# marqo-ai/marqo

Measured on AMD Instinct MI355X. Metric: embeddings/sec, higher is better.
Workload: dtype bf16; 1 GPU; open_clip ViT-B/32 image tower, uint8 224x224 resident in HBM (tower-only), batch 256/GPU; global_batch=256, parallelism=dp1 (replicated weights, sharded items, RCCL all_gather of embeddings), weights=random-init (seed 0) ViT-B-32, last_block_rows=pooled

## Files before the change

marqo_amd/csrc/embed.hip:

```cpp
#include "common.h"

namespace {

template <bool U8>
__global__ __launch_bounds__(256) void patchify_kernel(const void* __restrict__ in, bf16_t* __restrict__ out,
                                                       int64_t total_groups, int S, int P, int G, int Kp,
                                                       float sc0, float sc1, float sc2, float of0, float of1, float of2) {
    const int groups_per_row = Kp >> 3;
    const int PP = P * P;
    __shared__ float lutf[U8 ? 3 * 256 : 1];
    if (U8) {
        const float t = (float)threadIdx.x;
        lutf[threadIdx.x] = (t / 255.0f - of0) / sc0;
        lutf[(U8 ? 256 : 0) + (U8 ? threadIdx.x : 0)] = (t / 255.0f - of1) / sc1;
        lutf[(U8 ? 512 : 0) + (U8 ? threadIdx.x : 0)] = (t / 255.0f - of2) / sc2;
        __syncthreads();
    }
    for (int64_t gi = (int64_t)blockIdx.x * 256 + threadIdx.x; gi < total_groups; gi += (int64_t)gridDim.x * 256) {
        const int64_t prow = gi / groups_per_row;
        const int col0 = (int)(gi - prow * groups_per_row) * 8;
        const int64_t img = prow / (G * G);
        const int pidx = (int)(prow - img * (G * G));
        const int py = pidx / G, px = pidx - py * G;
        float v[8];
        if (U8 && (P & 7) == 0 && col0 < 3 * PP) {
            const int c = col0 / PP;
            const int rem = col0 - c * PP;
            const int ky = rem / P, kx = rem - ky * P;
            const uint8_t* src = (const uint8_t*)in + ((img * S + (py * P + ky)) * S + (px * P + kx)) * 3 + c;
#pragma unroll
            for (int e = 0; e < 8; ++e) v[e] = lutf[U8 ? c * 256 + src[e * 3] : 0];
        } else
#pragma unroll
        for (int e = 0; e < 8; ++e) {
            const int col = col0 + e;
            float val = 0.f;
            if (col < 3 * PP) {
                const int c = col / PP;
                const int rem = col - c * PP;
                const int ky = rem / P, kx = rem - ky * P;
                const int y = py * P + ky, x = px * P + kx;
                if (U8) {
                    const uint8_t b = ((const uint8_t*)in)[((img * S + y) * S + x) * 3 + c];
                    val = lutf[U8 ? c * 256 + b : 0];
                } else {
                    val = ((const float*)in)[((img * 3 + c) * S + y) * (int64_t)S + x];
                }
            }
            v[e] = val;
        }
        uint4 p;
        p.x = pack_bf16x2(v[0], v[1]);
        p.y = pack_bf16x2(v[2], v[3]);
        p.z = pack_bf16x2(v[4], v[5]);
        p.w = pack_bf16x2(v[6], v[7]);
        *(uint4*)(out + prow * Kp + col0) = p;
    }
}

__global__ __launch_bounds__(256) void patchify_u8x8_kernel(const uint8_t* __restrict__ in, bf16_t* __restrict__ out, int64_t total,
                                                            int S, int P, int G, int Kp, float sc0, float sc1, float sc2,
                                                            float of0, float of1, float of2) {
    __shared__ bf16_t lut[3 * 256];
    {
        const float t = (float)threadIdx.x;
        lut[threadIdx.x] = f32_to_bf16((t / 255.0f - of0) / sc0);
        lut[256 + threadIdx.x] = f32_to_bf16((t / 255.0f - of1) / sc1);
        lut[512 + threadIdx.x] = f32_to_bf16((t / 255.0f - of2) / sc2);
    }
    __syncthreads();
    const int per_row = P >> 3, per_patch = P * per_row, PP = P * P;
    for (int64_t gi = (int64_t)blockIdx.x * 256 + threadIdx.x; gi < total; gi += (int64_t)gridDim.x * 256) {
        const int64_t prow = gi / per_patch;
        const int rem = (int)(gi - prow * per_patch);
        const int ky = rem / per_row, kx = (rem - ky * per_row) * 8;
        const int64_t img = prow / (G * G);
        const int pidx = (int)(prow - img * (G * G));
        const int py = pidx / G, px = pidx - py * G;
        const uint2* src = (const uint2*)(in + ((img * S + (py * P + ky)) * S + (px * P + kx)) * 3);
        const uint2 w0 = src[0], w1 = src[1], w2 = src[2];
        const uint32_t words[6] = {w0.x, w0.y, w1.x, w1.y, w2.x, w2.y};
        uint32_t v[3][8];
#pragma unroll
        for (int b = 0; b < 24; ++b) {
            const uint32_t byte = (words[b >> 2] >> ((b & 3) * 8)) & 0xffu;
            const int c = b % 3, e = b / 3;
            v[c][e] = (uint32_t)lut[c * 256 + byte];
        }
        bf16_t* dst = out + prow * Kp + ky * P + kx;
#pragma unroll
        for (int c = 0; c < 3; ++c) {
            uint4 p;
            p.x = v[c][0] | (v[c][1] << 16);
            p.y = v[c][2] | (v[c][3] << 16);
            p.z = v[c][4] | (v[c][5] << 16);
            p.w = v[c][6] | (v[c][7] << 16);
            *(uint4*)(dst + c * PP) = p;
        }
    }
}

constexpr int MAXC = 8;
template <int CH>
__global__ __launch_bounds__(256, (CH <= 4 ? 8 : 4)) void vit_assemble_kernel(
    const float* __restrict__ patch_out, const float* __restrict__ cls, const float* __restrict__ pos,
    const float* __restrict__ gam, const float* __restrict__ bet, float* __restrict__ x, int64_t rows, int T, int W, float eps, int x_bf16) {
    const int lane = threadIdx.x & 63;
    const int64_t row = (int64_t)blockIdx.x * 4 + (threadIdx.x >> 6);
    if (row >= rows) return;
    auto put = [&](int c, const f32x4& y) {
        if (x_bf16) {
            uint2 q;
            q.x = pack_bf16x2(y[0], y[1]);
            q.y = pack_bf16x2(y[2], y[3]);
            *(uint2*)((bf16_t*)x + row * W + c * 4) = q;
        } else {
            *(f32x4*)(x + row * W + c * 4) = y;
        }
    };
    const int64_t b = row / T;
    const int t = (int)(row - b * T);
    const float* src = !cls ? patch_out + row * W : (t == 0 ? cls : patch_out + (b * (T - 1) + (t - 1)) * W);
    const float* pr = pos + (int64_t)t * W;
    const int nch = W >> 2;
    f32x4 v[CH];
#pragma unroll
    for (int i = 0; i < CH; ++i) {
        const int c = lane + i * 64;
        v[i] = c < nch ? *(const f32x4*)(src + c * 4) + *(const f32x4*)(pr + c * 4) : f32x4{0.f, 0.f, 0.f, 0.f};
    }
    if (!gam) {
#pragma unroll
        for (int i = 0; i < CH; ++i) {
            const int c = lane + i * 64;
            if (c < nch) put(c, v[i]);
        }
        return;
    }
    ln_normalize_row<CH>(v, lane, nch, W, eps);
#pragma unroll
    for (int i = 0; i < CH; ++i) {
        const int c = lane + i * 64;
        if (c < nch) {
            const f32x4 gg = *(const f32x4*)(gam + c * 4);
            const f32x4 bb = *(const f32x4*)(bet + c * 4);
            f32x4 y;
#pragma unroll
            for (int e = 0; e < 4; ++e) y[e] = v[i][e] * gg[e] + bb[e];
            put(c, y);
        }
    }
}

__global__ __launch_bounds__(256) void map_pool_kernel(const bf16_t* __restrict__ kv, const float* __restrict__ q, bf16_t* __restrict__ out,
                                                       int64_t nh, int T, int W, int heads, int hd) {
    extern __shared__ float sp[];
    const int lane = threadIdx.x & 63, wave = threadIdx.x >> 6;
    const int64_t item = (int64_t)blockIdx.x * 4 + wave;
    if (item >= nh) return;
    const int64_t img = item / heads;
    const int h = (int)(item - img * heads);
    float* p = sp + wave * T;
    const bf16_t* kbase = kv + img * T * (int64_t)(2 * W) + h * hd;
    const float* qh = q + h * hd;
    float mx = -INFINITY;
    for (int t = lane; t < T; t += 64) {
        const bf16_t* kr = kbase + (int64_t)t * (2 * W);
        float s = 0.f;
        for (int d = 0; d < hd; d += 8) {
            const uint4 k8 = *(const uint4*)(kr + d);
            const uint32_t kw[4] = {k8.x, k8.y, k8.z, k8.w};
#pragma unroll
            for (int e = 0; e < 4; ++e)
                s += __uint_as_float(kw[e] << 16) * qh[d + 2 * e] + __uint_as_float(kw[e] & 0xffff0000u) * qh[d + 2 * e + 1];
        }
        p[t] = s;
        mx = fmaxf(mx, s);
    }
    mx = wave_max(mx);
    float sum = 0.f;
    for (int t = lane; t < T; t += 64) {
        const float e = __expf(p[t] - mx);
        p[t] = e;
        sum += e;
    }
    sum = wave_sum(sum);
    const float inv = 1.0f / sum;
    __builtin_amdgcn_fence(__ATOMIC_RELEASE, "wavefront");
    __builtin_amdgcn_wave_barrier();
    const bf16_t* vbase = kbase + W;
    float o0 = 0.f, o1 = 0.f;
    const bool two = lane + 64 < hd;
    if (lane < hd) {
        for (int t = 0; t < T; ++t) {
            const bf16_t* vr = vbase + (int64_t)t * (2 * W);
            const float pt = p[t];
            o0 += pt * bf16_to_f32(vr[lane]);
            if (two) o1 += pt * bf16_to_f32(vr[lane + 64]);
        }
        bf16_t* orow = out + img * W + h * hd;
        orow[lane] = f32_to_bf16(o0 * inv);
        if (two) orow[lane + 64] = f32_to_bf16(o1 * inv);
    }
}

template <bool LN, int CH>
__global__ __launch_bounds__(256, (CH <= 2 ? 8 : 4)) void embed_tokens_kernel(
    const int32_t* __restrict__ ids, const int32_t* __restrict__ cu, const float* __restrict__ tok,
    const float* __restrict__ pos, const float* __restrict__ type0, const float* __restrict__ gam,
    const float* __restrict__ bet, float* __restrict__ x, bf16_t* __restrict__ xb, int W, int vocab, float eps, int last_pos) {
    const int lane = threadIdx.x & 63, wave = threadIdx.x >> 6;
    const int row0 = cu[blockIdx.x], len = cu[blockIdx.x + 1] - row0;
    const int nch = W >> 2;
    for (int t = wave; t < len; t += 4) {
        const int64_t row = row0 + t;
        int id = ids[row];
        id = id < 0 ? 0 : (id >= vocab ? vocab - 1 : id);
        const float* tr = tok + (int64_t)id * W;
        const float* pr = pos ? pos + (int64_t)((last_pos > 0 && t == len - 1) ? last_pos : t) * W : nullptr;
        f32x4 v[CH];
#pragma unroll
        for (int i = 0; i < CH; ++i) {
            const int c = lane + i * 64;
            v[i] = f32x4{0.f, 0.f, 0.f, 0.f};
            if (c < nch) {
                v[i] = *(const f32x4*)(tr + c * 4);
                if (pr) v[i] += *(const f32x4*)(pr + c * 4);
                if (type0) v[i] += *(const f32x4*)(type0 + c * 4);
            }
        }
        if (LN) ln_normalize_row<CH>(v, lane, nch, W, eps);
#pragma unroll
        for (int i = 0; i < CH; ++i) {
            const int c = lane + i * 64;
            if (c < nch) {
                f32x4 y = v[i];
                if (LN) {
                    const f32x4 gg = *(const f32x4*)(gam + c * 4);
                    const f32x4 bb = *(const f32x4*)(bet + c * 4);
#pragma unroll
                    for (int e = 0; e < 4; ++e) y[e] = v[i][e] * gg[e] + bb[e];
                }
                if (x) *(f32x4*)(x + row * W + c * 4) = y;
                if (xb) {
                    uint2 p;
                    p.x = pack_bf16x2(y[0], y[1]);
                    p.y = pack_bf16x2(y[2], y[3]);
                    *(uint2*)(xb + row * W + c * 4) = p;
                }
            }
        }
    }
}

__global__ __launch_bounds__(256) void pool_kernel(const float* __restrict__ x, const int32_t* __restrict__ cu,
                                                   float* __restrict__ out, int W, int pool, int normalize) {
    __shared__ float red[4];
    const int row0 = cu[blockIdx.x], len = cu[blockIdx.x + 1] - row0;
    float acc[8];
    float ss = 0.f;
#pragma unroll
    for (int i = 0; i < 8; ++i) {
        acc[i] = 0.f;
        const int c = threadIdx.x + i * 256;
        if (c < W) {
            if (pool == MQ_POOL_CLS) {
                acc[i] = x[(int64_t)row0 * W + c];
            } else {
                float s = 0.f;
                for (int t = 0; t < len; ++t) s += x[(int64_t)(row0 + t) * W + c];
                acc[i] = s / (float)len;
            }
            ss += acc[i] * acc[i];
        }
    }
    float inv = 1.f;
    if (normalize) {
        ss = wave_sum(ss);
        if ((threadIdx.x & 63) == 0) red[threadIdx.x >> 6] = ss;
        __syncthreads();
        const float tot = red[0] + red[1] + red[2] + red[3];
        inv = 1.0f / fmaxf(sqrtf(tot), 1e-12f);
    }
#pragma unroll
    for (int i = 0; i < 8; ++i) {
        const int c = threadIdx.x + i * 256;
        if (c < W) out[(int64_t)blockIdx.x * W + c] = acc[i] * inv;
    }
}

__global__ void last_rows_kernel(const int32_t* __restrict__ cu, int32_t* __restrict__ rows, int nseq) {
    const int i = blockIdx.x * blockDim.x + threadIdx.x;
    if (i < nseq) rows[i] = cu[i + 1] - 1;
}
__global__ void cls_rows_kernel(int32_t* __restrict__ rows, int n, int T) {
    const int i = blockIdx.x * blockDim.x + threadIdx.x;
    if (i < n) rows[i] = i * T;
}

template <bool SCATTER>
__global__ __launch_bounds__(256) void move_rows_kernel(uint4* __restrict__ sparse, const int32_t* __restrict__ idx,
                                                         uint4* __restrict__ dense, int64_t n, int chunks) {
    const int64_t total = n * chunks;
    for (int64_t i = (int64_t)blockIdx.x * 256 + threadIdx.x; i < total; i += (int64_t)gridDim.x * 256) {
        const int64_t r = i / chunks;
        const int c = (int)(i - r * chunks);
        uint4* sp = sparse + (int64_t)idx[r] * chunks + c;
        if (SCATTER) *sp = dense[i];
        else dense[i] = *sp;
    }
}

}

extern "C" int mq_patchify(const void* d_in, int32_t is_u8, void* d_out, int64_t n, int32_t S, int32_t P, int32_t Kp, const float* mean,
                           const float* std, void* stream) {
    const hipStream_t s = (hipStream_t)stream;
    const int G = S / P;
    const int64_t total = n * G * G * (Kp >> 3);
    if (total <= 0) return MQ_OK;
    MqProfScope prof(5, s);
    const unsigned grid = (unsigned)(cdiv64(total, 256) < 16384 ? cdiv64(total, 256) : 16384);
    if (is_u8 && (P & 7) == 0 && Kp == 3 * P * P && (S * 3) % 8 == 0 && ((uintptr_t)d_in & 7) == 0) {
        const int64_t items = n * G * G * P * (P >> 3);
        const unsigned g8 = (unsigned)(cdiv64(items, 256) < 16384 ? cdiv64(items, 256) : 16384);
        hipLaunchKernelGGL(patchify_u8x8_kernel, dim3(g8), dim3(256), 0, s, (const uint8_t*)d_in, (bf16_t*)d_out, items, S, P, G, Kp,
                           std[0], std[1], std[2], mean[0], mean[1], mean[2]);
    } else if (is_u8)
        hipLaunchKernelGGL(patchify_kernel<true>, dim3(grid), dim3(256), 0, s, d_in, (bf16_t*)d_out, total, S, P, G, Kp,
                           std[0], std[1], std[2], mean[0], mean[1], mean[2]);
    else
        hipLaunchKernelGGL(patchify_kernel<false>, dim3(grid), dim3(256), 0, s, d_in, (bf16_t*)d_out, total, S, P, G, Kp,
                           1.f, 1.f, 1.f, 0.f, 0.f, 0.f);
    MQ_CHECK_LAUNCH("mq_patchify");
    return MQ_OK;
}

extern "C" int mq_vit_assemble(const float* d_patch_out, const float* cls, const float* pos, const float* g, const float* b, void* d_x, int64_t n,
                               int32_t T, int32_t W, float eps, int32_t x_bf16, void* stream) {
    const hipStream_t s = (hipStream_t)stream;
    MQ_CHECK_ARG(W % 4 == 0 && W <= 64 * 4 * MAXC, "vit_assemble: W=%d unsupported", W);
    const int64_t rows = n * T;
    if (rows <= 0) return MQ_OK;
    MqProfScope prof(3, s);
    MQ_DISPATCH_CH(W, hipLaunchKernelGGL(vit_assemble_kernel<CH>, dim3((unsigned)cdiv64(rows, 4)), dim3(256), 0, s, d_patch_out,
                                         cls, pos, g, b, (float*)d_x, rows, T, W, eps, x_bf16));
    MQ_CHECK_LAUNCH("vit_assemble");
    return MQ_OK;
}

__global__ __launch_bounds__(256) void avg_tokens_kernel(const void* __restrict__ xv, int x_bf16, float* __restrict__ out, int T, int first, int W) {
    const int64_t img = blockIdx.x;
    const float inv = 1.0f / (float)(T - first);
    for (int c = threadIdx.x * 4; c < W; c += 256 * 4) {
        f32x4 acc = f32x4{0.f, 0.f, 0.f, 0.f};
        for (int t = first; t < T; ++t) {
            const int64_t o = (img * T + t) * (int64_t)W + c;
            if (x_bf16) {
                const uint2 q = *(const uint2*)((const bf16_t*)xv + o);
                acc += f32x4{__uint_as_float(q.x << 16), __uint_as_float(q.x & 0xffff0000u), __uint_as_float(q.y << 16), __uint_as_float(q.y & 0xffff0000u)};
            } else {
                acc += *(const f32x4*)((const float*)xv + o);
            }
        }
        *(f32x4*)(out + img * W + c) = acc * inv;
    }
}

extern "C" int mq_avg_tokens(const void* d_x, int32_t x_bf16, float* d_out, int64_t n, int32_t T, int32_t first, int32_t W, void* stream) {
    const hipStream_t s = (hipStream_t)stream;
    MQ_CHECK_ARG(W % 4 == 0 && first >= 0 && first < T, "avg_tokens: bad shape W=%d T=%d first=%d", W, T, first);
    if (n <= 0) return MQ_OK;
    MqProfScope prof(4, s);
    hipLaunchKernelGGL(avg_tokens_kernel, dim3((unsigned)n), dim3(256), 0, s, d_x, x_bf16, d_out, T, first, W);
    MQ_CHECK_LAUNCH("avg_tokens");
    return MQ_OK;
}

extern "C" int mq_map_pool(const void* d_kv, const float* d_q, void* d_out, int64_t n, int32_t T, int32_t W, int32_t heads, void* stream) {
    const hipStream_t s = (hipStream_t)stream;
    MQ_CHECK_ARG(heads >= 1 && W % heads == 0, "map_pool: W=%d heads=%d", W, heads);
    const int hd = W / heads;
    MQ_CHECK_ARG(hd % 8 == 0 && hd <= 128, "map_pool: head dim %d unsupported (multiple of 8, <= 128)", hd);
    MQ_CHECK_ARG(T >= 1 && T <= 4096, "map_pool: %d tokens unsupported", T);
    if (n <= 0) return MQ_OK;
    MqProfScope prof(4, s);
    const int64_t nh = n * heads;
    hipLaunchKernelGGL(map_pool_kernel, dim3((unsigned)cdiv64(nh, 4)), dim3(256), (size_t)4 * T * sizeof(float), s, (const bf16_t*)d_kv, d_q,
                       (bf16_t*)d_out, nh, T, W, heads, hd);
    MQ_CHECK_LAUNCH("map_pool");
    return MQ_OK;
}

extern "C" int mq_embed_tokens(const int32_t* d_ids, const int32_t* d_cu, int64_t nseq, const float* tok, const float* pos, const float* type0,
                               const float* g, const float* b, float* d_x, void* d_xb, int32_t W, int32_t vocab, float eps, int32_t last_pos,
                               void* stream) {
    const hipStream_t s = (hipStream_t)stream;
    MQ_CHECK_ARG(W % 4 == 0 && W <= 64 * 4 * MAXC, "embed_tokens: W=%d unsupported", W);
    if (nseq <= 0) return MQ_OK;
    MqProfScope prof(3, s);
    if (g)
        MQ_DISPATCH_CH(W, hipLaunchKernelGGL((embed_tokens_kernel<true, CH>), dim3((unsigned)nseq), dim3(256), 0, s, d_ids, d_cu,
                                             tok, pos, type0, g, b, d_x, (bf16_t*)d_xb, W, vocab, eps, last_pos));
    else
        MQ_DISPATCH_CH(W, hipLaunchKernelGGL((embed_tokens_kernel<false, CH>), dim3((unsigned)nseq), dim3(256), 0, s, d_ids, d_cu,
                                             tok, pos, type0, g, b, d_x, (bf16_t*)d_xb, W, vocab, eps, last_pos));
    MQ_CHECK_LAUNCH("embed_tokens");
    return MQ_OK;
}

__global__ __launch_bounds__(256) void rope_kernel(bf16_t* __restrict__ qkv, const int32_t* __restrict__ cu, int fixed_len, int Wa, int heads,
                                                   int hs, int hd, const float* __restrict__ inv_freq) {
    const int row0 = cu ? cu[blockIdx.x] : blockIdx.x * fixed_len;
    const int len = cu ? cu[blockIdx.x + 1] - row0 : fixed_len;
    const int half = hd >> 1, chunks = half >> 3;
    const int per_row = 2 * heads * chunks;
    for (int it = threadIdx.x; it < len * per_row; it += 256) {
        const int t = it / per_row, r = it - t * per_row;
        const int qk = r / (heads * chunks), r2 = r - qk * heads * chunks;
        const int h = r2 / chunks, c = r2 - h * chunks;
        bf16_t* p = qkv + (int64_t)(row0 + t) * (3 * Wa) + qk * Wa + h * hs + c * 8;
        uint4 lo = *(const uint4*)p, hi = *(const uint4*)(p + half);
        uint32_t* l = (uint32_t*)&lo;
        uint32_t* u = (uint32_t*)&hi;
#pragma unroll
        for (int e = 0; e < 4; ++e) {
            float x1[2] = {bf16_to_f32((bf16_t)(l[e] & 0xffff)), bf16_to_f32((bf16_t)(l[e] >> 16))};
            float x2[2] = {bf16_to_f32((bf16_t)(u[e] & 0xffff)), bf16_to_f32((bf16_t)(u[e] >> 16))};
            float y1[2], y2[2];
#pragma unroll
            for (int k = 0; k < 2; ++k) {
                float sn, cs;
                sincosf((float)t * inv_freq[c * 8 + e * 2 + k], &sn, &cs);
                y1[k] = x1[k] * cs - x2[k] * sn;
                y2[k] = x2[k] * cs + x1[k] * sn;
            }
            l[e] = pack_bf16x2(y1[0], y1[1]);
            u[e] = pack_bf16x2(y2[0], y2[1]);
        }
        *(uint4*)p = lo;
        *(uint4*)(p + half) = hi;
    }
}

extern "C" int mq_rope(void* d_qkv, const int32_t* d_cu, int64_t nseq, int32_t fixed_len, int32_t Wa, int32_t heads, const float* d_inv_freq,
                       void* stream) {
    const hipStream_t s = (hipStream_t)stream;
    const int hs = Wa / heads;
    MQ_CHECK_ARG(hs * heads == Wa && hs % 16 == 0, "rope: head width %d must be a multiple of 16", hs);
    if (nseq <= 0) return MQ_OK;
    MqProfScope prof(3, s);
    hipLaunchKernelGGL(rope_kernel, dim3((unsigned)nseq), dim3(256), 0, s, (bf16_t*)d_qkv, d_cu, fixed_len, Wa, heads, hs, hs, d_inv_freq);
    MQ_CHECK_LAUNCH("rope");
    return MQ_OK;
}

__device__ __forceinline__ float glu_act(float g, int act) { return act == MQ_ACT_SILU ? silu(g) : act == MQ_ACT_QUICKGELU ? quick_gelu(g) : gelu_erf(g); }

__global__ __launch_bounds__(256) void glu_kernel(bf16_t* __restrict__ buf, int64_t rows, int F, int act) {
    const int chunks = F >> 3;
    for (int64_t i = (int64_t)blockIdx.x * 256 + threadIdx.x; i < rows * chunks; i += (int64_t)gridDim.x * 256) {
        const int64_t r = i / chunks;
        const int c = (int)(i - r * chunks);
        bf16_t* p = buf + r * (2 * (int64_t)F) + c * 8;
        uint4 up = *(const uint4*)p;
        const uint4 gt = *(const uint4*)(p + F);
        uint32_t* a = (uint32_t*)&up;
        const uint32_t* g = (const uint32_t*)&gt;
#pragma unroll
        for (int e = 0; e < 4; ++e) {
            const float u0 = bf16_to_f32((bf16_t)(a[e] & 0xffff)), u1 = bf16_to_f32((bf16_t)(a[e] >> 16));
            const float g0 = bf16_to_f32((bf16_t)(g[e] & 0xffff)), g1 = bf16_to_f32((bf16_t)(g[e] >> 16));
            a[e] = pack_bf16x2(u0 * glu_act(g0, act), u1 * glu_act(g1, act));
        }
        *(uint4*)p = up;
    }
}

int mq_glu_il_rows(void* d_buf, int64_t rows, int F, int act, hipStream_t s);
extern "C" int mq_glu(void* d_buf, int64_t rows, int32_t F, int32_t act, int32_t interleaved, void* stream) {
    const hipStream_t s = (hipStream_t)stream;
    MQ_CHECK_ARG(F % 8 == 0 && (!interleaved || F % 16 == 0), "glu: F=%d must be a multiple of 8 (16 interleaved)", F);
    if (rows <= 0) return MQ_OK;
    MqProfScope prof(3, s);
    const int64_t blocks = cdiv64(rows * (F >> 3), 256);
    if (interleaved) {
        MQ_CHECK_ARG(F <= 4096, "glu (interleaved): F=%d > 4096", F);
        return mq_glu_il_rows(d_buf, rows, F, act, s);
    }
    hipLaunchKernelGGL(glu_kernel, dim3((unsigned)(blocks < 16384 ? blocks : 16384)), dim3(256), 0, s, (bf16_t*)d_buf, rows, F, act);
    MQ_CHECK_LAUNCH("glu");
    return MQ_OK;
}

template <int CH, int MODE = 0>
__global__ __launch_bounds__(256) void glu_ln_kernel(bf16_t* __restrict__ buf, int64_t rows, int F, int Ft, int act, const float* __restrict__ g,
                                                     const float* __restrict__ b, float eps) {
    const int64_t row = (int64_t)blockIdx.x * 4 + (threadIdx.x >> 6);
    const int lane = threadIdx.x & 63;
    if (row >= rows) return;
    bf16_t* p = buf + row * (2 * (int64_t)F);
    float v[CH][8];
    float s1 = 0.f;
// ... 165 lines not shown
```

marqo_amd/csrc/gemm_bf16.hip:

```cpp
#include <map>
#include <mutex>
#include <string>
#include <type_traits>
#include "common.h"
#include "gemm_epilogue.h"
#include "gemm_loop.h"
#include "gemm_sched.h"

extern mq_knob mq_tower_row_select;
extern mq_knob mq_tower_ln_fold;
extern mq_knob mq_tower_subln_fold;
extern mq_knob mq_tower_attn_proj;
extern mq_knob mq_tower_panel_gemm;
extern mq_knob mq_attention_waves;
extern mq_knob mq_tower_residual_bf16;
extern mq_knob mq_gemm_small_max_rows;
bool mq_gemm_small_ok(int64_t M, int64_t N, int64_t K, bool ln);
bool mq_gemm_small_grouped_ok(int64_t M, int64_t N, int64_t K);
extern mq_knob mq_gemm_small_group_rows;
extern mq_knob mq_ln_prefetch;
extern mq_knob mq_ln_rows_per_wave;
extern mq_knob mq_ln_bf16_wide;
int mq_gemm_small(const void* d_A, int64_t lda, const void* d_W, int64_t ldw, const float* d_bias, const void* d_residual, void* d_out,
                  int64_t ldc, int64_t M, int64_t N, int64_t K, int flags, hipStream_t s);
int mq_gemm_wd_launch(int flags, int mt, int ns, const void* A, int64_t lda, const void* W, int64_t ldw, const float* bias, const float* residual, void* out,
                      int64_t ldc, int M, int N, int K, const GemmGeom& g, int wide, const GemmLn& ln, hipStream_t s);

int mq_device_ok();

namespace {

struct GemmSk {
    float* partials;
    unsigned* flags;
    unsigned epoch;
    int tail_splits;
};

template <int FLAGS, int MT, int NH, int WM, int ORD>
__global__ __launch_bounds__(128 * WM, (NH == 1 && WM == 2) ? 2 : 1) void gemm_nt_kernel(
    const bf16_t* __restrict__ A, int64_t lda, const bf16_t* __restrict__ Wt, int64_t ldw,
    const float* __restrict__ bias, const float* residual, void* out, int64_t ldc,
    int M, int N, int K, int tiles_n, int num_tiles, int cgroup, int band_rows, int wide_store,
    unsigned a_bytes, unsigned w_bytes, GemmLn ln, GemmSk sk) {
    static_assert(!(NH == 2 && WM == 2), "the 4-wave 224 x 256 tile (one wave per SIMD) lost on every shape (profiles/r05a, r05b) and was removed in round 6");
    constexpr int BM = 16 * MT * WM, BN = 128 * NH;
    constexpr bool TAIL = WM == 4;
    constexpr int NTW = 4 * NH;
    constexpr int A_TILE_BYTES = BM * BK * 2, W_TILE_BYTES = BN * BK * 2;
    constexpr int STAGE_BYTES = A_TILE_BYTES + W_TILE_BYTES;
    constexpr int NPA = MT, NPW = 8 * NH / WM;
    constexpr int NLD = NPA + NPW;
    constexpr int NLR = MT + NTW;
    constexpr int NM = NTW * MT;
    constexpr bool LN_RES = (FLAGS & MQ_EPI_LN_APPLY) && (FLAGS & MQ_EPI_RESIDUAL);
    constexpr int ERG = !(FLAGS & MQ_EPI_RESIDUAL) ? MT : LN_RES ? ((NH == 2 || WM == 4) ? 1 : MT <= 4 ? MT : 2) : (NH == 2 || WM == 4) ? MT
                        : (FLAGS & MQ_EPI_OUT_F32) ? (MT <= 3 ? MT : (MT + 1) / 2) : (MT <= 5 ? MT : 3);
    extern __shared__ __attribute__((aligned(16))) char smem[];

    const GemmTileMap<BM, BN> tile_map(num_tiles, tiles_n, M, cgroup, band_rows);

    const int tid = threadIdx.x;
    const int lane = tid & 63;
    const int wave = __builtin_amdgcn_readfirstlane(tid >> 6);
    const int wm = wave >> 1, wn = wave & 1;
    const int l15 = lane & 15, g = lane >> 4;

    const int srow = lane >> 3;
    const unsigned chunk_off = (unsigned)(((lane & 7) ^ (srow & 7)) * 16);
    unsigned a_vo[NPA], w_vo[NPW];
    auto set_sources = [&](int m0, int n0) {
#pragma unroll
        for (int i = 0; i < MT; ++i) {
            int gm = m0 + wave * (8 * MT) + i * 8 + srow; gm = gm < M ? gm : M - 1;
            a_vo[i] = (unsigned)gm * (unsigned)lda * 2u + chunk_off;
        }
#pragma unroll
        for (int i = 0; i < NPW; ++i) {
            int gn = n0 + wave * (8 * NPW) + i * 8 + srow; gn = gn < N ? gn : N - 1;
            w_vo[i] = (unsigned)gn * (unsigned)ldw * 2u + chunk_off;
        }
    };
    const int nk = K / BK;
    int d_vbid = blockIdx.x, d_k = 0;
    unsigned a_rec = a_bytes, w_rec = w_bytes;
    bool tail_mode = false;
    int d_left = 0;
    const bool has_main = !TAIL || (int)blockIdx.x < num_tiles;
    if (has_main) {
        int m0, n0;
        tile_map.origin(d_vbid, m0, n0);
        set_sources(m0, n0);
    } else {
        a_rec = 0; w_rec = 0;
#pragma unroll
        for (int i = 0; i < NPA; ++i) a_vo[i] = 0;
#pragma unroll
        for (int i = 0; i < NPW; ++i) w_vo[i] = 0;
    }
    const unsigned lds0 = (unsigned)(uintptr_t)(__attribute__((address_space(3))) char*)smem;
    const unsigned dma_a0 = lds0 + (unsigned)wave * (8 * MT * 128), dma_w0 = lds0 + A_TILE_BYTES + (unsigned)wave * (8 * NPW * 128);
    auto issue_piece = [&](int i, unsigned bufoff) {
        const unsigned soff = (unsigned)d_k * (BK * 2);
        if (i < NPA) dma16(__builtin_amdgcn_make_buffer_rsrc((void*)A, 0, a_rec, 0x00020000), a_vo[i < NPA ? i : 0], soff, dma_a0 + bufoff + (unsigned)i * 1024u);
        else dma16(__builtin_amdgcn_make_buffer_rsrc((void*)Wt, 0, w_rec, 0x00020000), w_vo[i >= NPA ? i - NPA : 0], soff, dma_w0 + bufoff + (unsigned)(i - NPA) * 1024u);
    };
    auto advance_cursor = [&]() {
        if (TAIL && tail_mode) {
            ++d_k;
            if (--d_left <= 0) { a_rec = 0; w_rec = 0; }
            return;
        }
        if (++d_k == nk) {
            d_k = 0;
            d_vbid += gridDim.x;
            if (d_vbid < num_tiles) {
                int m0, n0;
                tile_map.origin(d_vbid, m0, n0);
                set_sources(m0, n0);
            } else {
                a_rec = 0; w_rec = 0;
            }
        }
    };

    const unsigned sw0 = (unsigned)((g ^ (l15 & 7)) << 4), sw1 = (unsigned)(((g + 4) ^ (l15 & 7)) << 4);
    const unsigned a_row = lds0 + (unsigned)((wm * (16 * MT) + l15) * 128);
    const unsigned w_row = lds0 + A_TILE_BYTES + (unsigned)((wn * (16 * NTW) + l15) * 128);
    const unsigned aB0 = a_row + sw0, aB1 = a_row + sw1, wB0 = w_row + sw0, wB1 = w_row + sw1;

    f32x4 acc[NH][MT][4];
    bf16x8 wf0[NTW], af0[MT], wf1[NTW], af1[MT];
    auto read_piece = [&](auto p_tag, unsigned wbase, unsigned abase, bf16x8 (&wf)[NTW], bf16x8 (&af)[MT]) {
        constexpr int P = decltype(p_tag)::value;
        if constexpr (P < NTW) wf[P] = lds_read16<P * 2048>(wbase);
        else af[P - NTW] = lds_read16<(P - NTW) * 2048>(abase);
    };

    unsigned bufoff = 0;
    auto prime = [&]() {
        bufoff = 0;
#pragma unroll
        for (int i = 0; i < NLD; ++i) issue_piece(i, 0);
        advance_cursor();
#pragma unroll
        for (int i = 0; i < NLD; ++i) issue_piece(i, STAGE_BYTES);
        advance_cursor();
        asm volatile("s_waitcnt vmcnt(%0)" ::"n"(NLD) : "memory");
        __builtin_amdgcn_s_barrier();
        asm volatile("" ::: "memory");
        static_for<NLR>([&](auto p_tag) { read_piece(p_tag, wB0, aB0, wf0, af0); });
    };
    if (has_main) prime();

    int c_vbid = blockIdx.x;

    auto kstep = [&]() {
        asm volatile("s_waitcnt lgkmcnt(0)" ::: "memory");
#pragma unroll
        for (int t = 0; t < NTW; ++t) landed(wf0[t]);
#pragma unroll
        for (int t = 0; t < MT; ++t) landed(af0[t]);
        __builtin_amdgcn_sched_barrier(0);
        {
            const unsigned wb = wB1 + bufoff, ab = aB1 + bufoff;
            constexpr int NS1 = NLR;
            static_for<NM>([&](auto idx_tag) {
                constexpr int idx = decltype(idx_tag)::value, mt = idx / NTW, nt = idx % NTW;
// ... 357 lines not shown
    MQ_CHECK_ARG(d_A && d_W && d_out, "mq_gemm_bf16: null operand");
    MQ_TRY(check_shape("mq_gemm_bf16", M, N, K, lda, ldw, ldc));
    MQ_CHECK_ARG(!(flags & MQ_EPI_BIAS) || d_bias, "mq_gemm_bf16: MQ_EPI_BIAS without bias");
    MQ_CHECK_ARG(!(flags & MQ_EPI_RESIDUAL) || d_residual, "mq_gemm_bf16: MQ_EPI_RESIDUAL without residual");
    MQ_CHECK_ARG(!(flags & MQ_EPI_GLU) || N % 32 == 0, "mq_gemm_bf16: MQ_EPI_GLU needs N %% 32 == 0 (16 up + 16 gate rows per group)");
    hipStream_t s = (hipStream_t)stream;
    if (flags & MQ_EPI_GLU) {
        MqProfScope prof(0, s, 2.0 * (double)M * (double)N * (double)K);
        return launch_gemm<MQ_EPI_BIAS | MQ_EPI_GLU>(d_A, lda, d_W, ldw, d_bias, d_residual ? (const float*)d_residual : nullptr, d_out, ldc, (int)M, (int)N, (int)K, s);
    }
    if (flags & MQ_EPI_RELU) {
        MqProfScope prof(0, s, 2.0 * (double)M * (double)N * (double)K);
        if (flags == (MQ_EPI_BIAS | MQ_EPI_RELU))
            return launch_gemm<MQ_EPI_BIAS | MQ_EPI_RELU>(d_A, lda, d_W, ldw, d_bias, nullptr, d_out, ldc, (int)M, (int)N, (int)K, s);
        if (flags == (MQ_EPI_BIAS | MQ_EPI_RESIDUAL | MQ_EPI_RELU))
            return launch_gemm<MQ_EPI_BIAS | MQ_EPI_RESIDUAL | MQ_EPI_RELU>(d_A, lda, d_W, ldw, d_bias, d_residual, d_out, ldc, (int)M, (int)N, (int)K, s);
        mq_set_error("mq_gemm_bf16: unsupported epilogue flag combination 0x%x", flags);
        return MQ_ERR_INVALID;
    }
    if (mq_gemm_small_ok(M, N, K, false) || mq_gemm_small_grouped_ok(M, N, K)) return mq_gemm_small(d_A, lda, d_W, ldw, d_bias, d_residual, d_out, ldc, M, N, K, flags, s);
    MqProfScope prof(0, s, 2.0 * (double)M * (double)N * (double)K);
    const int m = (int)M, n = (int)N, k = (int)K;
#define MQ_GEMM_CASE(F) \
    case (F): return launch_gemm<(F)>(d_A, lda, d_W, ldw, d_bias, d_residual, d_out, ldc, m, n, k, s)
    switch (flags) {
        MQ_GEMM_CASE(0);
        MQ_GEMM_CASE(MQ_EPI_OUT_F32);
        MQ_GEMM_CASE(MQ_EPI_BIAS | MQ_EPI_OUT_F32);
        MQ_GEMM_CASE(MQ_EPI_BIAS);
        MQ_GEMM_CASE(MQ_EPI_BIAS | MQ_EPI_GELU);
        MQ_GEMM_CASE(MQ_EPI_BIAS | MQ_EPI_QUICKGELU);
        MQ_GEMM_CASE(MQ_EPI_BIAS | MQ_EPI_RESIDUAL | MQ_EPI_OUT_F32);
        MQ_GEMM_CASE(MQ_EPI_BIAS | MQ_EPI_RESIDUAL);
        MQ_GEMM_CASE(MQ_EPI_BIAS | MQ_EPI_GLU);
        default:
            mq_set_error("mq_gemm_bf16: unsupported epilogue flag combination 0x%x", flags);
            return MQ_ERR_INVALID;
    }
#undef MQ_GEMM_CASE
}

extern "C" int mq_gemm_bf16_ln(const void* d_A, int64_t lda, const void* d_W, int64_t ldw, const float* d_bias, const float* d_colsum,
                               const float* d_rowstats, void* d_out, int64_t ldc, int64_t M, int64_t N, int64_t K, int flags, void* stream) {
    MQ_CHECK_ARG(d_A && d_W && d_out && d_bias && d_colsum && d_rowstats, "mq_gemm_bf16_ln: null operand");
    MQ_TRY(check_shape("mq_gemm_bf16_ln", M, N, K, lda, ldw, ldc));
    MQ_CHECK_ARG(!(flags & MQ_EPI_GLU) || N % 32 == 0, "mq_gemm_bf16_ln: MQ_EPI_GLU needs N %% 32 == 0");
    hipStream_t s = (hipStream_t)stream;
    MqProfScope prof(0, s, 2.0 * (double)M * (double)N * (double)K);
    const int m = (int)M, n = (int)N, k = (int)K;
    GemmLn ln{};
    ln.colsum = d_colsum;
    ln.rowstats = (const float2*)d_rowstats;
#define MQ_GEMM_LN_CASE(F) \
    case (F): return launch_gemm<(F)>(d_A, lda, d_W, ldw, d_bias, nullptr, d_out, ldc, m, n, k, s, ln)
    switch (flags | MQ_EPI_LN_APPLY) {
        MQ_GEMM_LN_CASE(MQ_EPI_BIAS | MQ_EPI_LN_APPLY);
        MQ_GEMM_LN_CASE(MQ_EPI_BIAS | MQ_EPI_GELU | MQ_EPI_LN_APPLY);
        MQ_GEMM_LN_CASE(MQ_EPI_BIAS | MQ_EPI_QUICKGELU | MQ_EPI_LN_APPLY);
        MQ_GEMM_LN_CASE(MQ_EPI_BIAS | MQ_EPI_RELU | MQ_EPI_LN_APPLY);
        MQ_GEMM_LN_CASE(MQ_EPI_BIAS | MQ_EPI_GLU | MQ_EPI_LN_APPLY);
        default:
            mq_set_error("mq_gemm_bf16_ln: unsupported epilogue flag combination 0x%x", flags);
            return MQ_ERR_INVALID;
    }
#undef MQ_GEMM_LN_CASE
}

extern "C" int mq_gemm_bf16_rs(const void* d_A, int64_t lda, const void* d_W, int64_t ldw, const float* d_bias, const void* d_residual, void* d_out,
                               int64_t ldc, int64_t M, int64_t N, int64_t K, int flags, float* d_partials, void* stream) {
    MQ_CHECK_ARG(d_A && d_W && d_out && d_bias && d_residual && d_partials, "mq_gemm_bf16_rs: null operand");
    MQ_CHECK_ARG((flags | MQ_EPI_ROW_STATS) == (MQ_EPI_BIAS | MQ_EPI_RESIDUAL | MQ_EPI_ROW_STATS), "mq_gemm_bf16_rs: flags must be MQ_EPI_BIAS | MQ_EPI_RESIDUAL");
    MQ_TRY(check_shape("mq_gemm_bf16_rs", M, N, K, lda, ldw, ldc));
    hipStream_t s = (hipStream_t)stream;
    MqProfScope prof(0, s, 2.0 * (double)M * (double)N * (double)K);
    GemmLn ln{};
    ln.partials = (float2*)d_partials;
    ln.nslots = (int)((N + 63) / 64);
    ln.part_ld = M;
    return launch_gemm<MQ_EPI_BIAS | MQ_EPI_RESIDUAL | MQ_EPI_ROW_STATS>(d_A, lda, d_W, ldw, d_bias, (const float*)d_residual, d_out, ldc, (int)M, (int)N, (int)K, s, ln);
}

extern "C" int mq_gemm_bf16_lnrs(const void* d_A, int64_t lda, const void* d_W, int64_t ldw, const float* d_bias, const float* d_colsum, const float* d_rowstats,
                                 const void* d_residual, void* d_out, int64_t ldc, int64_t M, int64_t N, int64_t K, int flags, float* d_partials, void* stream) {
    MQ_CHECK_ARG(d_A && d_W && d_out && d_bias && d_colsum && d_rowstats && d_partials, "mq_gemm_bf16_lnrs: null operand");
    MQ_CHECK_ARG(flags == (MQ_EPI_BIAS | MQ_EPI_RESIDUAL) || flags == (MQ_EPI_BIAS | MQ_EPI_GLU), "mq_gemm_bf16_lnrs: flags must be MQ_EPI_BIAS | MQ_EPI_RESIDUAL or MQ_EPI_BIAS | MQ_EPI_GLU");
    MQ_CHECK_ARG(!(flags & MQ_EPI_RESIDUAL) || d_residual, "mq_gemm_bf16_lnrs: MQ_EPI_RESIDUAL without residual");
    MQ_TRY(check_shape("mq_gemm_bf16_lnrs", M, N, K, lda, ldw, ldc));
    MQ_CHECK_ARG(!(flags & MQ_EPI_GLU) || N % 32 == 0, "mq_gemm_bf16_lnrs: MQ_EPI_GLU needs N %% 32 == 0");
    hipStream_t s = (hipStream_t)stream;
    MqProfScope prof(0, s, 2.0 * (double)M * (double)N * (double)K);
    GemmLn ln{};
    ln.colsum = d_colsum;
    ln.rowstats = (const float2*)d_rowstats;
    ln.partials = (float2*)d_partials;
    ln.nslots = (int)((N + 63) / 64);
    ln.part_ld = M;
    if (flags & MQ_EPI_GLU)
        return launch_gemm<MQ_EPI_BIAS | MQ_EPI_GLU | MQ_EPI_LN_APPLY | MQ_EPI_ROW_STATS>(d_A, lda, d_W, ldw, d_bias, nullptr, d_out, ldc, (int)M, (int)N, (int)K, s, ln);
    return launch_gemm<MQ_EPI_BIAS | MQ_EPI_RESIDUAL | MQ_EPI_LN_APPLY | MQ_EPI_ROW_STATS>(d_A, lda, d_W, ldw, d_bias, (const float*)d_residual, d_out, ldc, (int)M, (int)N, (int)K, s, ln);
}

int mq_row_stats_finalize_pf(const float* d_partials, int32_t nslots, float* d_stats, int64_t rows, int32_t W, float eps, const void* pf_a, size_t bytes_a,
                             const void* pf_b, size_t bytes_b, hipStream_t s);
extern "C" int64_t mq_gemm_band_counters(int64_t M) { return M / 32 + 16; }
bool mq_gemm_rs_in_launch() { return g_tune.rs_fin && !g_tune.tail; }
extern "C" int mq_gemm_bf16_rsf(const void* d_A, int64_t lda, const void* d_W, int64_t ldw, const float* d_bias, const void* d_residual, void* d_out,
                                int64_t ldc, int64_t M, int64_t N, int64_t K, int flags, float* d_partials, float* d_stats, float eps,
                                uint32_t* d_band_ctr, const void* d_pf_a, size_t pf_a_bytes, const void* d_pf_b, size_t pf_b_bytes, void* stream) {
    MQ_CHECK_ARG(d_A && d_W && d_out && d_bias && d_residual && d_partials && d_stats, "mq_gemm_bf16_rsf: null operand");
    MQ_CHECK_ARG((flags | MQ_EPI_ROW_STATS) == (MQ_EPI_BIAS | MQ_EPI_RESIDUAL | MQ_EPI_ROW_STATS), "mq_gemm_bf16_rsf: flags must be MQ_EPI_BIAS | MQ_EPI_RESIDUAL");
    MQ_TRY(check_shape("mq_gemm_bf16_rsf", M, N, K, lda, ldw, ldc));
    hipStream_t s = (hipStream_t)stream;
    const int nslots = (int)((N + 63) / 64);
    const bool in_launch = d_band_ctr && g_tune.rs_fin && !g_tune.tail;
    {
        MqProfScope prof(0, s, 2.0 * (double)M * (double)N * (double)K);
        GemmLn ln{};
        ln.partials = (float2*)d_partials;
        ln.nslots = nslots;
        ln.part_ld = M;
        if (in_launch) {
            ln.band_ctr = d_band_ctr;
            ln.stats_out = (float2*)d_stats;
            ln.inv_w = 1.0f / (float)N;
            ln.eps = eps;
            ln.pf_a = (const unsigned*)d_pf_a;
            ln.pf_b = (const unsigned*)d_pf_b;
            ln.pf_na = d_pf_a ? (unsigned)(pf_a_bytes / 128) : 0u;
            ln.pf_nb = d_pf_b ? (unsigned)(pf_b_bytes / 128) : 0u;
        }
        MQ_TRY(launch_gemm<MQ_EPI_BIAS | MQ_EPI_RESIDUAL | MQ_EPI_ROW_STATS>(d_A, lda, d_W, ldw, d_bias, (const float*)d_residual, d_out, ldc, (int)M, (int)N, (int)K, s, ln));
    }
    if (in_launch) return MQ_OK;
    return mq_row_stats_finalize_pf(d_partials, nslots, d_stats, M, (int32_t)N, eps, d_pf_a, pf_a_bytes, d_pf_b, pf_b_bytes, s);
}

extern "C" int mq_tune(const char* key, int value) {
    MQ_CHECK_ARG(key, "mq_tune: null key");
    const std::string k(key);
    if (k == "gemm_mt") g_tune.mt = value;
    else if (k == "gemm_cgroup") g_tune.cgroup = value;
    else if (k == "gemm_nh") { g_tune.nh = value; g_tune.fp8_big = value == 4 ? 0 : value; }
    else if (k == "gemm_tail") g_tune.tail = value;
    else if (k == "gemm_wd") g_tune.wd = value;
    else if (k == "rs_finalize") g_tune.rs_fin = value;
    else if (k == "row_select") mq_tower_row_select = value;
    else if (k == "ln_fold") mq_tower_ln_fold = value;
    else if (k == "subln_fold") mq_tower_subln_fold = value;
    else if (k == "attn_proj") mq_tower_attn_proj = value;
    else if (k == "panel_gemm") mq_tower_panel_gemm = value;
    else if (k == "xcd_band") mq_xcd_band = value;
    else if (k == "attn_waves") mq_attention_waves = value;
    else if (k == "residual_bf16") mq_tower_residual_bf16 = value;
    else if (k == "small_m") mq_gemm_small_max_rows = value;
    else if (k == "small_m_grouped") mq_gemm_small_group_rows = value;
    else if (k == "ln_prefetch") mq_ln_prefetch = value;
    else if (k == "ln_rows") mq_ln_rows_per_wave = value;
    else if (k == "ln_bf16_wide") mq_ln_bf16_wide = value;
    else if (k == "gemm_addr_limit_mb") mq_gemm_addr_limit = value > 0 ? ((uint64_t)value << 20) - 1 : 0xffffffffull;
    else { mq_set_error("mq_tune: unknown key %s", key); return MQ_ERR_INVALID; }
    return MQ_OK;
}
#endif
```

marqo_amd/csrc/rowops.hip:

```cpp
#include <stdlib.h>
#include "common.h"

mq_knob mq_ln_rows_per_wave{getenv("MQ_LN_ROWS") ? atoi(getenv("MQ_LN_ROWS")) : 2};
extern mq_knob mq_gemm_small_max_rows;
int mq_layernorm_pf(const void* d_x, int x_bf16, const int32_t* d_row_idx, const float* d_g, const float* d_b, void* d_out_bf16, float* d_out_f32,
                    int64_t rows, int32_t W, float eps, const void* pf_a, size_t bytes_a, const void* pf_b, size_t bytes_b, hipStream_t s);
int mq_layernorm_fp8_pf(const void* d_x, int x_bf16, const float* d_g, const float* d_b, void* d_out_fp8, float* d_row_scale, float* d_out_f32,
                        int64_t rows, int32_t W, float eps, const void* pf_a, size_t bytes_a, const void* pf_b, size_t bytes_b, hipStream_t s);
mq_knob mq_ln_bf16_wide{getenv("MQ_LN_BF16_WIDE") ? atoi(getenv("MQ_LN_BF16_WIDE")) : 1};

namespace {

constexpr int LN_MAX_CHUNKS = 8;

struct LnExtra {
    int band;
    unsigned na, nb;
    const unsigned* pfa;
    const unsigned* pfb;
    unsigned step;
};
constexpr int LN_PF = 2;

__device__ __forceinline__ void ln_prefetch_issue(const LnExtra& ex, unsigned (&pq)[LN_PF]) {
#pragma unroll
    for (int j = 0; j < LN_PF; ++j) pq[j] = 0u;
    if (ex.na | ex.nb) {
        const unsigned nt = gridDim.x * 256u, t = blockIdx.x * 256u + threadIdx.x;
#pragma unroll
        for (int j = 0; j < LN_PF; ++j) {
            const unsigned c = t + j * nt;
            if (c < ex.na) pq[j] = ex.pfa[(size_t)c * ex.step];
            else if (c - ex.na < ex.nb) pq[j] = ex.pfb[(size_t)(c - ex.na) * ex.step];
        }
    }
}
__device__ __forceinline__ void ln_prefetch_retire(const unsigned (&pq)[LN_PF]) {
#pragma unroll
    for (int j = 0; j < LN_PF; ++j) asm volatile("" ::"v"(pq[j]));
}

template <int CH, int R, bool XB = false>
__global__ __launch_bounds__(256, (CH * R <= 2 ? 8 : CH * R <= 4 ? 5 : CH * R <= 6 ? 3 : 2)) void layernorm_kernel(
    const void* __restrict__ xv, const int32_t* __restrict__ row_idx, const float* __restrict__ gam,
    const float* __restrict__ bet, bf16_t* out_bf16, float* out_f32, int64_t rows, int W, float eps, LnExtra ex) {
    const int lane = threadIdx.x & 63;
    const int64_t row0 = ((int64_t)xcd_banded_block(blockIdx.x, gridDim.x, ex.band) * 4 + (threadIdx.x >> 6)) * R;
    if (row0 >= rows) return;
    const int nch = W >> 2;

    f32x4 v[R][CH];
#pragma unroll
    for (int r = 0; r < R; ++r) {
        const int64_t row = row0 + r < rows ? row0 + r : rows - 1;
        const int64_t src = row_idx ? (int64_t)row_idx[row] : row;
#pragma unroll
        for (int i = 0; i < CH; ++i) {
            const int c = lane + i * 64;
            if (c >= nch) { v[r][i] = f32x4{0.f, 0.f, 0.f, 0.f}; continue; }
            if (XB) {
                const uint2 q = *(const uint2*)((const bf16_t*)xv + src * W + c * 4);
                v[r][i] = f32x4{__uint_as_float(q.x << 16), __uint_as_float(q.x & 0xffff0000u), __uint_as_float(q.y << 16), __uint_as_float(q.y & 0xffff0000u)};
            } else {
                v[r][i] = *(const f32x4*)((const float*)xv + src * W + c * 4);
            }
        }
    }
    unsigned pq[LN_PF];
    ln_prefetch_issue(ex, pq);
    f32x4 gv[CH], bv[CH];
#pragma unroll
    for (int i = 0; i < CH; ++i) {
        const int c = lane + i * 64;
        gv[i] = c < nch ? *(const f32x4*)(gam + c * 4) : f32x4{0.f, 0.f, 0.f, 0.f};
        bv[i] = c < nch ? *(const f32x4*)(bet + c * 4) : f32x4{0.f, 0.f, 0.f, 0.f};
    }
    float mean[R], rstd[R];
#pragma unroll
    for (int r = 0; r < R; ++r) {
        float s1 = 0.f;
#pragma unroll
        for (int i = 0; i < CH; ++i)
            if (lane + i * 64 < nch) s1 += (v[r][i][0] + v[r][i][1]) + (v[r][i][2] + v[r][i][3]);
        mean[r] = s1;
    }
#pragma unroll
    for (int o = 32; o > 0; o >>= 1)
#pragma unroll
        for (int r = 0; r < R; ++r) mean[r] += __shfl_xor(mean[r], o, 64);
#pragma unroll
    for (int r = 0; r < R; ++r) {
        mean[r] = mean[r] / (float)W;
        float s2 = 0.f;
#pragma unroll
        for (int i = 0; i < CH; ++i)
            if (lane + i * 64 < nch) {
#pragma unroll
                for (int e = 0; e < 4; ++e) { const float d = v[r][i][e] - mean[r]; s2 += d * d; }
            }
        rstd[r] = s2;
    }
#pragma unroll
    for (int o = 32; o > 0; o >>= 1)
#pragma unroll
        for (int r = 0; r < R; ++r) rstd[r] += __shfl_xor(rstd[r], o, 64);
#pragma unroll
    for (int r = 0; r < R; ++r) rstd[r] = rsqrtf(rstd[r] / (float)W + eps);

#pragma unroll
    for (int i = 0; i < CH; ++i) {
        const int c = lane + i * 64;
        if (c < nch) {
            const f32x4 gg = gv[i], bb = bv[i];
#pragma unroll
            for (int r = 0; r < R; ++r) {
                const int64_t row = row0 + r;
                if (row >= rows) continue;
                f32x4 y;
#pragma unroll
                for (int e = 0; e < 4; ++e) y[e] = (v[r][i][e] - mean[r]) * rstd[r] * gg[e] + bb[e];
                if (out_f32) *(f32x4*)(out_f32 + row * W + c * 4) = y;
                if (out_bf16) {
                    uint2 p;
                    p.x = pack_bf16x2(y[0], y[1]);
                    p.y = pack_bf16x2(y[2], y[3]);
                    *(uint2*)(out_bf16 + row * W + c * 4) = p;
                }
            }
        }
    }
    ln_prefetch_retire(pq);
}

template <int CH8, int R>
__global__ __launch_bounds__(256) void layernorm_bf16in_kernel(
    const bf16_t* __restrict__ x, const int32_t* __restrict__ row_idx, const float* __restrict__ gam, const float* __restrict__ bet,
    bf16_t* out_bf16, float* out_f32, int64_t rows, int W, float eps, LnExtra ex) {
    const int lane = threadIdx.x & 63;
    const int64_t row0 = ((int64_t)xcd_banded_block(blockIdx.x, gridDim.x, ex.band) * 4 + (threadIdx.x >> 6)) * R;
    if (row0 >= rows) return;
    const int nch = W >> 3;
    float v[R][CH8][8];
#pragma unroll
    for (int r = 0; r < R; ++r) {
        const int64_t row = row0 + r < rows ? row0 + r : rows - 1;
        const int64_t src = row_idx ? (int64_t)row_idx[row] : row;
#pragma unroll
        for (int i = 0; i < CH8; ++i) {
            const int c = lane + i * 64;
            uint4 q = make_uint4(0u, 0u, 0u, 0u);
            if (c < nch) q = *(const uint4*)(x + src * W + c * 8);
            const unsigned w4[4] = {q.x, q.y, q.z, q.w};
#pragma unroll
            for (int e = 0; e < 4; ++e) { v[r][i][2 * e] = __uint_as_float(w4[e] << 16); v[r][i][2 * e + 1] = __uint_as_float(w4[e] & 0xffff0000u); }
        }
    }
    unsigned pq[LN_PF];
    ln_prefetch_issue(ex, pq);
    f32x4 gv[CH8][2], bv[CH8][2];
#pragma unroll
    for (int i = 0; i < CH8; ++i) {
        const int c = lane + i * 64;
#pragma unroll
        for (int h = 0; h < 2; ++h) {
            gv[i][h] = c < nch ? *(const f32x4*)(gam + c * 8 + h * 4) : f32x4{0.f, 0.f, 0.f, 0.f};
            bv[i][h] = c < nch ? *(const f32x4*)(bet + c * 8 + h * 4) : f32x4{0.f, 0.f, 0.f, 0.f};
        }
    }
    float mean[R], rstd[R];
#pragma unroll
    for (int r = 0; r < R; ++r) {
        float s1 = 0.f;
#pragma unroll
        for (int i = 0; i < CH8; ++i)
            if (lane + i * 64 < nch) s1 += ((v[r][i][0] + v[r][i][1]) + (v[r][i][2] + v[r][i][3])) + ((v[r][i][4] + v[r][i][5]) + (v[r][i][6] + v[r][i][7]));
        mean[r] = s1;
    }
#pragma unroll
    for (int o = 32; o > 0; o >>= 1)
#pragma unroll
        for (int r = 0; r < R; ++r) mean[r] += __shfl_xor(mean[r], o, 64);
#pragma unroll
    for (int r = 0; r < R; ++r) {
        mean[r] = mean[r] / (float)W;
        float s2 = 0.f;
#pragma unroll
        for (int i = 0; i < CH8; ++i)
            if (lane + i * 64 < nch) {
#pragma unroll
                for (int e = 0; e < 8; ++e) { const float d = v[r][i][e] - mean[r]; s2 += d * d; }
            }
        rstd[r] = s2;
    }
#pragma unroll
    for (int o = 32; o > 0; o >>= 1)
#pragma unroll
        for (int r = 0; r < R; ++r) rstd[r] += __shfl_xor(rstd[r], o, 64);
#pragma unroll
    for (int r = 0; r < R; ++r) rstd[r] = rsqrtf(rstd[r] / (float)W + eps);
#pragma unroll
    for (int i = 0; i < CH8; ++i) {
        const int c = lane + i * 64;
        if (c >= nch) continue;
#pragma unroll
        for (int r = 0; r < R; ++r) {
            const int64_t row = row0 + r;
            if (row >= rows) continue;
            float y[8];
#pragma unroll
            for (int e = 0; e < 8; ++e) y[e] = (v[r][i][e] - mean[r]) * rstd[r] * gv[i][e >> 2][e & 3] + bv[i][e >> 2][e & 3];
            if (out_f32) {
                *(f32x4*)(out_f32 + row * W + c * 8) = f32x4{y[0], y[1], y[2], y[3]};
                *(f32x4*)(out_f32 + row * W + c * 8 + 4) = f32x4{y[4], y[5], y[6], y[7]};
            }
            if (out_bf16)
                *(uint4*)(out_bf16 + row * W + c * 8) = make_uint4(pack_bf16x2(y[0], y[1]), pack_bf16x2(y[2], y[3]), pack_bf16x2(y[4], y[5]), pack_bf16x2(y[6], y[7]));
        }
    }
    ln_prefetch_retire(pq);
}

template <int CH8, int R>
__global__ __launch_bounds__(256) void row_stats_bf16_kernel(const bf16_t* __restrict__ x, float2* __restrict__ stats, int64_t rows, int W, float eps, LnExtra ex) {
    const int lane = threadIdx.x & 63;
    const int64_t row0 = ((int64_t)xcd_banded_block(blockIdx.x, gridDim.x, ex.band) * 4 + (threadIdx.x >> 6)) * R;
    if (row0 >= rows) return;
    const int nch = W >> 3;
    float v[R][CH8][8];
#pragma unroll
    for (int r = 0; r < R; ++r) {
        const int64_t row = row0 + r < rows ? row0 + r : rows - 1;
#pragma unroll
        for (int i = 0; i < CH8; ++i) {
            const int c = lane + i * 64;
            uint4 q = make_uint4(0u, 0u, 0u, 0u);
            if (c < nch) q = *(const uint4*)(x + row * W + c * 8);
            const unsigned w4[4] = {q.x, q.y, q.z, q.w};
#pragma unroll
            for (int e = 0; e < 4; ++e) { v[r][i][2 * e] = __uint_as_float(w4[e] << 16); v[r][i][2 * e + 1] = __uint_as_float(w4[e] & 0xffff0000u); }
        }
    }
    unsigned pq[LN_PF];
    ln_prefetch_issue(ex, pq);
    float mean[R], rstd[R];
#pragma unroll
    for (int r = 0; r < R; ++r) {
        float s1 = 0.f;
#pragma unroll
        for (int i = 0; i < CH8; ++i)
            if (lane + i * 64 < nch) s1 += ((v[r][i][0] + v[r][i][1]) + (v[r][i][2] + v[r][i][3])) + ((v[r][i][4] + v[r][i][5]) + (v[r][i][6] + v[r][i][7]));
        mean[r] = s1;
    }
#pragma unroll
    for (int o = 32; o > 0; o >>= 1)
#pragma unroll
        for (int r = 0; r < R; ++r) mean[r] += __shfl_xor(mean[r], o, 64);
#pragma unroll
    for (int r = 0; r < R; ++r) {
        mean[r] = mean[r] / (float)W;
        float s2 = 0.f;
#pragma unroll
        for (int i = 0; i < CH8; ++i)
            if (lane + i * 64 < nch) {
#pragma unroll
                for (int e = 0; e < 8; ++e) { const float d = v[r][i][e] - mean[r]; s2 += d * d; }
            }
        rstd[r] = s2;
    }
#pragma unroll
    for (int o = 32; o > 0; o >>= 1)
#pragma unroll
        for (int r = 0; r < R; ++r) rstd[r] += __shfl_xor(rstd[r], o, 64);
#pragma unroll
    for (int r = 0; r < R; ++r)
        if (lane == 0 && row0 + r < rows) stats[row0 + r] = make_float2(mean[r], rsqrtf(rstd[r] / (float)W + eps));
    ln_prefetch_retire(pq);
}

template <int CH, bool NORM = true, bool XB = false>
__global__ __launch_bounds__(256, (CH <= 2 ? 8 : CH <= 4 ? 5 : CH <= 6 ? 3 : 2)) void layernorm_fp8_kernel(
    const void* __restrict__ x, const float* __restrict__ gam, const float* __restrict__ bet, uint8_t* __restrict__ out8,
    float* __restrict__ row_scale, float* out_f32, int64_t rows, int W, float eps, LnExtra ex) {
    const int lane = threadIdx.x & 63;
    const int64_t row = (int64_t)blockIdx.x * 4 + (threadIdx.x >> 6);
    if (row >= rows) return;
    const int nch = W >> 2;
    f32x4 v[CH];
#pragma unroll
    for (int i = 0; i < CH; ++i) {
        const int c = lane + i * 64;
        if (c >= nch) { v[i] = f32x4{0.f, 0.f, 0.f, 0.f}; continue; }
        if (XB) {
            const uint2 q = *(const uint2*)((const bf16_t*)x + row * W + c * 4);
            v[i] = f32x4{__uint_as_float(q.x << 16), __uint_as_float(q.x & 0xffff0000u), __uint_as_float(q.y << 16), __uint_as_float(q.y & 0xffff0000u)};
        } else {
            v[i] = *(const f32x4*)((const float*)x + row * W + c * 4);
        }
    }
    unsigned pq[LN_PF];
    ln_prefetch_issue(ex, pq);
    if (NORM) ln_normalize_row<CH>(v, lane, nch, W, eps);
    float mx = 0.f;
#pragma unroll
    for (int i = 0; i < CH; ++i) {
        const int c = lane + i * 64;
        if (c < nch) {
            if (NORM) {
                const f32x4 gg = *(const f32x4*)(gam + c * 4);
                const f32x4 bb = *(const f32x4*)(bet + c * 4);
#pragma unroll
                for (int e = 0; e < 4; ++e) v[i][e] = v[i][e] * gg[e] + bb[e];
                if (out_f32) *(f32x4*)(out_f32 + row * W + c * 4) = v[i];
            }
#pragma unroll
            for (int e = 0; e < 4; ++e) mx = fmaxf(mx, fabsf(v[i][e]));
        }
    }
    mx = wave_max(mx);
    const float sc = mx > 0.f ? mx * (1.0f / 448.f) : 1.f;
    const float inv = 1.0f / sc;
    if (lane == 0) row_scale[row] = sc;
#pragma unroll
    for (int i = 0; i < CH; ++i) {
        const int c = lane + i * 64;
        if (c < nch) {
            int w = __builtin_amdgcn_cvt_pk_fp8_f32(v[i][0] * inv, v[i][1] * inv, 0, false);
            w = __builtin_amdgcn_cvt_pk_fp8_f32(v[i][2] * inv, v[i][3] * inv, w, true);
            *(int*)(out8 + row * W + c * 4) = w;
        }
    }
    ln_prefetch_retire(pq);
}

__global__ __launch_bounds__(256) void l2norm_kernel(const float* __restrict__ x, float* out, int64_t rows, int D) {
    const int lane = threadIdx.x & 63;
    const int64_t row = (int64_t)blockIdx.x * 4 + (threadIdx.x >> 6);
    if (row >= rows) return;
    const float* xr = x + row * D;
    float s = 0.f;
    for (int c = lane; c < D; c += 64) { const float t = xr[c]; s += t * t; }
    const float inv = 1.0f / sqrtf(wave_sum(s));
    for (int c = lane; c < D; c += 64) out[row * D + c] = xr[c] * inv;
}

__global__ __launch_bounds__(256) void cast_bf16_kernel(const float* __restrict__ x, bf16_t* out, int64_t n4) {
    for (int64_t i = (int64_t)blockIdx.x * 256 + threadIdx.x; i < n4; i += (int64_t)gridDim.x * 256) {
        const f32x4 v = *(const f32x4*)(x + i * 4);
        uint2 p;
        p.x = pack_bf16x2(v[0], v[1]);
        p.y = pack_bf16x2(v[2], v[3]);
        *(uint2*)(out + i * 4) = p;
    }
}

}

extern "C" int mq_layernorm(const float* d_x, const int32_t* d_row_idx, const float* d_g, const float* d_b,
                            void* d_out_bf16, float* d_out_f32, int64_t rows, int32_t W, float eps, void* stream) {
    return mq_layernorm_ex(d_x, 0, d_row_idx, d_g, d_b, d_out_bf16, d_out_f32, rows, W, eps, stream);
}

mq_knob mq_ln_prefetch{getenv("MQ_LN_PREFETCH") ? atoi(getenv("MQ_LN_PREFETCH")) : 1};

static LnExtra ln_extra(int band, int64_t rows, const void* pf_a, size_t bytes_a, const void* pf_b, size_t bytes_b) {
    LnExtra ex{band, 0u, 0u, nullptr, nullptr, 32u};
    if (mq_ln_prefetch && rows >= 1024) {
        const size_t gran = mq_ln_prefetch == 2 ? 64 : mq_ln_prefetch == 3 ? 32 : 128;
        ex.step = (unsigned)(gran / 4);
        auto lines = [gran](const void* p, size_t b) { return (p && ((uintptr_t)p & 3) == 0) ? (unsigned)(b < ((size_t)1 << 30) ? b / gran : 0) : 0u; };
        ex.pfa = (const unsigned*)pf_a; ex.na = lines(pf_a, bytes_a);
        ex.pfb = (const unsigned*)pf_b; ex.nb = lines(pf_b, bytes_b);
    }
    return ex;
}


extern "C" int mq_layernorm_ex(const void* d_x, int x_bf16, const int32_t* d_row_idx, const float* d_g, const float* d_b,
                               void* d_out_bf16, float* d_out_f32, int64_t rows, int32_t W, float eps, void* stream) {
    return mq_layernorm_pf(d_x, x_bf16, d_row_idx, d_g, d_b, d_out_bf16, d_out_f32, rows, W, eps, nullptr, 0, nullptr, 0, (hipStream_t)stream);
}

int mq_layernorm_pf(const void* d_x, int x_bf16, const int32_t* d_row_idx, const float* d_g, const float* d_b, void* d_out_bf16, float* d_out_f32,
                    int64_t rows, int32_t W, float eps, const void* pf_a, size_t bytes_a, const void* pf_b, size_t bytes_b, hipStream_t s) {
    MQ_CHECK_ARG(d_x && d_g && d_b && (d_out_bf16 || d_out_f32), "mq_layernorm: null pointer");
    MQ_CHECK_ARG(W >= 4 && W % 4 == 0 && W <= 64 * 4 * LN_MAX_CHUNKS, "mq_layernorm: W=%d unsupported (multiple of 4, <= 2048)", W);
    if (rows <= 0) return MQ_OK;
    MqProfScope prof(1, s);
    const LnExtra band = ln_extra((mq_xcd_band && !d_row_idx && rows >= 4096) ? 1 : 0, rows, pf_a, bytes_a, pf_b, bytes_b);
    if (x_bf16 && mq_ln_bf16_wide && rows > mq_gemm_small_max_rows && W % 8 == 0 && W <= 1024 && ((uintptr_t)d_x & 15) == 0 && (!d_out_bf16 || ((uintptr_t)d_out_bf16 & 15) == 0)) {
        const bf16_t* xb = (const bf16_t*)d_x;
        const bool many = rows >= 16384;
        if (W <= 512) {
            if (many && mq_ln_bf16_wide < 4) hipLaunchKernelGGL((layernorm_bf16in_kernel<1, 2>), dim3((unsigned)cdiv64(rows, 8)), dim3(256), 0, s, xb, d_row_idx, d_g, d_b, (bf16_t*)d_out_bf16, d_out_f32, rows, (int)W, eps, band);
            else if (many) hipLaunchKernelGGL((layernorm_bf16in_kernel<1, 4>), dim3((unsigned)cdiv64(rows, 16)), dim3(256), 0, s, xb, d_row_idx, d_g, d_b, (bf16_t*)d_out_bf16, d_out_f32, rows, (int)W, eps, band);
            else hipLaunchKernelGGL((layernorm_bf16in_kernel<1, 1>), dim3((unsigned)cdiv64(rows, 4)), dim3(256), 0, s, xb, d_row_idx, d_g, d_b, (bf16_t*)d_out_bf16, d_out_f32, rows, (int)W, eps, band);
        } else {
            if (rows >= 16384 && mq_ln_bf16_wide >= 4) hipLaunchKernelGGL((layernorm_bf16in_kernel<2, 4>), dim3((unsigned)cdiv64(rows, 16)), dim3(256), 0, s, xb, d_row_idx, d_g, d_b, (bf16_t*)d_out_bf16, d_out_f32, rows, (int)W, eps, band);
            else if (rows >= 8192) hipLaunchKernelGGL((layernorm_bf16in_kernel<2, 2>), dim3((unsigned)cdiv64(rows, 8)), dim3(256), 0, s, xb, d_row_idx, d_g, d_b, (bf16_t*)d_out_bf16, d_out_f32, rows, (int)W, eps, band);
            else hipLaunchKernelGGL((layernorm_bf16in_kernel<2, 1>), dim3((unsigned)cdiv64(rows, 4)), dim3(256), 0, s, xb, d_row_idx, d_g, d_b, (bf16_t*)d_out_bf16, d_out_f32, rows, (int)W, eps, band);
        }
    } else if (x_bf16) {
        if (mq_ln_rows_per_wave >= 2 && rows >= 8192 && W <= 1024)
            MQ_DISPATCH_CH(W, hipLaunchKernelGGL((layernorm_kernel<CH, 2, true>), dim3((unsigned)cdiv64(rows, 8)), dim3(256), 0, s, d_x, d_row_idx,
                                                 d_g, d_b, (bf16_t*)d_out_bf16, d_out_f32, rows, (int)W, eps, band));
        else
            MQ_DISPATCH_CH(W, hipLaunchKernelGGL((layernorm_kernel<CH, 1, true>), dim3((unsigned)cdiv64(rows, 4)), dim3(256), 0, s, d_x, d_row_idx,
                                                 d_g, d_b, (bf16_t*)d_out_bf16, d_out_f32, rows, (int)W, eps, band));
    } else if (mq_ln_rows_per_wave >= 2 && rows >= 8192 && W <= 1024)
        MQ_DISPATCH_CH(W, hipLaunchKernelGGL((layernorm_kernel<CH, 2>), dim3((unsigned)cdiv64(rows, 8)), dim3(256), 0, s, d_x, d_row_idx,
                                             d_g, d_b, (bf16_t*)d_out_bf16, d_out_f32, rows, (int)W, eps, band));
    else
        MQ_DISPATCH_CH(W, hipLaunchKernelGGL((layernorm_kernel<CH, 1>), dim3((unsigned)cdiv64(rows, 4)), dim3(256), 0, s, d_x, d_row_idx,
                                             d_g, d_b, (bf16_t*)d_out_bf16, d_out_f32, rows, (int)W, eps, band));
    MQ_CHECK_LAUNCH("mq_layernorm");
    return MQ_OK;
}

extern "C" int mq_layernorm_fp8_ex(const void* d_x, int x_bf16, const float* d_g, const float* d_b, void* d_out_fp8, float* d_row_scale,
                                   float* d_out_f32, int64_t rows, int32_t W, float eps, void* stream) {
    return mq_layernorm_fp8_pf(d_x, x_bf16, d_g, d_b, d_out_fp8, d_row_scale, d_out_f32, rows, W, eps, nullptr, 0, nullptr, 0, (hipStream_t)stream);
}

int mq_layernorm_fp8_pf(const void* d_x, int x_bf16, const float* d_g, const float* d_b, void* d_out_fp8, float* d_row_scale, float* d_out_f32,
                        int64_t rows, int32_t W, float eps, const void* pf_a, size_t bytes_a, const void* pf_b, size_t bytes_b, hipStream_t s) {
    MQ_CHECK_ARG(d_x && d_g && d_b && d_out_fp8 && d_row_scale, "mq_layernorm_fp8: null pointer");
    MQ_CHECK_ARG(W >= 4 && W % 4 == 0 && W <= 64 * 4 * LN_MAX_CHUNKS, "mq_layernorm_fp8: W=%d unsupported (multiple of 4, <= 2048)", W);
    MQ_CHECK_ARG(!x_bf16 || !d_out_f32, "mq_layernorm_fp8: the fp32 copy of the normalised rows belongs to the fp32 stream");
    if (rows <= 0) return MQ_OK;
    MqProfScope prof(1, s);
    const LnExtra ex = ln_extra(0, rows, pf_a, bytes_a, pf_b, bytes_b);
    if (x_bf16)
        MQ_DISPATCH_CH(W, hipLaunchKernelGGL((layernorm_fp8_kernel<CH, true, true>), dim3((unsigned)cdiv64(rows, 4)), dim3(256), 0, s, d_x, d_g, d_b,
                                             (uint8_t*)d_out_fp8, d_row_scale, d_out_f32, rows, (int)W, eps, ex));
    else
        MQ_DISPATCH_CH(W, hipLaunchKernelGGL((layernorm_fp8_kernel<CH, true, false>), dim3((unsigned)cdiv64(rows, 4)), dim3(256), 0, s, d_x, d_g, d_b,
                                             (uint8_t*)d_out_fp8, d_row_scale, d_out_f32, rows, (int)W, eps, ex));
    MQ_CHECK_LAUNCH("mq_layernorm_fp8");
    return MQ_OK;
}

extern "C" int mq_layernorm_fp8(const float* d_x, const float* d_g, const float* d_b, void* d_out_fp8, float* d_row_scale, float* d_out_f32,
                                int64_t rows, int32_t W, float eps, void* stream) {
    return mq_layernorm_fp8_ex(d_x, 0, d_g, d_b, d_out_fp8, d_row_scale, d_out_f32, rows, W, eps, stream);
}

extern "C" int mq_rowquant_fp8(const float* d_x, void* d_out_fp8, float* d_row_scale, int64_t rows, int32_t W, void* stream) {
    MQ_CHECK_ARG(d_x && d_out_fp8 && d_row_scale, "mq_rowquant_fp8: null pointer");
    MQ_CHECK_ARG(W >= 4 && W % 4 == 0 && W <= 64 * 4 * LN_MAX_CHUNKS, "mq_rowquant_fp8: W=%d unsupported (multiple of 4, <= 2048)", W);
    if (rows <= 0) return MQ_OK;
    hipStream_t s = (hipStream_t)stream;
    MqProfScope prof(1, s);
    MQ_DISPATCH_CH(W, hipLaunchKernelGGL((layernorm_fp8_kernel<CH, false>), dim3((unsigned)cdiv64(rows, 4)), dim3(256), 0, s, (const void*)d_x,
                                         (const float*)nullptr, (const float*)nullptr, (uint8_t*)d_out_fp8, d_row_scale, (float*)nullptr, rows,
                                         (int)W, 0.f, LnExtra{0, 0u, 0u, nullptr, nullptr, 32u}));
    MQ_CHECK_LAUNCH("mq_rowquant_fp8");
    return MQ_OK;
}

extern "C" int mq_l2_normalize(const float* d_x, float* d_out, int64_t rows, int32_t D, void* stream) {
    MQ_CHECK_ARG(d_x && d_out && D >= 1, "mq_l2_normalize: bad argument");
    if (rows <= 0) return MQ_OK;
    hipStream_t s = (hipStream_t)stream;
    MqProfScope prof(4, s);
    hipLaunchKernelGGL(l2norm_kernel, dim3((unsigned)cdiv64(rows, 4)), dim3(256), 0, s, d_x, d_out, rows, (int)D);
    MQ_CHECK_LAUNCH("mq_l2_normalize");
    return MQ_OK;
}

int mq_cast_bf16(const float* d_x, void* d_out, int64_t n, hipStream_t s) {
    MQ_CHECK_ARG(n % 4 == 0, "mq_cast_bf16: n must be a multiple of 4");
    if (n <= 0) return MQ_OK;
    MqProfScope prof(1, s);
    const int64_t n4 = n / 4;
    const unsigned grid = (unsigned)(cdiv64(n4, 256) < 4096 ? cdiv64(n4, 256) : 4096);
    hipLaunchKernelGGL(cast_bf16_kernel, dim3(grid), dim3(256), 0, s, d_x, (bf16_t*)d_out, n4);
    MQ_CHECK_LAUNCH("mq_cast_bf16");
    return MQ_OK;
}


__global__ __launch_bounds__(256) void row_stats_finalize_kernel(const float2* __restrict__ partials, int nslots, float2* __restrict__ stats, int64_t rows,
                                                                 float inv_w, float eps, LnExtra ex) {
    const int64_t row = (int64_t)blockIdx.x * 256 + threadIdx.x;
    float s1 = 0.f, s2 = 0.f;
    if (row < rows) {
        const float2* p = partials + row;
        for (int i0 = 0; i0 < nslots; i0 += 8) {
            float2 v[8];
#pragma unroll
            for (int j = 0; j < 8; ++j) v[j] = i0 + j < nslots ? p[(int64_t)(i0 + j) * rows] : make_float2(0.f, 0.f);
#pragma unroll
            for (int j = 0; j < 8; ++j) { s1 += v[j].x; s2 += v[j].y; }
        }
    }
    unsigned pq[LN_PF];
    ln_prefetch_issue(ex, pq);
    if (row < rows) stats[row] = mq_finalize_stats(s1, s2, inv_w, eps);
    ln_prefetch_retire(pq);
}
int mq_row_stats_finalize_pf(const float* d_partials, int32_t nslots, float* d_stats, int64_t rows, int32_t W, float eps, const void* pf_a, size_t bytes_a,
                             const void* pf_b, size_t bytes_b, hipStream_t s) {
    MQ_CHECK_ARG(d_partials && d_stats && nslots >= 1 && W >= 1, "mq_row_stats_finalize: bad argument");
    if (rows <= 0) return MQ_OK;
    MqProfScope prof(1, s);
    LnExtra ex = ln_extra(0, rows, pf_a, bytes_a, pf_b, bytes_b);
    const int64_t want = ((int64_t)ex.na + ex.nb + LN_PF - 1) / LN_PF;
    const int64_t threads = rows > want ? rows : want;
    hipLaunchKernelGGL(row_stats_finalize_kernel, dim3((unsigned)cdiv64(threads, 256)), dim3(256), 0, s, (const float2*)d_partials, (int)nslots, (float2*)d_stats,
                       rows, 1.0f / (float)W, eps, ex);
    MQ_CHECK_LAUNCH("mq_row_stats_finalize");
    return MQ_OK;
}
extern "C" int mq_row_stats_finalize(const float* d_partials, int32_t nslots, float* d_stats, int64_t rows, int32_t W, float eps, void* stream) {
    return mq_row_stats_finalize_pf(d_partials, nslots, d_stats, rows, W, eps, nullptr, 0, nullptr, 0, (hipStream_t)stream);
}

bool mq_row_stats_ok(int32_t W) { return W % 8 == 0 && W >= 8 && W <= 2048; }
int mq_row_stats_pf(const void* d_x_bf16, float* d_stats, int64_t rows, int32_t W, float eps, const void* pf_a, size_t bytes_a, const void* pf_b,
                    size_t bytes_b, hipStream_t s) {
    MQ_CHECK_ARG(d_x_bf16 && d_stats, "mq_row_stats: null pointer");
    MQ_CHECK_ARG(mq_row_stats_ok(W), "mq_row_stats: W=%d unsupported (multiple of 8, <= 2048)", W);
    if (rows <= 0) return MQ_OK;
    MqProfScope prof(1, s);
    const LnExtra ex = ln_extra((mq_xcd_band && rows >= 4096) ? 1 : 0, rows, pf_a, bytes_a, pf_b, bytes_b);
    const int ch8 = ((W >> 3) + 63) / 64;
    const bool many = rows >= 4096;
    const int R = !many ? 1 : ch8 == 1 ? 4 : ch8 == 2 ? 2 : 1;
    const unsigned grid = (unsigned)cdiv64(rows, 4 * R);
#define MQ_RS(C, RR) hipLaunchKernelGGL((row_stats_bf16_kernel<C, RR>), dim3(grid), dim3(256), 0, s, (const bf16_t*)d_x_bf16, (float2*)d_stats, rows, (int)W, eps, ex)
    if (ch8 == 1) { if (R == 4) MQ_RS(1, 4); else MQ_RS(1, 1); }
    else if (ch8 == 2) { if (R == 2) MQ_RS(2, 2); else MQ_RS(2, 1); }
    else MQ_RS(4, 1);
#undef MQ_RS
    MQ_CHECK_LAUNCH("mq_row_stats");
    return MQ_OK;
}
extern "C" int mq_row_stats(const void* d_x_bf16, float* d_stats, int64_t rows, int32_t W, float eps, void* stream) {
    return mq_row_stats_pf(d_x_bf16, d_stats, rows, W, eps, nullptr, 0, nullptr, 0, (hipStream_t)stream);
}
```

marqo_amd/csrc/towers.hip:

```cpp
#include <stdlib.h>
#include "common.h"

int mq_cast_bf16(const float* d_x, void* d_out, int64_t n, hipStream_t s);
extern "C" int mq_rowquant_fp8(const float* d_x, void* d_out_fp8, float* d_row_scale, int64_t rows, int32_t W, void* stream);

static_assert(sizeof(mq_block_weights) == 36 * 8, "mq_block_weights layout");
static_assert(sizeof(mq_encoder_cfg) == 112, "mq_encoder_cfg layout");
static_assert(sizeof(mq_vit_cfg) == 168 && sizeof(mq_clip_text_cfg) == 128 && sizeof(mq_bert_cfg) == 136, "tower cfg layouts");
static_assert(sizeof(mq_vit_weights) == 11 * 8 && sizeof(mq_map_head) == 11 * 8 && sizeof(mq_clip_text_weights) == 7 * 8, "tower weight layouts");

mq_knob mq_tower_row_select{getenv("MQ_ROW_SELECT") ? atoi(getenv("MQ_ROW_SELECT")) : 1};
mq_knob mq_tower_ln_fold{getenv("MQ_LN_FOLD") ? atoi(getenv("MQ_LN_FOLD")) : 2};
mq_knob mq_tower_subln_fold{getenv("MQ_SUBLN_FOLD") ? atoi(getenv("MQ_SUBLN_FOLD")) : 1};
mq_knob mq_tower_attn_proj{getenv("MQ_ATTN_PROJ") ? atoi(getenv("MQ_ATTN_PROJ")) : 128};
static bool attn_proj_fill_ok(int64_t nseq) {
    const int64_t rounds = (nseq + 255) / 256;
    return mq_tower_attn_proj > 0 && nseq >= mq_tower_attn_proj && (rounds == 1 || nseq * 4 >= rounds * 256 * 3);
}
mq_knob mq_tower_panel_gemm{getenv("MQ_PANEL_GEMM") ? atoi(getenv("MQ_PANEL_GEMM")) : 0};
static bool panel_fill_ok(int64_t nseq) {
    const int64_t rounds = (nseq + 255) / 256;
    return mq_tower_panel_gemm > 0 && nseq >= mq_tower_panel_gemm && nseq * 4 >= rounds * 256 * 3;
}
mq_knob mq_tower_residual_bf16{getenv("MQ_RESIDUAL_BF16") ? atoi(getenv("MQ_RESIDUAL_BF16")) : 0};
extern "C" int mq_layernorm_ex(const void* d_x, int x_bf16, const int32_t* d_row_idx, const float* d_g, const float* d_b, void* d_out_bf16,
                               float* d_out_f32, int64_t rows, int32_t W, float eps, void* stream);
bool mq_gemm_small_ok(int64_t M, int64_t N, int64_t K, bool ln);
int mq_ln_gemm_small(const void* d_x, int64_t ldx, int x_bf16, const float* ln_g, const float* ln_b, float eps, const void* d_W, int64_t ldw,
                     const float* d_bias, void* d_out, int64_t ldc, int64_t M, int64_t N, int64_t K, int flags, float* d_ln_out,
                     const int32_t* d_rows, hipStream_t s);
int mq_layernorm_pf(const void* d_x, int x_bf16, const int32_t* d_row_idx, const float* d_g, const float* d_b, void* d_out_bf16, float* d_out_f32,
                    int64_t rows, int32_t W, float eps, const void* pf_a, size_t bytes_a, const void* pf_b, size_t bytes_b, hipStream_t s);
static thread_local bool t_ln_prefetch = false;
static bool weights_outlive_cache(const mq_encoder_cfg* c, int Wa) {
    const double per_layer = ((double)4 * Wa * c->width + (double)(c->mlp_glu ? 3 : 2) * c->width * c->mlp_dim) * 2.0;
    return per_layer * c->layers >= 128.0 * 1024 * 1024;
}
static inline const void* pf(const void* w) { return t_ln_prefetch ? w : nullptr; }
int mq_layernorm_fp8_pf(const void* d_x, int x_bf16, const float* d_g, const float* d_b, void* d_out_fp8, float* d_row_scale, float* d_out_f32,
                        int64_t rows, int32_t W, float eps, const void* pf_a, size_t bytes_a, const void* pf_b, size_t bytes_b, hipStream_t s);
bool mq_gemm_small_grouped_ok(int64_t M, int64_t N, int64_t K);
int mq_gemm_small(const void* d_A, int64_t lda, const void* d_W, int64_t ldw, const float* d_bias, const void* d_residual, void* d_out, int64_t ldc, int64_t M,
                  int64_t N, int64_t K, int flags, hipStream_t s);
static inline int act_epi(int act) { return act == MQ_ACT_QUICKGELU ? MQ_EPI_QUICKGELU : act == MQ_ACT_RELU ? MQ_EPI_RELU : MQ_EPI_GELU; }
extern "C" int mq_gemm_bf16_ln(const void* d_A, int64_t lda, const void* d_W, int64_t ldw, const float* d_bias, const float* d_colsum,
                               const float* d_rowstats, void* d_out, int64_t ldc, int64_t M, int64_t N, int64_t K, int flags, void* stream);
extern "C" int mq_gemm_bf16_rs(const void* d_A, int64_t lda, const void* d_W, int64_t ldw, const float* d_bias, const void* d_residual, void* d_out,
                               int64_t ldc, int64_t M, int64_t N, int64_t K, int flags, float* d_partials, void* stream);
extern "C" int mq_gemm_bf16_rsf(const void* d_A, int64_t lda, const void* d_W, int64_t ldw, const float* d_bias, const void* d_residual, void* d_out,
                                int64_t ldc, int64_t M, int64_t N, int64_t K, int flags, float* d_partials, float* d_stats, float eps,
                                uint32_t* d_band_ctr, const void* d_pf_a, size_t pf_a_bytes, const void* d_pf_b, size_t pf_b_bytes, void* stream);
extern "C" int64_t mq_gemm_band_counters(int64_t M);
bool mq_gemm_rs_in_launch();
int mq_row_stats_finalize_pf(const float* d_partials, int32_t nslots, float* d_stats, int64_t rows, int32_t W, float eps, const void* pf_a, size_t bytes_a,
                             const void* pf_b, size_t bytes_b, hipStream_t s);
bool mq_row_stats_ok(int32_t W);
int mq_row_stats_pf(const void* d_x_bf16, float* d_stats, int64_t rows, int32_t W, float eps, const void* pf_a, size_t bytes_a, const void* pf_b,
                    size_t bytes_b, hipStream_t s);
static bool fold_ok(int xb, const void* wf, const float* bf, const float* sf, int64_t rows, int N, int K) {
    return mq_tower_ln_fold && xb && wf && bf && sf && mq_row_stats_ok(K) && !mq_gemm_small_ok(rows, N, K, false) && !mq_gemm_small_grouped_ok(rows, N, K);
}
static int ln_gemm(const void* d_x, int xb, const float* g, const float* b, float eps, void* h, const void* W, const float* bias, void* out,
                   int64_t rows, int N, int K, int flags, hipStream_t s, const void* next_w = nullptr, size_t next_bytes = 0,
                   const void* wf = nullptr, const float* bf = nullptr, const float* sf = nullptr, float* row_stats = nullptr,
                   bool stats_ready = false ) {
    if (mq_gemm_small_ok(rows, N, K, true)) return mq_ln_gemm_small(d_x, K, xb, g, b, eps, W, K, bias, out, N, rows, N, K, flags, nullptr, nullptr, s);
    if (row_stats && fold_ok(xb, wf, bf, sf, rows, N, K)) {
        if (!stats_ready) MQ_TRY(mq_row_stats_pf(d_x, row_stats, rows, K, eps, pf(wf), (size_t)N * K * 2, pf(next_w), next_bytes, s));
        return mq_gemm_bf16_ln(d_x, K, wf, K, bf, sf, row_stats, out, N, rows, N, K, flags, s);
    }
    MQ_TRY(mq_layernorm_pf(d_x, xb, nullptr, g, b, h, nullptr, rows, K, eps, pf(W), (size_t)N * K * 2, pf(next_w), next_bytes, s));
    if ((flags & MQ_EPI_RELU) && (mq_gemm_small_ok(rows, N, K, false) || mq_gemm_small_grouped_ok(rows, N, K)))
        return mq_gemm_small(h, K, W, K, bias, nullptr, out, N, rows, N, K, flags, s);
    return mq_gemm_bf16(h, K, W, K, bias, nullptr, out, N, rows, N, K, flags, s);
}
static int ln_gemm_panel(bool& taken, const void* d_x, int xb, float eps, void* out, int64_t rows, int64_t nseq, int32_t fixed_len, const int32_t* d_cu_seqlens, int N, int K,
                         int flags, hipStream_t s, const void* next_w, size_t next_bytes, const void* wf, const float* bf, const float* sf, float* row_stats, bool stats_ready) {
    taken = false;
    if (!(row_stats && xb && !d_cu_seqlens && fixed_len > 0 && rows == nseq * fixed_len && panel_fill_ok(nseq) && fold_ok(xb, wf, bf, sf, rows, N, K) &&
          mq_panel_gemm_ln_ok(nseq, fixed_len, N, K)))
        return MQ_OK;
    if (!stats_ready) MQ_TRY(mq_row_stats_pf(d_x, row_stats, rows, K, eps, pf(wf), (size_t)N * K * 2, pf(next_w), next_bytes, s));
    MQ_TRY(mq_panel_gemm_ln(d_x, wf, bf, sf, row_stats, out, N, nseq, fixed_len, N, K, flags, s));
    taken = true;
    return MQ_OK;
}
static bool stream_bf16(const mq_encoder_cfg* c) {
    const bool want = c->residual_stream == 1 || (c->residual_stream == 0 && mq_tower_residual_bf16 && c->precision == MQ_PREC_BF16);
    return want && (c->precision == MQ_PREC_BF16 || c->precision == MQ_PREC_FP8) && !c->post_ln && !c->d_rope_inv_freq;
}
static bool eva_form(const mq_encoder_cfg* c) { return !c->post_ln && (c->mlp_glu || c->d_rope_table); }

static bool stream_post16(const mq_encoder_cfg* c) {
    return c->residual_stream == 1 && c->post_ln && c->precision == MQ_PREC_BF16 && !c->mlp_glu && !c->d_rope_inv_freq;
}

namespace {
inline int attn_bf16(const mq_encoder_cfg* cfg, const void* qf, void* a, const int32_t* d_cu_seqlens, int64_t nseq, int32_t fixed_len,
                     int32_t max_len, int32_t Wa, hipStream_t s) {
    if (cfg->d_rel_bias) return mq_attention_bias(qf, a, d_cu_seqlens, nseq, fixed_len, max_len, Wa, cfg->heads, cfg->d_rel_bias, cfg->rel_span, s);
    return mq_attention(qf, a, d_cu_seqlens, nseq, fixed_len, max_len, Wa, cfg->heads, cfg->mask, s);
}
}

namespace {

constexpr size_t WS_ALIGN = 256;

struct Off {
    size_t off = 0;
    size_t take(size_t bytes) {
        off = align_up(off, WS_ALIGN);
        const size_t o = off;
        off += bytes;
        return o;
    }
    size_t end() const { return align_up(off, WS_ALIGN); }
};

int check_encoder_cfg(const mq_encoder_cfg* c) {
    MQ_CHECK_ARG(c, "encoder cfg is null");
    MQ_CHECK_ARG(c->width >= 64 && c->width % 64 == 0, "encoder width %d must be a multiple of 64", c->width);
    const int wa = c->attn_width ? c->attn_width : c->width;
    MQ_CHECK_ARG(c->heads >= 1 && (wa == c->heads * 64 || wa == c->heads * 96 || wa == c->heads * 112 || wa == c->heads * 128),
                 "encoder attention width must be heads * {64, 96, 112, 128} (attention width %d, heads %d)", wa, c->heads);
    MQ_CHECK_ARG(c->mlp_dim >= 64 && c->mlp_dim % 64 == 0, "encoder mlp_dim %d must be a multiple of 64", c->mlp_dim);
    MQ_CHECK_ARG(c->layers >= 0, "encoder layers < 0");
    MQ_CHECK_ARG(c->act == MQ_ACT_GELU || c->act == MQ_ACT_QUICKGELU || (c->act == MQ_ACT_SILU && c->mlp_glu) || c->act == MQ_ACT_RELU,
                 "encoder act %d unsupported (MQ_ACT_SILU: gated MLPs only)", c->act);
    if (c->act == MQ_ACT_RELU)
        MQ_CHECK_ARG(c->precision == MQ_PREC_BF16 && !c->post_ln && !c->mlp_glu && !c->d_rope_inv_freq && !c->d_rope_table,
                     "MQ_ACT_RELU: plain pre-LN encoders on bf16 operands only (no fp8, no gated MLP, no rotary positions)");
    MQ_CHECK_ARG(c->mlp_glu >= 0 && c->mlp_glu <= 2 && (c->mlp_glu != 2 || (!c->post_ln && c->act == MQ_ACT_SILU && c->mlp_dim % 16 == 0)),
                 "mlp_glu = 2 (fc1 rows interleaved for MQ_EPI_GLU): pre-LN blocks with MQ_ACT_SILU and mlp_dim %% 16 == 0");
    MQ_CHECK_ARG(c->precision == MQ_PREC_BF16 || c->precision == MQ_PREC_FP8, "encoder precision %d unsupported", c->precision);
    if (c->precision == MQ_PREC_FP8) {
        MQ_CHECK_ARG(c->width % 128 == 0 && c->mlp_dim % 128 == 0 && wa % 128 == 0, "fp8 path needs width / mlp_dim multiples of 128");
        MQ_CHECK_ARG(c->d_fp8_act_scale, "fp8 path needs d_fp8_act_scale");
        MQ_CHECK_ARG(c->fp8_first_layer >= 0, "fp8_first_layer < 0");
        MQ_CHECK_ARG(c->fp8_mlp_extra >= 0 && c->fp8_mlp_extra <= c->fp8_first_layer && (c->fp8_mlp_extra == 0 || !c->post_ln),
                     "fp8_mlp_extra = %d must lie in [0, fp8_first_layer = %d] (pre-LN encoders only)", c->fp8_mlp_extra, c->fp8_first_layer);
        MQ_CHECK_ARG(!c->mlp_glu && !c->d_rope_inv_freq && !c->d_rope_table, "the gated-MLP / rotary encoder variants run on the bf16 path only");
    }
    if (c->d_rope_inv_freq)
        MQ_CHECK_ARG(c->post_ln == 1, "d_rope_inv_freq: the rotary positions of the post-LN NewModel family (EVA02 towers: d_rope_table)");
    if (c->mlp_glu || c->d_rope_inv_freq || c->d_rope_table)
        MQ_CHECK_ARG(wa == c->width, "the gated-MLP / rotary encoder variants run un-padded heads");
    if (c->d_rope_table)
        MQ_CHECK_ARG(!c->post_ln && !c->d_rel_bias && c->rope_prefix >= 0 && c->mask == MQ_MASK_NONE, "d_rope_table: pre-LN, unmasked, fixed-length sequences (the EVA02 vision towers)");
    MQ_CHECK_ARG(c->mlp_ln_dim >= 0 && c->mlp_ln_dim <= c->mlp_dim, "mlp_ln_dim %d must lie in [0, mlp_dim = %d]", c->mlp_ln_dim, c->mlp_dim);
    if (c->d_rel_bias)
        MQ_CHECK_ARG(c->precision == MQ_PREC_BF16 && c->mask == MQ_MASK_NONE && wa == c->width && wa == c->heads * 64 && c->rel_span >= 1,
                     "the relative-position attention bias (MPNet) runs on the bf16 path with un-padded 64-wide heads and no mask");
    return MQ_OK;
}

int attn_width(const mq_encoder_cfg* c) { return c->attn_width ? c->attn_width : c->width; }

constexpr int64_t SMALL_LN_ROWS = 32;

size_t part_slots(const mq_encoder_cfg* c) {
    size_t n = (size_t)(c->width + 63) / 64;
    if (c->mlp_glu == 2) {
        const size_t g = (size_t)(2 * c->mlp_dim + 63) / 64, hd = (size_t)c->heads;
        n = n > g ? n : g;
        n = n > hd ? n : hd;
    }
    return n;
}

size_t encoder_ws(const mq_encoder_cfg* c, int64_t rows) {
    Off cv;
    const int wa = attn_width(c);
    const int fcols = c->mlp_glu ? 2 * c->mlp_dim : c->mlp_dim;
    const size_t big = (size_t)(3 * wa > fcols ? 3 * wa : fcols);
    cv.take((size_t)rows * c->width * 2);
    cv.take((size_t)rows * wa * 2);
    cv.take((size_t)rows * big * 2);
    cv.take((size_t)rows * 4);
    cv.take((size_t)rows * 8);
    cv.take((size_t)rows * part_slots(c) * 8);
    cv.take((size_t)(rows < SMALL_LN_ROWS ? rows : SMALL_LN_ROWS) * c->width * 4);
    cv.take((size_t)mq_gemm_band_counters(rows) * 4);
    return cv.end();
}

int ceil64(int v) { return (v + 63) / 64 * 64; }

}

extern "C" size_t mq_encoder_workspace_bytes(const mq_encoder_cfg* cfg, int64_t rows, int64_t nseq) {
    (void)nseq;
    if (!cfg || rows <= 0) return 0;
    return encoder_ws(cfg, rows);
}

namespace {

int last_block_selected(const mq_encoder_cfg* cfg, const mq_block_weights& b, int l, float* d_x, int64_t rows,
                        const int32_t* d_cu_seqlens, int64_t nseq, int32_t fixed_len, int32_t max_len,
                        const int32_t* d_sel, int64_t nsel, void* h, void* a, void* qf, float* row_scale, float* row_stats, bool stats_ready, float* x_sel,
                        bool f8, hipStream_t s) {
    const int W = cfg->width, F = cfg->mlp_dim, Wa = attn_width(cfg);
    const int act_flag = act_epi(cfg->act);
    const int res_flags = MQ_EPI_BIAS | MQ_EPI_RESIDUAL | MQ_EPI_OUT_F32;
    if (f8) {
        const float* s_attn = cfg->d_fp8_act_scale + 2 * l;
        const float* s_mlp = s_attn + 1;
        const int act8 = act_flag | MQ_EPI_BIAS | MQ_EPI_OUT_FP8;
        const int xb = stream_bf16(cfg) ? 1 : 0;
        const int rflags = xb ? (MQ_EPI_BIAS | MQ_EPI_RESIDUAL) : res_flags;
        MQ_TRY(mq_layernorm_fp8_pf(d_x, xb, b.ln1_g, b.ln1_b, h, row_scale, nullptr, rows, W, cfg->ln_eps, pf(b.qkv_w8), (size_t)3 * Wa * W, nullptr, 0, s));
        MQ_TRY(mq_gemm_fp8(h, W, b.qkv_w8, W, row_scale, 1, b.qkv_ws, b.qkv_b, nullptr, qf, 3 * Wa, nullptr, nullptr, rows, 3 * Wa, W,
                           MQ_EPI_BIAS, s));
        MQ_TRY(mq_attention_ex(qf, a, d_cu_seqlens, nseq, fixed_len, max_len, Wa, cfg->heads, cfg->mask, 1, s_attn, nullptr, s));
        MQ_TRY(mq_move_rows(a, d_sel, h, nsel, (int64_t)Wa, false, s));
        MQ_TRY(mq_move_rows(d_x, d_sel, x_sel, nsel, (int64_t)W * (xb ? 2 : 4), false, s));
        MQ_TRY(mq_gemm_fp8(h, Wa, b.out_w8, Wa, s_attn, 0, b.out_ws, b.out_b, x_sel, x_sel, W, nullptr, nullptr, nsel, W, Wa, rflags, s));
        MQ_TRY(mq_layernorm_fp8_ex(x_sel, xb, b.ln2_g, b.ln2_b, a, row_scale, nullptr, nsel, W, cfg->ln_eps, s));
        MQ_TRY(mq_gemm_fp8(a, W, b.fc1_w8, W, row_scale, 1, b.fc1_ws, b.fc1_b, nullptr, qf, F, s_mlp, nullptr, nsel, F, W, act8, s));
        MQ_TRY(mq_gemm_fp8(qf, F, b.fc2_w8, F, s_mlp, 0, b.fc2_ws, b.fc2_b, x_sel, x_sel, W, nullptr, nullptr, nsel, W, F, rflags, s));
    } else if (!cfg->post_ln) {
        const int xb = stream_bf16(cfg) ? 1 : 0;
        const int rflags = xb ? (MQ_EPI_BIAS | MQ_EPI_RESIDUAL) : res_flags;
        const int64_t xrow = (int64_t)W * (xb ? 2 : 4);
        MQ_TRY(ln_gemm(d_x, xb, b.ln1_g, b.ln1_b, cfg->ln_eps, h, b.qkv_w, b.qkv_b, qf, rows, 3 * Wa, W, MQ_EPI_BIAS, s, nullptr, 0, b.qkv_wf, b.qkv_bf, b.qkv_sf, row_stats, stats_ready));
        MQ_TRY(attn_bf16(cfg, qf, a, d_cu_seqlens, nseq, fixed_len, max_len, Wa, s));
        MQ_TRY(mq_move_rows(a, d_sel, h, nsel, (int64_t)Wa * 2, false, s));
        MQ_TRY(mq_move_rows(d_x, d_sel, x_sel, nsel, xrow, false, s));
        MQ_TRY(mq_gemm_bf16(h, Wa, b.out_w, Wa, b.out_b, x_sel, x_sel, W, nsel, W, Wa, rflags, s));
        MQ_TRY(ln_gemm(x_sel, xb, b.ln2_g, b.ln2_b, cfg->ln_eps, a, b.fc1_w, b.fc1_b, qf, nsel, F, W, MQ_EPI_BIAS | act_flag, s));
        MQ_TRY(mq_gemm_bf16(qf, F, b.fc2_w, F, b.fc2_b, x_sel, x_sel, W, nsel, W, F, rflags, s));
    } else if (stream_post16(cfg)) {
        const int rflags = MQ_EPI_BIAS | MQ_EPI_RESIDUAL;
        void* h_sel = x_sel;
        float* out_sel = (float*)a;
        MQ_TRY(mq_gemm_bf16(h, W, b.qkv_w, W, b.qkv_b, nullptr, qf, 3 * Wa, rows, 3 * Wa, W, MQ_EPI_BIAS, s));
        MQ_TRY(attn_bf16(cfg, qf, a, d_cu_seqlens, nseq, fixed_len, max_len, Wa, s));
        MQ_TRY(mq_move_rows(a, d_sel, qf, nsel, (int64_t)Wa * 2, false, s));
        MQ_TRY(mq_move_rows(h, d_sel, h_sel, nsel, (int64_t)W * 2, false, s));
        MQ_TRY(mq_gemm_bf16(qf, Wa, b.out_w, Wa, b.out_b, (const float*)h_sel, h_sel, W, nsel, W, Wa, rflags, s));
        MQ_TRY(mq_layernorm_ex(h_sel, 1, nullptr, b.ln1_g, b.ln1_b, h_sel, nullptr, nsel, W, cfg->ln_eps, s));
        MQ_TRY(mq_gemm_bf16(h_sel, W, b.fc1_w, W, b.fc1_b, nullptr, qf, F, nsel, F, W, MQ_EPI_BIAS | act_flag, s));
        MQ_TRY(mq_gemm_bf16(qf, F, b.fc2_w, F, b.fc2_b, (const float*)h_sel, h_sel, W, nsel, W, F, rflags, s));
        MQ_TRY(mq_layernorm_ex(h_sel, 1, nullptr, b.ln2_g, b.ln2_b, nullptr, out_sel, nsel, W, cfg->ln_eps, s));
        MQ_TRY(mq_move_rows(d_x, d_sel, out_sel, nsel, (int64_t)W * 4, true, s));
        return MQ_OK;
    } else {
        MQ_TRY(mq_gemm_bf16(h, W, b.qkv_w, W, b.qkv_b, nullptr, qf, 3 * Wa, rows, 3 * Wa, W, MQ_EPI_BIAS, s));
        MQ_TRY(attn_bf16(cfg, qf, a, d_cu_seqlens, nseq, fixed_len, max_len, Wa, s));
        MQ_TRY(mq_move_rows(a, d_sel, h, nsel, (int64_t)Wa * 2, false, s));
        MQ_TRY(mq_move_rows(d_x, d_sel, x_sel, nsel, (int64_t)W * 4, false, s));
        MQ_TRY(mq_gemm_bf16(h, Wa, b.out_w, Wa, b.out_b, x_sel, x_sel, W, nsel, W, Wa, res_flags, s));
        MQ_TRY(mq_layernorm(x_sel, nullptr, b.ln1_g, b.ln1_b, a, x_sel, nsel, W, cfg->ln_eps, s));
        MQ_TRY(mq_gemm_bf16(a, W, b.fc1_w, W, b.fc1_b, nullptr, qf, F, nsel, F, W, MQ_EPI_BIAS | act_flag, s));
        MQ_TRY(mq_gemm_bf16(qf, F, b.fc2_w, F, b.fc2_b, x_sel, x_sel, W, nsel, W, F, res_flags, s));
        MQ_TRY(mq_layernorm(x_sel, nullptr, b.ln2_g, b.ln2_b, nullptr, x_sel, nsel, W, cfg->ln_eps, s));
    }
    MQ_TRY(mq_move_rows(d_x, d_sel, x_sel, nsel, (int64_t)W * (stream_bf16(cfg) ? 2 : 4), true, s));
    return MQ_OK;
}

struct EncoderPass {
    const mq_encoder_cfg* cfg;
    const mq_block_weights* blocks;
    float* d_x;
    int64_t rows;
    const int32_t* d_cu_seqlens;
    int64_t nseq;
    int32_t fixed_len, max_len;
    const int32_t* d_sel;
    int64_t nsel;
    hipStream_t s;
    int W, F, Wa;
    void *h, *a, *qf;
    float *row_scale, *row_stats, *row_part, *xn;
    uint32_t* band_ctr;
    bool x_has_partials;
    int act_flag, res_flags, first8;

    int block_fp8(const mq_block_weights& b, int l);
    int block_eva(const mq_block_weights& b, int l);
    int block_pre_ln(const mq_block_weights& b, int l);
    int block_post_ln_small(const mq_block_weights& b, int l);
    int block_post_ln_bf16(const mq_block_weights& b, int l);
    int block_post_ln(const mq_block_weights& b, int l);
};

int EncoderPass::block_fp8(const mq_block_weights& b, int l) {
    const float* s_attn = cfg->d_fp8_act_scale + 2 * l;
    const float* s_mlp = s_attn + 1;
    float* m_attn = cfg->d_fp8_act_amax ? cfg->d_fp8_act_amax + 2 * l : nullptr;
    float* m_mlp = m_attn ? m_attn + 1 : nullptr;
    const int act8 = (cfg->act == MQ_ACT_QUICKGELU ? MQ_EPI_QUICKGELU : MQ_EPI_GELU) | MQ_EPI_BIAS | MQ_EPI_OUT_FP8;
    if (cfg->post_ln) {
        MQ_TRY(mq_gemm_fp8(h, W, b.qkv_w8, W, row_scale, 1, b.qkv_ws, b.qkv_b, nullptr, qf, 3 * Wa, nullptr, nullptr, rows, 3 * Wa, W,
                           MQ_EPI_BIAS, s));
        MQ_TRY(mq_attention_ex(qf, a, d_cu_seqlens, nseq, fixed_len, max_len, Wa, cfg->heads, cfg->mask, 1, s_attn, m_attn, s));
        MQ_TRY(mq_gemm_fp8(a, Wa, b.out_w8, Wa, s_attn, 0, b.out_ws, b.out_b, d_x, d_x, W, nullptr, nullptr, rows, W, Wa, res_flags, s));
        MQ_TRY(mq_layernorm_fp8(d_x, b.ln1_g, b.ln1_b, h, row_scale, d_x, rows, W, cfg->ln_eps, s));
        MQ_TRY(mq_gemm_fp8(h, W, b.fc1_w8, W, row_scale, 1, b.fc1_ws, b.fc1_b, nullptr, qf, F, s_mlp, m_mlp, rows, F, W, act8, s));
        MQ_TRY(mq_gemm_fp8(qf, F, b.fc2_w8, F, s_mlp, 0, b.fc2_ws, b.fc2_b, d_x, d_x, W, nullptr, nullptr, rows, W, F, res_flags, s));
        MQ_TRY(mq_layernorm_fp8(d_x, b.ln2_g, b.ln2_b, h, row_scale, d_x, rows, W, cfg->ln_eps, s));
        return MQ_OK;
    }
    const int xb = stream_bf16(cfg) ? 1 : 0;
    const int rflags = xb ? (MQ_EPI_BIAS | MQ_EPI_RESIDUAL) : res_flags;
    MQ_TRY(mq_layernorm_fp8_pf(d_x, xb, b.ln1_g, b.ln1_b, h, row_scale, nullptr, rows, W, cfg->ln_eps, pf(b.qkv_w8), (size_t)3 * Wa * W,
                               pf(b.out_w8), (size_t)W * Wa, s));
    MQ_TRY(mq_gemm_fp8(h, W, b.qkv_w8, W, row_scale, 1, b.qkv_ws, b.qkv_b, nullptr, qf, 3 * Wa, nullptr, nullptr, rows, 3 * Wa, W,
                       MQ_EPI_BIAS, s));
    MQ_TRY(mq_attention_ex(qf, a, d_cu_seqlens, nseq, fixed_len, max_len, Wa, cfg->heads, cfg->mask, 1, s_attn, m_attn, s));
    MQ_TRY(mq_gemm_fp8(a, Wa, b.out_w8, Wa, s_attn, 0, b.out_ws, b.out_b, d_x, d_x, W, nullptr, nullptr, rows, W, Wa, rflags, s));
    MQ_TRY(mq_layernorm_fp8_pf(d_x, xb, b.ln2_g, b.ln2_b, h, row_scale, nullptr, rows, W, cfg->ln_eps, pf(b.fc1_w8), (size_t)F * W,
                               pf(b.fc2_w8), (size_t)W * F, s));
    MQ_TRY(mq_gemm_fp8(h, W, b.fc1_w8, W, row_scale, 1, b.fc1_ws, b.fc1_b, nullptr, qf, F, s_mlp, m_mlp, rows, F, W, act8, s));
    MQ_TRY(mq_gemm_fp8(qf, F, b.fc2_w8, F, s_mlp, 0, b.fc2_ws, b.fc2_b, d_x, d_x, W, nullptr, nullptr, rows, W, F, rflags, s));
    return MQ_OK;
}

int EncoderPass::block_eva(const mq_block_weights& b, int l) {
    MQ_CHECK_ARG(!cfg->d_rope_table || (fixed_len > 0 && !d_cu_seqlens && rows == nseq * fixed_len && fixed_len > cfg->rope_prefix),
                 "mq_encoder_forward: d_rope_table needs fixed-length sequences longer than rope_prefix");
    MQ_CHECK_ARG(!b.attn_ln_g == !b.attn_ln_b && !b.mlp_ln_g == !b.mlp_ln_b && (!b.mlp_ln_g || cfg->mlp_glu), "mq_encoder_forward: layer %d: sub-LayerNorm weights must come in pairs (mlp_ln: gated MLPs only)", l);
    const int xb = stream_bf16(cfg) ? 1 : 0;
    const int rflags = xb ? (MQ_EPI_BIAS | MQ_EPI_RESIDUAL) : res_flags;
    const int fc1_cols = cfg->mlp_glu ? 2 * F : F;
    const bool sub_fold = mq_tower_subln_fold && mq_tower_ln_fold >= 2 && xb;
    const bool fold_attn_ln = sub_fold && b.attn_ln_g && b.out_wf && b.out_sf && b.out_bf && !cfg->d_rel_bias && !mq_gemm_small_ok(rows, W, Wa, false) &&
                              !mq_gemm_small_grouped_ok(rows, W, Wa);
    const void* out_w_run = fold_attn_ln ? b.out_wf : b.out_w;
    MQ_TRY(ln_gemm(d_x, xb, b.ln1_g, b.ln1_b, cfg->ln_eps, h, b.qkv_w, b.qkv_b, qf, rows, 3 * Wa, W, MQ_EPI_BIAS, s, out_w_run, (size_t)W * Wa * 2,
                   b.qkv_wf, b.qkv_bf, b.qkv_sf, row_stats, x_has_partials));
    x_has_partials = false;
    if (cfg->d_rope_table) MQ_TRY(mq_rope_table(qf, rows, fixed_len, cfg->rope_prefix, Wa, cfg->heads, cfg->d_rope_table, s));
    const bool fold_mlp = mq_tower_ln_fold >= 2 && fold_ok(xb, b.fc1_wf, b.fc1_bf, b.fc1_sf, rows, fc1_cols, W) && !mq_gemm_small_ok(rows, W, Wa, false) &&
                          !mq_gemm_small_grouped_ok(rows, W, Wa);
    if (fold_attn_ln) {
        MQ_TRY(mq_attention_stats(qf, a, d_cu_seqlens, nseq, fixed_len, max_len, Wa, cfg->heads, cfg->mask, row_part, rows, s));
        MQ_TRY(mq_row_stats_finalize_pf(row_part, cfg->heads, row_stats, rows, Wa, cfg->ln_eps, nullptr, 0, nullptr, 0, s));
        MQ_TRY(mq_gemm_bf16_lnrs(a, Wa, b.out_wf, Wa, b.out_bf, b.out_sf, row_stats, d_x, d_x, W, rows, W, Wa, rflags, row_part, s));
        if (fold_mlp) MQ_TRY(mq_row_stats_finalize_pf(row_part, (W + 63) / 64, row_stats, rows, W, cfg->ln_eps, pf(b.fc1_wf), (size_t)fc1_cols * W * 2, pf(b.fc2_w), (size_t)W * F * 2, s));
    } else {
        MQ_TRY(attn_bf16(cfg, qf, a, d_cu_seqlens, nseq, fixed_len, max_len, Wa, s));
        if (b.attn_ln_g) MQ_TRY(mq_layernorm_ex(a, 1, nullptr, b.attn_ln_g, b.attn_ln_b, a, nullptr, rows, Wa, cfg->ln_eps, s));
        if (fold_mlp) MQ_TRY(mq_gemm_bf16_rsf(a, Wa, b.out_w, Wa, b.out_b, d_x, d_x, W, rows, W, Wa, rflags, row_part, row_stats, cfg->ln_eps, band_ctr, pf(b.fc1_wf),
                                              (size_t)fc1_cols * W * 2, pf(b.fc2_w), (size_t)W * F * 2, s));
        else MQ_TRY(mq_gemm_bf16(a, Wa, b.out_w, Wa, b.out_b, (const float*)d_x, d_x, W, rows, W, Wa, rflags, s));
    }
    const bool il = cfg->mlp_glu == 2;
    const bool glu_epi = il && !mq_gemm_small_ok(rows, fc1_cols, W, true) && !mq_gemm_small_ok(rows, fc1_cols, W, false) && !mq_gemm_small_grouped_ok(rows, fc1_cols, W);
    const mq_block_weights* nbk = l + 1 < cfg->layers ? &blocks[l + 1] : nullptr;
    const bool fold_next = mq_tower_ln_fold >= 2 && nbk && fold_ok(xb, nbk->qkv_wf, nbk->qkv_bf, nbk->qkv_sf, rows, 3 * Wa, W) && !mq_gemm_small_ok(rows, W, F, false) &&
                           !mq_gemm_small_grouped_ok(rows, W, F);
    const bool fold_mlp_ln = sub_fold && fold_mlp && glu_epi && b.mlp_ln_g && b.fc2_wf && b.fc2_sf && b.fc2_bf && !mq_gemm_small_ok(rows, W, F, false) &&
                             !mq_gemm_small_grouped_ok(rows, W, F);
    if (fold_mlp_ln) {
        const int Fln = cfg->mlp_ln_dim ? cfg->mlp_ln_dim : F;
        MQ_TRY(mq_gemm_bf16_lnrs(d_x, W, b.fc1_wf, W, b.fc1_bf, b.fc1_sf, row_stats, nullptr, qf, fc1_cols, rows, fc1_cols, W, MQ_EPI_BIAS | MQ_EPI_GLU, row_part, s));
        MQ_TRY(mq_row_stats_finalize_pf(row_part, (fc1_cols + 63) / 64, row_stats, rows, Fln, cfg->ln_eps, pf(b.fc2_wf), (size_t)W * F * 2, nullptr, 0, s));
        MQ_TRY(mq_gemm_bf16_lnrs(qf, fc1_cols, b.fc2_wf, F, b.fc2_bf, b.fc2_sf, row_stats, d_x, d_x, W, rows, W, F, rflags, row_part, s));
        if (fold_next) MQ_TRY(mq_row_stats_finalize_pf(row_part, (W + 63) / 64, row_stats, rows, W, cfg->ln_eps, pf(nbk->qkv_wf), (size_t)3 * Wa * W * 2, pf(nbk->out_w),
                                                       (size_t)W * Wa * 2, s));
        x_has_partials = fold_next;
        return MQ_OK;
    }
    MQ_TRY(ln_gemm(d_x, xb, b.ln2_g, b.ln2_b, cfg->ln_eps, h, b.fc1_w, b.fc1_b, qf, rows, fc1_cols, W, MQ_EPI_BIAS | (cfg->mlp_glu ? (glu_epi ? MQ_EPI_GLU : 0) : act_flag), s,
                   b.fc2_w, (size_t)W * F * 2, b.fc1_wf, b.fc1_bf, b.fc1_sf, row_stats, fold_mlp));
    if (cfg->mlp_glu) {
        const int mode = glu_epi ? 2 : il ? 1 : 0;
        if (b.mlp_ln_g) MQ_TRY(mq_glu_ln(qf, rows, F, cfg->mlp_ln_dim ? cfg->mlp_ln_dim : F, cfg->act, b.mlp_ln_g, b.mlp_ln_b, cfg->ln_eps, mode, s));
        else if (!glu_epi) MQ_TRY(mq_glu(qf, rows, F, cfg->act, il ? 1 : 0, s));
    }
    if (fold_next) MQ_TRY(mq_gemm_bf16_rsf(qf, fc1_cols, b.fc2_w, F, b.fc2_b, d_x, d_x, W, rows, W, F, rflags, row_part, row_stats, cfg->ln_eps, band_ctr, pf(nbk->qkv_wf),
                                           (size_t)3 * Wa * W * 2, pf(nbk->out_w), (size_t)W * Wa * 2, s));
    else MQ_TRY(mq_gemm_bf16(qf, fc1_cols, b.fc2_w, F, b.fc2_b, (const float*)d_x, d_x, W, rows, W, F, rflags, s));
    x_has_partials = fold_next;
    return MQ_OK;
}

int EncoderPass::block_pre_ln(const mq_block_weights& b, int l) {
    const int xb = stream_bf16(cfg) ? 1 : 0;
    const int rflags = xb ? (MQ_EPI_BIAS | MQ_EPI_RESIDUAL) : res_flags;
    bool panel = false;
    MQ_TRY(ln_gemm_panel(panel, d_x, xb, cfg->ln_eps, qf, rows, nseq, fixed_len, d_cu_seqlens, 3 * Wa, W, MQ_EPI_BIAS, s, b.out_w, (size_t)W * Wa * 2, b.qkv_wf, b.qkv_bf,
                         b.qkv_sf, row_stats, x_has_partials));
    if (!panel)
        MQ_TRY(ln_gemm(d_x, xb, b.ln1_g, b.ln1_b, cfg->ln_eps, h, b.qkv_w, b.qkv_b, qf, rows, 3 * Wa, W, MQ_EPI_BIAS, s, b.out_w, (size_t)W * Wa * 2,
                       b.qkv_wf, b.qkv_bf, b.qkv_sf, row_stats, x_has_partials));
    x_has_partials = false;
    const bool last_pooled = d_sel && nsel > 0 && l == cfg->layers - 1;
    const bool mlp_fp8 = cfg->precision == MQ_PREC_FP8 && l >= first8 - cfg->fp8_mlp_extra;
    const bool fold_mlp = mq_tower_ln_fold >= 2 && !last_pooled && !mlp_fp8 && fold_ok(xb, b.fc1_wf, b.fc1_bf, b.fc1_sf, rows, F, W) &&
                          !mq_gemm_small_ok(rows, W, Wa, false) && !mq_gemm_small_grouped_ok(rows, W, Wa);
    if (mq_tower_attn_proj && fold_mlp && xb && !d_cu_seqlens && fixed_len > 0 && rows == nseq * fixed_len && Wa == W && cfg->mask == MQ_MASK_NONE && !cfg->d_rel_bias &&
        attn_proj_fill_ok(nseq) && mq_attention_proj_ok(nseq, fixed_len, W, cfg->heads)) {
        MQ_TRY(mq_attention_proj(qf, b.out_w, b.out_b, d_x, row_stats, nseq, fixed_len, W, cfg->heads, cfg->ln_eps, pf(b.fc1_wf), (size_t)F * W * 2, pf(b.fc2_w), (size_t)W * F * 2, s));
    } else {
    MQ_TRY(attn_bf16(cfg, qf, a, d_cu_seqlens, nseq, fixed_len, max_len, Wa, s));
    if (fold_mlp) MQ_TRY(mq_gemm_bf16_rsf(a, Wa, b.out_w, Wa, b.out_b, d_x, d_x, W, rows, W, Wa, rflags, row_part, row_stats, cfg->ln_eps, band_ctr, pf(b.fc1_wf),
                                          (size_t)F * W * 2, pf(b.fc2_w), (size_t)W * F * 2, s));
    else MQ_TRY(mq_gemm_bf16(a, Wa, b.out_w, Wa, b.out_b, (const float*)d_x, d_x, W, rows, W, Wa, rflags, s));
    }
    if (mlp_fp8) {
        MQ_CHECK_ARG(b.fc1_w8 && b.fc1_ws && b.fc2_w8 && b.fc2_ws, "mq_encoder_forward: layer %d has no fp8 MLP weights", l);
        const float* s_mlp = cfg->d_fp8_act_scale + 2 * l + 1;
        float* m_mlp = cfg->d_fp8_act_amax ? cfg->d_fp8_act_amax + 2 * l + 1 : nullptr;
        const int act8 = (cfg->act == MQ_ACT_QUICKGELU ? MQ_EPI_QUICKGELU : MQ_EPI_GELU) | MQ_EPI_BIAS | MQ_EPI_OUT_FP8;
        MQ_TRY(mq_layernorm_fp8_pf(d_x, xb, b.ln2_g, b.ln2_b, h, row_scale, nullptr, rows, W, cfg->ln_eps, pf(b.fc1_w8), (size_t)F * W,
                                   pf(b.fc2_w8), (size_t)W * F, s));
        MQ_TRY(mq_gemm_fp8(h, W, b.fc1_w8, W, row_scale, 1, b.fc1_ws, b.fc1_b, nullptr, qf, F, s_mlp, m_mlp, rows, F, W, act8, s));
        MQ_TRY(mq_gemm_fp8(qf, F, b.fc2_w8, F, s_mlp, 0, b.fc2_ws, b.fc2_b, (const float*)d_x, d_x, W, nullptr, nullptr, rows, W, F, rflags, s));
        return MQ_OK;
    }
    panel = false;
    if (!last_pooled && !(act_flag & MQ_EPI_RELU))
        MQ_TRY(ln_gemm_panel(panel, d_x, xb, cfg->ln_eps, qf, rows, nseq, fixed_len, d_cu_seqlens, F, W, MQ_EPI_BIAS | act_flag, s, b.fc2_w, (size_t)W * F * 2, b.fc1_wf, b.fc1_bf,
                             b.fc1_sf, row_stats, fold_mlp));
    if (!panel)
        MQ_TRY(ln_gemm(d_x, xb, b.ln2_g, b.ln2_b, cfg->ln_eps, h, b.fc1_w, b.fc1_b, qf, rows, F, W, MQ_EPI_BIAS | act_flag, s, b.fc2_w, (size_t)W * F * 2,
                       last_pooled ? nullptr : b.fc1_wf, b.fc1_bf, b.fc1_sf, row_stats, fold_mlp));
    const mq_block_weights* nbk = l + 1 < cfg->layers && l + 1 < first8 ? &blocks[l + 1] : nullptr;
    const bool fold_next = mq_tower_ln_fold >= 2 && nbk && fold_ok(xb, nbk->qkv_wf, nbk->qkv_bf, nbk->qkv_sf, rows, 3 * Wa, W) && !mq_gemm_small_ok(rows, W, F, false) &&
                           !mq_gemm_small_grouped_ok(rows, W, F);
    if (fold_next) MQ_TRY(mq_gemm_bf16_rsf(qf, F, b.fc2_w, F, b.fc2_b, d_x, d_x, W, rows, W, F, rflags, row_part, row_stats, cfg->ln_eps, band_ctr, pf(nbk->qkv_wf),
                                           (size_t)3 * Wa * W * 2, pf(nbk->out_w), (size_t)W * Wa * 2, s));
    else MQ_TRY(mq_gemm_bf16(qf, F, b.fc2_w, F, b.fc2_b, (const float*)d_x, d_x, W, rows, W, F, rflags, s));
    x_has_partials = fold_next;
    return MQ_OK;
}

int EncoderPass::block_post_ln_small(const mq_block_weights& b, int l) {
    const float* res = d_x;
    if (l == 0) MQ_TRY(mq_gemm_bf16(h, W, b.qkv_w, W, b.qkv_b, nullptr, qf, 3 * Wa, rows, 3 * Wa, W, MQ_EPI_BIAS, s));
    else {
        const mq_block_weights& pb = blocks[l - 1];
        MQ_TRY(mq_ln_gemm_small(d_x, W, 0, pb.ln2_g, pb.ln2_b, cfg->ln_eps, b.qkv_w, W, b.qkv_b, qf, 3 * Wa, rows, 3 * Wa, W, MQ_EPI_BIAS, xn, nullptr, s));
        res = xn;
    }
    MQ_TRY(attn_bf16(cfg, qf, a, d_cu_seqlens, nseq, fixed_len, max_len, Wa, s));
    MQ_TRY(mq_gemm_bf16(a, Wa, b.out_w, Wa, b.out_b, res, d_x, W, rows, W, Wa, res_flags, s));
    MQ_TRY(mq_ln_gemm_small(d_x, W, 0, b.ln1_g, b.ln1_b, cfg->ln_eps, b.fc1_w, W, b.fc1_b, qf, F, rows, F, W, MQ_EPI_BIAS | act_flag, xn, nullptr, s));
    MQ_TRY(mq_gemm_bf16(qf, F, b.fc2_w, F, b.fc2_b, xn, d_x, W, rows, W, F, res_flags, s));
    if (l == cfg->layers - 1) MQ_TRY(mq_layernorm(d_x, nullptr, b.ln2_g, b.ln2_b, h, d_x, rows, W, cfg->ln_eps, s));
    return MQ_OK;
}

int EncoderPass::block_post_ln_bf16(const mq_block_weights& b, int l) {
    const int rflags = MQ_EPI_BIAS | MQ_EPI_RESIDUAL;
    const bool last = l == cfg->layers - 1;
    MQ_TRY(mq_gemm_bf16(h, W, b.qkv_w, W, b.qkv_b, nullptr, qf, 3 * Wa, rows, 3 * Wa, W, MQ_EPI_BIAS, s));
    MQ_TRY(attn_bf16(cfg, qf, a, d_cu_seqlens, nseq, fixed_len, max_len, Wa, s));
    MQ_TRY(mq_gemm_bf16(a, Wa, b.out_w, Wa, b.out_b, (const float*)h, h, W, rows, W, Wa, rflags, s));
    MQ_TRY(mq_layernorm_pf(h, 1, nullptr, b.ln1_g, b.ln1_b, h, nullptr, rows, W, cfg->ln_eps, pf(b.fc1_w), (size_t)F * W * 2, pf(b.fc2_w),
                           (size_t)W * F * 2, s));
    MQ_TRY(mq_gemm_bf16(h, W, b.fc1_w, W, b.fc1_b, nullptr, qf, F, rows, F, W, MQ_EPI_BIAS | act_flag, s));
    MQ_TRY(mq_gemm_bf16(qf, F, b.fc2_w, F, b.fc2_b, (const float*)h, h, W, rows, W, F, rflags, s));
    const mq_block_weights* nb = !last ? &blocks[l + 1] : nullptr;
    MQ_TRY(mq_layernorm_pf(h, 1, nullptr, b.ln2_g, b.ln2_b, last ? nullptr : h, last ? d_x : nullptr, rows, W, cfg->ln_eps,
                           pf(nb ? nb->qkv_w : nullptr), (size_t)3 * Wa * W * 2, pf(nb ? nb->out_w : nullptr), (size_t)W * Wa * 2, s));
    return MQ_OK;
}

int EncoderPass::block_post_ln(const mq_block_weights& b, int l) {
    MQ_TRY(mq_gemm_bf16(h, W, b.qkv_w, W, b.qkv_b, nullptr, qf, 3 * Wa, rows, 3 * Wa, W, MQ_EPI_BIAS, s));
    if (cfg->d_rope_inv_freq) MQ_TRY(mq_rope(qf, d_cu_seqlens, nseq, fixed_len, Wa, cfg->heads, cfg->d_rope_inv_freq, s));
    MQ_TRY(attn_bf16(cfg, qf, a, d_cu_seqlens, nseq, fixed_len, max_len, Wa, s));
    MQ_TRY(mq_gemm_bf16(a, Wa, b.out_w, Wa, b.out_b, d_x, d_x, W, rows, W, Wa, res_flags, s));
    MQ_TRY(mq_layernorm_pf(d_x, 0, nullptr, b.ln1_g, b.ln1_b, h, d_x, rows, W, cfg->ln_eps, pf(b.fc1_w), (size_t)(cfg->mlp_glu ? 2 : 1) * F * W * 2,
                           pf(b.fc2_w), (size_t)W * F * 2, s));
    if (cfg->mlp_glu) {
        MQ_TRY(mq_gemm_bf16(h, W, b.fc1_w, W, b.fc1_b, nullptr, qf, 2 * F, rows, 2 * F, W, b.fc1_b ? MQ_EPI_BIAS : 0, s));
        MQ_TRY(mq_glu(qf, rows, F, cfg->act, 0, s));
        MQ_TRY(mq_gemm_bf16(qf, 2 * F, b.fc2_w, F, b.fc2_b, d_x, d_x, W, rows, W, F, res_flags, s));
    } else {
        MQ_TRY(mq_gemm_bf16(h, W, b.fc1_w, W, b.fc1_b, nullptr, qf, F, rows, F, W, MQ_EPI_BIAS | act_flag, s));
        MQ_TRY(mq_gemm_bf16(qf, F, b.fc2_w, F, b.fc2_b, d_x, d_x, W, rows, W, F, res_flags, s));
    }
    const mq_block_weights* nb = l + 1 < cfg->layers && l + 1 < first8 ? &blocks[l + 1] : nullptr;
    MQ_TRY(mq_layernorm_pf(d_x, 0, nullptr, b.ln2_g, b.ln2_b, h, d_x, rows, W, cfg->ln_eps, pf(nb ? nb->qkv_w : nullptr), (size_t)3 * Wa * W * 2,
                           pf(nb ? nb->out_w : nullptr), (size_t)W * Wa * 2, s));
    return MQ_OK;
}

int encoder_forward_impl(const mq_encoder_cfg* cfg, const mq_block_weights* blocks, float* d_x, int64_t rows,
                         const int32_t* d_cu_seqlens, int64_t nseq, int32_t fixed_len, int32_t max_len,
                         const int32_t* d_sel, int64_t nsel, void* d_workspace, size_t workspace_bytes, hipStream_t s) {
    MQ_TRY(check_encoder_cfg(cfg));
    MQ_CHECK_ARG(d_x && (blocks || cfg->layers == 0), "mq_encoder_forward: null pointer");
    if (rows <= 0 || cfg->layers == 0) return MQ_OK;
    if (workspace_bytes < encoder_ws(cfg, rows)) {
        mq_set_error("mq_encoder_forward: workspace %zu < required %zu", workspace_bytes, encoder_ws(cfg, rows));
        return MQ_ERR_WORKSPACE;
    }
    const int W = cfg->width, F = cfg->mlp_dim, Wa = attn_width(cfg);
    const int fcols = cfg->mlp_glu ? 2 * F : F;
    const size_t big = (size_t)(3 * Wa > fcols ? 3 * Wa : fcols);
    Off cv;
    char* wsb = (char*)d_workspace;
    void* h = wsb + cv.take((size_t)rows * W * 2);
    void* a = wsb + cv.take((size_t)rows * Wa * 2);
    void* qf = wsb + cv.take((size_t)rows * big * 2);
    float* row_scale = (float*)(wsb + cv.take((size_t)rows * 4));
    float* row_stats = (float*)(wsb + cv.take((size_t)rows * 8));
    float* row_part = (float*)(wsb + cv.take((size_t)rows * part_slots(cfg) * 8));
    float* xn = (float*)(wsb + cv.take((size_t)(rows < SMALL_LN_ROWS ? rows : SMALL_LN_ROWS) * W * 4));
    uint32_t* band_ctr = (uint32_t*)(wsb + cv.take((size_t)mq_gemm_band_counters(rows) * 4));
    if (stream_bf16(cfg) && mq_gemm_rs_in_launch()) MQ_CHECK_HIP(hipMemsetAsync(band_ctr, 0, (size_t)mq_gemm_band_counters(rows) * 4, s));
    else band_ctr = nullptr;

    const size_t xsel_off = align_up((size_t)(nsel > 0 ? nsel : 0) * F * 2, WS_ALIGN);
    const bool select_last = d_sel && nsel > 0 && nsel * 2 <= rows && mq_tower_row_select && !cfg->mlp_glu && !cfg->d_rope_inv_freq && !cfg->d_rope_table &&
                             !mq_gemm_small_ok(rows, W, W, false) &&
                             !(cfg->precision == MQ_PREC_FP8 && (cfg->d_fp8_act_amax || cfg->post_ln)) &&
                             xsel_off + (size_t)nsel * W * 4 <= (size_t)rows * big * 2;

    t_ln_prefetch = weights_outlive_cache(cfg, Wa);
    const int first8 = cfg->precision == MQ_PREC_FP8 ? (cfg->fp8_first_layer < cfg->layers ? cfg->fp8_first_layer : cfg->layers) : cfg->layers;

    const bool small_post_ln = cfg->post_ln && first8 >= cfg->layers && !cfg->mlp_glu && !cfg->d_rope_inv_freq && rows <= SMALL_LN_ROWS &&
                               mq_gemm_small_ok(rows, 3 * Wa, W, true) && mq_gemm_small_ok(rows, F, W, true) && mq_gemm_small_ok(rows, W, F, false);
    const bool post16 = stream_post16(cfg) && !small_post_ln && !mq_gemm_small_ok(rows, W, W, false);
    if (cfg->post_ln && first8 == 0) MQ_TRY(mq_rowquant_fp8(d_x, h, row_scale, rows, W, s));
    else if (cfg->post_ln) MQ_TRY(mq_cast_bf16(d_x, h, rows * W, s));

    EncoderPass p{cfg, blocks, d_x, rows, d_cu_seqlens, nseq, fixed_len, max_len, d_sel, nsel, s, W, F, Wa, h, a, qf, row_scale, row_stats, row_part, xn, band_ctr,
                   false, act_epi(cfg->act), MQ_EPI_BIAS | MQ_EPI_RESIDUAL | MQ_EPI_OUT_F32, first8};
    for (int l = 0; l < cfg->layers; ++l) {
        const mq_block_weights& b = blocks[l];
        const bool f8 = l >= first8;
        MQ_CHECK_ARG(b.qkv_w && b.out_w && b.fc1_w && b.fc2_w && b.ln1_g && b.ln2_g, "mq_encoder_forward: layer %d has null weights", l);
        if (f8)
            MQ_CHECK_ARG(b.qkv_w8 && b.qkv_ws && b.out_w8 && b.out_ws && b.fc1_w8 && b.fc1_ws && b.fc2_w8 && b.fc2_ws,
                         "mq_encoder_forward: layer %d has no fp8 weights", l);
        if (cfg->post_ln && f8 && l == first8 && l > 0) MQ_TRY(mq_rowquant_fp8(d_x, h, row_scale, rows, W, s));
        if (select_last && l == cfg->layers - 1) {
            MQ_TRY(last_block_selected(cfg, b, l, d_x, rows, d_cu_seqlens, nseq, fixed_len, max_len, d_sel, nsel, h, a, qf, row_scale, row_stats, p.x_has_partials,
                                       (float*)((char*)qf + xsel_off), f8, s));
            break;
        }
        if (f8) MQ_TRY(p.block_fp8(b, l));
        else if (eva_form(cfg)) MQ_TRY(p.block_eva(b, l));
        else if (!cfg->post_ln) MQ_TRY(p.block_pre_ln(b, l));
        else if (small_post_ln) MQ_TRY(p.block_post_ln_small(b, l));
        else if (post16) MQ_TRY(p.block_post_ln_bf16(b, l));
        else MQ_TRY(p.block_post_ln(b, l));
    }
    return MQ_OK;
}
}

extern "C" int mq_encoder_forward(const mq_encoder_cfg* cfg, const mq_block_weights* blocks, float* d_x, int64_t rows,
                                  const int32_t* d_cu_seqlens, int64_t nseq, int32_t fixed_len, int32_t max_len,
                                  void* d_workspace, size_t workspace_bytes, void* stream) {
    return encoder_forward_impl(cfg, blocks, d_x, rows, d_cu_seqlens, nseq, fixed_len, max_len, nullptr, 0, d_workspace, workspace_bytes,
                                (hipStream_t)stream);
}

extern "C" int mq_encoder_forward_rows(const mq_encoder_cfg* cfg, const mq_block_weights* blocks, float* d_x, int64_t rows,
                                       const int32_t* d_cu_seqlens, int64_t nseq, int32_t fixed_len, int32_t max_len,
                                       const int32_t* d_out_rows, int64_t n_out_rows, void* d_workspace, size_t workspace_bytes,
                                       void* stream) {
    MQ_CHECK_ARG(d_out_rows && n_out_rows > 0, "mq_encoder_forward_rows: empty row selection");
    return encoder_forward_impl(cfg, blocks, d_x, rows, d_cu_seqlens, nseq, fixed_len, max_len, d_out_rows, n_out_rows, d_workspace,
                                workspace_bytes, (hipStream_t)stream);
}

namespace {
struct VitPlan {
    int T, np, Kp; int64_t rows;
    size_t off_x, off_rows, off_cls, off_enc, off_patches, off_patch_out, total;
    size_t off_map_y, off_map_z, off_map_h, off_tok, off_kv;
};
VitPlan vit_plan(const mq_vit_cfg* c, int64_t n) {
    VitPlan p;
    const int G = c->image_size / c->patch_size;
    const bool map = c->pool == MQ_VIT_POOL_MAP || c->pool == MQ_VIT_POOL_QUERY;
    p.np = G * G; p.T = p.np + (c->pool == MQ_VIT_POOL_MAP ? 0 : 1); p.Kp = ceil64(3 * c->patch_size * c->patch_size); p.rows = n * p.T;
    const int W = c->enc.width;
    Off cv;
    p.off_x = cv.take((size_t)p.rows * W * 4);
    p.off_rows = cv.take((size_t)n * 4);
    p.off_cls = cv.take((size_t)n * W * 2);
    p.off_map_y = p.off_map_z = p.off_map_h = p.off_tok = p.off_kv = 0;
    if (map) {
        p.off_map_y = cv.take((size_t)n * W * 4);
        p.off_map_z = cv.take((size_t)n * W * 2);
        p.off_map_h = cv.take((size_t)n * c->map_mlp_dim * 2);
    }
    p.off_enc = cv.end();
    size_t enc = encoder_ws(&c->enc, p.rows);
    if (map) {
        Off mv;
        p.off_tok = p.off_enc + mv.take((size_t)p.rows * W * 2);
        p.off_kv = p.off_enc + mv.take((size_t)p.rows * 2 * W * 2);
        if (mv.end() > enc) enc = mv.end();
    }
    Off pv;
    p.off_patches = p.off_enc + pv.take((size_t)n * p.np * p.Kp * 2);
    p.off_patch_out = p.off_enc + pv.take((size_t)n * p.np * W * 4);
    const size_t patches = pv.end();
    p.total = p.off_enc + (enc > patches ? enc : patches);
    return p;
}

int encode_image_impl(const mq_vit_cfg* cfg, const mq_vit_weights* w, const void* d_pixels, bool is_u8, int64_t n,
                      float* d_out, int normalize, void* ws, size_t ws_bytes, hipStream_t s) {
    MQ_CHECK_ARG(cfg && w && d_out, "mq_encode_image: null pointer");
    MQ_TRY(check_encoder_cfg(&cfg->enc));
    MQ_CHECK_ARG(cfg->patch_size > 0 && cfg->image_size >= cfg->patch_size, "mq_encode_image: image %d smaller than patch %d",
                 cfg->image_size, cfg->patch_size);
    MQ_CHECK_ARG(cfg->out_dim >= 4 && cfg->out_dim % 4 == 0, "mq_encode_image: out_dim %d must be a multiple of 4", cfg->out_dim);
    const bool map = cfg->pool == MQ_VIT_POOL_MAP;
    const bool avg = cfg->pool == MQ_VIT_POOL_AVG;
    const bool qpool = cfg->pool == MQ_VIT_POOL_QUERY;
    MQ_CHECK_ARG(cfg->pool == MQ_VIT_POOL_CLS || map || avg || qpool, "mq_encode_image: bad pool %d", cfg->pool);
    MQ_CHECK_ARG(w->patch_w && w->pos && w->ln_post_g && w->ln_post_b, "mq_encode_image: null weight pointer");
    const int W = cfg->enc.width;
    if (map) {
        const mq_map_head* m = w->map;
        MQ_CHECK_ARG(m && m->q && m->kv_w && m->kv_b && m->proj_w && m->proj_b && m->ln_g && m->ln_b && m->fc1_w && m->fc1_b && m->fc2_w && m->fc2_b,
                     "mq_encode_image: MQ_VIT_POOL_MAP needs the attention-pool head's weights");
        MQ_CHECK_ARG(!w->cls && !w->ln_pre_g && !w->ln_pre_b, "mq_encode_image: MQ_VIT_POOL_MAP has no class token / ln_pre");
        MQ_CHECK_ARG(cfg->map_mlp_dim >= 64 && cfg->map_mlp_dim % 64 == 0, "mq_encode_image: map_mlp_dim %d must be a multiple of 64", cfg->map_mlp_dim);
        MQ_CHECK_ARG(w->proj_w || cfg->out_dim == W, "mq_encode_image: without a projection out_dim (%d) must equal the width (%d)", cfg->out_dim, W);
    } else {
        MQ_CHECK_ARG(w->cls && w->proj_w && (avg || eva_form(&cfg->enc) || (w->ln_pre_g && w->ln_pre_b)) && (!w->ln_pre_g == !w->ln_pre_b),
                     "mq_encode_image: null weight pointer (ln_pre may be absent only with MQ_VIT_POOL_AVG and in the EVA02 form)");
        MQ_CHECK_ARG(!w->proj_b || cfg->pool == MQ_VIT_POOL_CLS, "mq_encode_image: proj_b goes with MQ_VIT_POOL_CLS");
    }
    if (qpool) {
        const mq_map_head* m = w->map;
        MQ_CHECK_ARG(m && m->q && m->kv_w && m->kv_b && m->proj_w && m->proj_b && m->ln_g && m->ln_b, "mq_encode_image: MQ_VIT_POOL_QUERY needs the pooler's weights");
        MQ_CHECK_ARG(cfg->pool_dim >= 64 && cfg->pool_dim % 64 == 0 && cfg->pool_dim <= W && cfg->pool_heads >= 1 && cfg->pool_dim % cfg->pool_heads == 0,
                     "mq_encode_image: pool_dim %d / pool_heads %d unsupported (pool_dim a multiple of 64, <= the width %d)", cfg->pool_dim, cfg->pool_heads, W);
    }
    if (n <= 0) return MQ_OK;
    MQ_CHECK_ARG(d_pixels && ws, "mq_encode_image: null input / workspace");
    const VitPlan p = vit_plan(cfg, n);
    if (ws_bytes < p.total) { mq_set_error("mq_encode_image: workspace %zu < required %zu", ws_bytes, p.total); return MQ_ERR_WORKSPACE; }
    char* base = (char*)ws;
    float* x = (float*)(base + p.off_x);
    int32_t* rows_idx = (int32_t*)(base + p.off_rows);
    void* cls_ln = base + p.off_cls;
    void* patches = base + p.off_patches;
    float* patch_out = (float*)(base + p.off_patch_out);

    MQ_TRY(mq_patchify(d_pixels, is_u8, patches, n, cfg->image_size, cfg->patch_size, p.Kp, cfg->mean, cfg->std, s));
    MQ_TRY(mq_gemm_bf16(patches, p.Kp, w->patch_w, p.Kp, nullptr, nullptr, patch_out, W, n * p.np, W, p.Kp, MQ_EPI_OUT_F32, s));
    const int xb = stream_bf16(&cfg->enc) ? 1 : 0;
    MQ_TRY(mq_vit_assemble(patch_out, w->cls, w->pos, w->ln_pre_g, w->ln_pre_b, x, n, p.T, W, cfg->enc.ln_eps, xb, s));
    if (map) {
        const mq_map_head* m = w->map;
        const int F = cfg->map_mlp_dim;
        MQ_TRY(encoder_forward_impl(&cfg->enc, w->blocks, x, p.rows, nullptr, n, p.T, p.T, nullptr, 0, base + p.off_enc,
                                    ws_bytes - p.off_enc, s));
        void* tok = base + p.off_tok;
        void* kv = base + p.off_kv;
        float* y = (float*)(base + p.off_map_y);
        void* z = base + p.off_map_z;
        void* hmid = base + p.off_map_h;
        MQ_TRY(mq_layernorm_ex(x, xb, nullptr, w->ln_post_g, w->ln_post_b, tok, nullptr, p.rows, W, cfg->enc.ln_eps, s));
        MQ_TRY(mq_gemm_bf16(tok, W, m->kv_w, W, m->kv_b, nullptr, kv, 2 * W, p.rows, 2 * W, W, MQ_EPI_BIAS, s));
        MQ_TRY(mq_map_pool(kv, m->q, cls_ln, n, p.T, W, cfg->enc.heads, s));
        MQ_CHECK_HIP(hipMemsetAsync(y, 0, (size_t)n * W * 4, s));
        MQ_TRY(mq_gemm_bf16(cls_ln, W, m->proj_w, W, m->proj_b, y, y, W, n, W, W, MQ_EPI_BIAS | MQ_EPI_RESIDUAL | MQ_EPI_OUT_F32, s));
        MQ_TRY(mq_layernorm(y, nullptr, m->ln_g, m->ln_b, z, nullptr, n, W, cfg->enc.ln_eps, s));
        MQ_TRY(mq_gemm_bf16(z, W, m->fc1_w, W, m->fc1_b, nullptr, hmid, F, n, F, W, MQ_EPI_BIAS | MQ_EPI_GELU, s));
        MQ_TRY(mq_gemm_bf16(hmid, F, m->fc2_w, F, m->fc2_b, y, y, W, n, W, F, MQ_EPI_BIAS | MQ_EPI_RESIDUAL | MQ_EPI_OUT_F32, s));
        if (w->proj_w) {
            MQ_TRY(mq_cast_bf16(y, z, (int64_t)n * W, s));
            MQ_TRY(mq_gemm_bf16(z, W, w->proj_w, W, nullptr, nullptr, d_out, cfg->out_dim, n, cfg->out_dim, W, MQ_EPI_OUT_F32, s));
            if (normalize) MQ_TRY(mq_l2_normalize(d_out, d_out, n, cfg->out_dim, s));
        } else if (normalize) {
            MQ_TRY(mq_l2_normalize(y, d_out, n, W, s));
        } else {
            MQ_CHECK_HIP(hipMemcpyAsync(d_out, y, (size_t)n * W * 4, hipMemcpyDeviceToDevice, s));
        }
        return MQ_OK;
    }
    if (qpool) {
        const mq_map_head* m = w->map;
        const int Dp = cfg->pool_dim;
        MQ_TRY(encoder_forward_impl(&cfg->enc, w->blocks, x, p.rows, nullptr, n, p.T, p.T, nullptr, 0, base + p.off_enc, ws_bytes - p.off_enc, s));
        void* tok = base + p.off_tok;
        void* kv = base + p.off_kv;
        float* y = (float*)(base + p.off_map_y);
        void* z = base + p.off_map_z;
        MQ_TRY(mq_layernorm_ex(x, xb, nullptr, w->ln_post_g, w->ln_post_b, tok, nullptr, p.rows, W, cfg->enc.ln_eps, s));
        MQ_TRY(mq_gemm_bf16(tok, W, m->kv_w, W, m->kv_b, nullptr, kv, 2 * Dp, p.rows, 2 * Dp, W, MQ_EPI_BIAS, s));
        MQ_TRY(mq_map_pool(kv, m->q, cls_ln, n, p.T, Dp, cfg->pool_heads, s));
        MQ_CHECK_HIP(hipMemsetAsync(y, 0, (size_t)n * Dp * 4, s));
        MQ_TRY(mq_gemm_bf16(cls_ln, Dp, m->proj_w, Dp, m->proj_b, y, y, Dp, n, Dp, Dp, MQ_EPI_BIAS | MQ_EPI_RESIDUAL | MQ_EPI_OUT_F32, s));
        MQ_TRY(mq_layernorm(y, nullptr, m->ln_g, m->ln_b, z, nullptr, n, Dp, cfg->enc.ln_eps, s));
        MQ_TRY(mq_gemm_bf16(z, Dp, w->proj_w, Dp, nullptr, nullptr, d_out, cfg->out_dim, n, cfg->out_dim, Dp, MQ_EPI_OUT_F32, s));
        if (normalize) MQ_TRY(mq_l2_normalize(d_out, d_out, n, cfg->out_dim, s));
        return MQ_OK;
    }
    if (avg) {
        MQ_TRY(encoder_forward_impl(&cfg->enc, w->blocks, x, p.rows, nullptr, n, p.T, p.T, nullptr, 0, base + p.off_enc, ws_bytes - p.off_enc, s));
        float* pooled = (float*)(base + p.off_enc);
        MQ_TRY(mq_avg_tokens(x, xb, pooled, n, p.T, 1, W, s));
        MQ_TRY(mq_layernorm(pooled, nullptr, w->ln_post_g, w->ln_post_b, cls_ln, nullptr, n, W, cfg->enc.ln_eps, s));
        MQ_TRY(mq_gemm_bf16(cls_ln, W, w->proj_w, W, nullptr, nullptr, d_out, cfg->out_dim, n, cfg->out_dim, W, MQ_EPI_OUT_F32, s));
        if (normalize) MQ_TRY(mq_l2_normalize(d_out, d_out, n, cfg->out_dim, s));
        return MQ_OK;
    }
    MQ_TRY(mq_cls_rows(rows_idx, n, p.T, s));
    MQ_TRY(encoder_forward_impl(&cfg->enc, w->blocks, x, p.rows, nullptr, n, p.T, p.T, rows_idx, n, base + p.off_enc,
                                ws_bytes - p.off_enc, s));
    if (mq_gemm_small_ok(n, cfg->out_dim, W, true))
        MQ_TRY(mq_ln_gemm_small(x, W, xb, w->ln_post_g, w->ln_post_b, cfg->enc.ln_eps, w->proj_w, W, w->proj_b, d_out, cfg->out_dim, n, cfg->out_dim,
                                W, MQ_EPI_OUT_F32 | (w->proj_b ? MQ_EPI_BIAS : 0), nullptr, rows_idx, s));
    else {
        MQ_TRY(mq_layernorm_ex(x, xb, rows_idx, w->ln_post_g, w->ln_post_b, cls_ln, nullptr, n, W, cfg->enc.ln_eps, s));
        MQ_TRY(mq_gemm_bf16(cls_ln, W, w->proj_w, W, w->proj_b, nullptr, d_out, cfg->out_dim, n, cfg->out_dim, W, MQ_EPI_OUT_F32 | (w->proj_b ? MQ_EPI_BIAS : 0), s));
    }
    if (normalize) MQ_TRY(mq_l2_normalize(d_out, d_out, n, cfg->out_dim, s));
    return MQ_OK;
}
}

extern "C" size_t mq_vit_workspace_bytes(const mq_vit_cfg* cfg, int64_t n_images) {
    if (!cfg || n_images <= 0 || cfg->patch_size <= 0) return 0;
    return vit_plan(cfg, n_images).total;
}

extern "C" int mq_encode_image_u8(const mq_vit_cfg* cfg, const mq_vit_weights* w, const uint8_t* d_pixels, int64_t n,
                                  float* d_out, int normalize, void* d_workspace, size_t workspace_bytes, void* stream) {
    return encode_image_impl(cfg, w, d_pixels, true, n, d_out, normalize, d_workspace, workspace_bytes, (hipStream_t)stream);
}

extern "C" int mq_encode_image_f32(const mq_vit_cfg* cfg, const mq_vit_weights* w, const float* d_pixels, int64_t n,
                                   float* d_out, int normalize, void* d_workspace, size_t workspace_bytes, void* stream) {
    return encode_image_impl(cfg, w, d_pixels, false, n, d_out, normalize, d_workspace, workspace_bytes, (hipStream_t)stream);
}

namespace {
struct TextPlan { size_t off_x, off_rows, off_pool, off_enc, total; };
TextPlan text_plan(const mq_encoder_cfg* enc, int64_t rows, int64_t nseq) {
    TextPlan p;
    Off cv;
    p.off_x = cv.take((size_t)rows * enc->width * 4);
    p.off_rows = cv.take((size_t)nseq * 4);
    p.off_pool = cv.take((size_t)nseq * enc->width * 4);
    p.off_enc = cv.end();
    p.total = p.off_enc + encoder_ws(enc, rows);
    return p;
}
int max_seq_len(const int32_t* h_cu, int64_t nseq, int64_t* rows_out) {
    int mx = 0;
    for (int64_t i = 0; i < nseq; ++i) {
        const int l = h_cu[i + 1] - h_cu[i];
        if (l < 1) return -1;
        if (l > mx) mx = l;
    }
    *rows_out = h_cu[nseq] - h_cu[0];
    return mx;
}
}

extern "C" size_t mq_clip_text_workspace_bytes(const mq_clip_text_cfg* cfg, int64_t rows, int64_t nseq) {
    if (!cfg || rows <= 0 || nseq <= 0) return 0;
    return text_plan(&cfg->enc, rows, nseq).total;
}

extern "C" int mq_encode_clip_text(const mq_clip_text_cfg* cfg, const mq_clip_text_weights* w, const int32_t* d_ids,
                                   const int32_t* d_cu_seqlens, const int32_t* h_cu_seqlens, int64_t nseq,
                                   const int32_t* d_pool_rows, float* d_out, int normalize, void* d_workspace,
                                   size_t workspace_bytes, void* stream) {
    MQ_CHECK_ARG(cfg && w && d_out, "mq_encode_clip_text: null pointer");
    MQ_TRY(check_encoder_cfg(&cfg->enc));
    MQ_CHECK_ARG(cfg->out_dim >= 4 && cfg->out_dim % 4 == 0, "mq_encode_clip_text: out_dim %d must be a multiple of 4", cfg->out_dim);
    MQ_CHECK_ARG(w->tok_emb && w->pos && w->ln_final_g && w->ln_final_b && w->proj_w, "mq_encode_clip_text: null weight pointer");
    if (nseq <= 0) return MQ_OK;
    MQ_CHECK_ARG(d_ids && d_cu_seqlens && h_cu_seqlens && d_workspace, "mq_encode_clip_text: null input / workspace");
    MQ_CHECK_ARG(h_cu_seqlens[0] == 0, "mq_encode_clip_text: cu_seqlens[0] must be 0");
    int64_t rows = 0;
    const int maxl = max_seq_len(h_cu_seqlens, nseq, &rows);
    MQ_CHECK_ARG(maxl >= 1 && maxl <= cfg->ctx + (cfg->cls_pos > 0 ? 1 : 0), "mq_encode_clip_text: sequence lengths must be in [1, ctx=%d]", cfg->ctx);
    MQ_CHECK_ARG(cfg->cls_pos >= 0 && cfg->cls_pos < cfg->ctx, "mq_encode_clip_text: cls_pos %d outside the position table [0, %d)", cfg->cls_pos, cfg->ctx);
    const TextPlan p = text_plan(&cfg->enc, rows, nseq);
    if (workspace_bytes < p.total) { mq_set_error("mq_encode_clip_text: workspace %zu < required %zu", workspace_bytes, p.total); return MQ_ERR_WORKSPACE; }
    hipStream_t s = (hipStream_t)stream;
    char* base = (char*)d_workspace;
    float* x = (float*)(base + p.off_x);
    int32_t* rows_idx = (int32_t*)(base + p.off_rows);
    void* pooled = base + p.off_pool;
    const int W = cfg->enc.width;

    const int xb = stream_bf16(&cfg->enc) ? 1 : 0;
    MQ_TRY(mq_embed_tokens(d_ids, d_cu_seqlens, nseq, w->tok_emb, w->pos, nullptr, nullptr, nullptr, xb ? nullptr : x, xb ? (void*)x : nullptr, W,
                           cfg->vocab, 0.f, cfg->cls_pos, s));
    const int32_t* pool_rows = d_pool_rows;
    if (!pool_rows) { MQ_TRY(mq_last_rows(d_cu_seqlens, rows_idx, nseq, s)); pool_rows = rows_idx; }
    MQ_TRY(encoder_forward_impl(&cfg->enc, w->blocks, x, rows, d_cu_seqlens, nseq, 0, maxl, pool_rows, nseq, base + p.off_enc,
                                workspace_bytes - p.off_enc, s));
    if (!w->proj_b && mq_gemm_small_ok(nseq, cfg->out_dim, W, true)) {
        MQ_TRY(mq_ln_gemm_small(x, W, xb, w->ln_final_g, w->ln_final_b, cfg->enc.ln_eps, w->proj_w, W, nullptr, d_out, cfg->out_dim, nseq,
                                cfg->out_dim, W, MQ_EPI_OUT_F32, nullptr, pool_rows, s));
        if (normalize) MQ_TRY(mq_l2_normalize(d_out, d_out, nseq, cfg->out_dim, s));
        return MQ_OK;
    }
    MQ_TRY(mq_layernorm_ex(x, xb, pool_rows, w->ln_final_g, w->ln_final_b, pooled, nullptr, nseq, W, cfg->enc.ln_eps, s));
    if (w->proj_b) {
        MQ_CHECK_HIP(hipMemsetAsync(d_out, 0, (size_t)nseq * cfg->out_dim * 4, s));
        MQ_TRY(mq_gemm_bf16(pooled, W, w->proj_w, W, w->proj_b, d_out, d_out, cfg->out_dim, nseq, cfg->out_dim, W,
                            MQ_EPI_BIAS | MQ_EPI_RESIDUAL | MQ_EPI_OUT_F32, s));
    } else
        MQ_TRY(mq_gemm_bf16(pooled, W, w->proj_w, W, nullptr, nullptr, d_out, cfg->out_dim, nseq, cfg->out_dim, W, MQ_EPI_OUT_F32, s));
    if (normalize) MQ_TRY(mq_l2_normalize(d_out, d_out, nseq, cfg->out_dim, s));
    return MQ_OK;
}

extern "C" size_t mq_bert_workspace_bytes(const mq_bert_cfg* cfg, int64_t rows, int64_t nseq) {
    if (!cfg || rows <= 0 || nseq <= 0) return 0;
    return text_plan(&cfg->enc, rows, nseq).total;
}

extern "C" int mq_encode_bert(const mq_bert_cfg* cfg, const mq_bert_weights* w, const int32_t* d_ids,
                              const int32_t* d_cu_seqlens, const int32_t* h_cu_seqlens, int64_t nseq, float* d_out,
                              int normalize, void* d_workspace, size_t workspace_bytes, void* stream) {
    MQ_CHECK_ARG(cfg && w && d_out, "mq_encode_bert: null pointer");
    MQ_TRY(check_encoder_cfg(&cfg->enc));
    MQ_CHECK_ARG(cfg->enc.post_ln == 1 && cfg->enc.mask == MQ_MASK_NONE, "mq_encode_bert: BERT is post-LN with full attention");
    MQ_CHECK_ARG(cfg->pool == MQ_POOL_MEAN || cfg->pool == MQ_POOL_CLS, "mq_encode_bert: bad pooling %d", cfg->pool);
    if (cfg->out_dim)
        MQ_CHECK_ARG(cfg->out_dim >= 4 && cfg->out_dim % 4 == 0 && w->proj1_w && w->proj1_b &&
                     (w->proj2_w ? (cfg->proj_hidden >= 64 && cfg->proj_hidden % 64 == 0 && cfg->proj_hidden <= 3 * cfg->enc.width) : cfg->proj_hidden == 0),
                     "mq_encode_bert: projection head needs out_dim %% 4 == 0, proj1_w / proj1_b, and either proj2_w with proj_hidden %% 64 == 0 "
                     "(<= 3 W: the MLP head) or neither (one biased Linear)");
    MQ_CHECK_ARG(w->word_emb && (w->pos_emb || cfg->enc.d_rope_inv_freq) && w->emb_ln_g && w->emb_ln_b, "mq_encode_bert: null weight pointer");
    if (nseq <= 0) return MQ_OK;
    MQ_CHECK_ARG(d_ids && d_cu_seqlens && h_cu_seqlens && d_workspace, "mq_encode_bert: null input / workspace");
    MQ_CHECK_ARG(h_cu_seqlens[0] == 0, "mq_encode_bert: cu_seqlens[0] must be 0");
    int64_t rows = 0;
    const int maxl = max_seq_len(h_cu_seqlens, nseq, &rows);
    MQ_CHECK_ARG(maxl >= 1 && maxl <= cfg->max_pos, "mq_encode_bert: sequence lengths must be in [1, max_pos=%d]", cfg->max_pos);
    const TextPlan p = text_plan(&cfg->enc, rows, nseq);
    if (workspace_bytes < p.total) { mq_set_error("mq_encode_bert: workspace %zu < required %zu", workspace_bytes, p.total); return MQ_ERR_WORKSPACE; }
    hipStream_t s = (hipStream_t)stream;
    char* base = (char*)d_workspace;
    float* x = (float*)(base + p.off_x);
    const int W = cfg->enc.width;

    MQ_TRY(mq_embed_tokens(d_ids, d_cu_seqlens, nseq, w->word_emb, w->pos_emb, w->type_emb, w->emb_ln_g, w->emb_ln_b, x, nullptr, W,
                           cfg->vocab, cfg->enc.ln_eps, 0, s));
    const int32_t* sel = cfg->pool == MQ_POOL_CLS ? d_cu_seqlens : nullptr;
    MQ_TRY(encoder_forward_impl(&cfg->enc, w->blocks, x, rows, d_cu_seqlens, nseq, 0, maxl, sel, sel ? nseq : 0, base + p.off_enc,
                                workspace_bytes - p.off_enc, s));
    if (!cfg->out_dim) {
        MQ_TRY(mq_pool(x, d_cu_seqlens, nseq, d_out, W, cfg->pool, normalize, s));
        return MQ_OK;
    }
    float* pooled = (float*)(base + p.off_pool);
    bf16_t* pb = (bf16_t*)(base + p.off_enc);
    bf16_t* h1 = pb + (size_t)nseq * W;
    MQ_TRY(mq_pool(x, d_cu_seqlens, nseq, pooled, W, cfg->pool, 0, s));
    MQ_TRY(mq_cast_bf16(pooled, pb, (int64_t)nseq * W, s));
    if (!w->proj2_w) {
        MQ_TRY(mq_gemm_bf16(pb, W, w->proj1_w, W, w->proj1_b, nullptr, d_out, cfg->out_dim, nseq, cfg->out_dim, W, MQ_EPI_BIAS | MQ_EPI_OUT_F32, s));
    } else {
        MQ_TRY(mq_gemm_bf16(pb, W, w->proj1_w, W, w->proj1_b, nullptr, h1, cfg->proj_hidden, nseq, cfg->proj_hidden, W, MQ_EPI_BIAS | MQ_EPI_GELU, s));
        MQ_TRY(mq_gemm_bf16(h1, cfg->proj_hidden, w->proj2_w, cfg->proj_hidden, nullptr, nullptr, d_out, cfg->out_dim, nseq, cfg->out_dim,
                            cfg->proj_hidden, MQ_EPI_OUT_F32, s));
    }
    if (normalize) MQ_TRY(mq_l2_normalize(d_out, d_out, nseq, cfg->out_dim, s));
    return MQ_OK;
// ... 2 lines not shown
```

marqo_amd/engine/towers.py:

```python
from __future__ import annotations

import ctypes as C
import logging
import os
import threading
from typing import Dict, Optional, Sequence, Tuple

import numpy as np
import torch

from marqo_amd import _lib as L
from marqo_amd.engine import native_queue as NQ
from marqo_amd.engine.archs import BertArch, ClipTextArch, VitArch, OPENAI_DATASET_MEAN, OPENAI_DATASET_STD
from marqo_amd.engine.tower_weights import (
    EVA_GLU_EPILOGUE, KERNEL_HEAD_DIMS, LN_FOLD, RESNET_BN_EPS, _OPEN_CLIP_KEYS, _TIMM_KEYS, _Holder, _bert_blocks, _ceil64, _clip_blocks,
    _eva_blocks, _head_dim, _kernel_head_dim, _need, _pad_heads, _pad_mlp, convnext_downsample_gather, convnext_downsample_weight,
    convnext_dw_taps, convnext_fold_gamma_fc2, convnext_fold_ln_fc1, fold_layernorm, nllb_clip_state_dict, patch_embed_weight, resnet_attnpool_weights,
    resnet_conv1x1_weight, resnet_conv3x3_weight, resnet_fold_bn, resnet_pad64, resnet_pad_vec, resnet_stem_weight)

Tensor = torch.Tensor
_log = logging.getLogger(__name__)

MAX_ROWS_PER_CALL = 1 << 18

# ... 258 lines not shown
        enc, layers = self.cfg.enc, self.cfg.enc.layers
        getattr(self, "_graphs", {}).clear()
        enc.fp8_first_layer, enc.fp8_mlp_extra = 0, 0
        self.calibrate_fp8(run, passes=2, margin=self.FP8_SCALE_MARGIN if margin is None else margin)
        self._fp8.calibrated = False
        enc.precision = L.MQ_PREC_BF16
        ref = run().double()
        enc.precision = L.MQ_PREC_FP8

        def err_split(first: int, extra: int = 0) -> float:
            enc.fp8_first_layer, enc.fp8_mlp_extra = first, extra
            return _max_cos_error(run().double(), ref)

        enc.residual_stream, self.residual_stream, self.residual_stream_error = 2, "fp32", None
        mode = _residual_mode()
        if not enc.post_ln and mode != "fp32":
            enc.residual_stream = 1
            e_stream = err_split(layers, 0)
            if mode == "bf16" or e_stream <= self.FP8_STREAM_SHARE * budget:
                self.residual_stream, self.residual_stream_error = "bf16", e_stream
            else:
                enc.residual_stream = 2
        e0 = err_split(0)
        self.fp8_all_blocks_error = e0
        if e0 <= budget:
            first, e = 0, e0
        else:
            lo, hi, e = 0, layers, 0.0
            while hi - lo > 1:
                mid = (lo + hi) // 2
                em = err_split(mid)
                if em <= budget:
                    hi, e = mid, em
                else:
                    lo = mid
            first = hi
        extra = 0
        self.fp8_policy_trace = [(first, 0, e)]
        if not enc.post_ln and os.environ.get("MARQO_AMD_FP8_MLP_ONLY", "1") != "0":
            best = (self._fp8_share(layers, first, 0), first, 0, e)
            step = max(1, layers // 8)
            for s_ in sorted({min(layers, first + k * step) for k in range(0, 9)} | {layers}):
                if s_ == 0:
                    continue
                lo_x, hi_x = 0, s_
                e_s = err_split(s_, 0) if s_ != first else e
                if e_s > budget:
                    continue
                e_at = {0: e_s}
                while hi_x - lo_x > 0:
                    mid = (lo_x + hi_x + 1) // 2
                    em = err_split(s_, mid)
                    e_at[mid] = em
                    if em <= budget:
                        lo_x = mid
                    else:
                        hi_x = mid - 1
                share = self._fp8_share(layers, s_, lo_x)
                self.fp8_policy_trace.append((s_, lo_x, e_at[lo_x]))
                if share > best[0] + 1e-9:
                    best = (share, s_, lo_x, e_at[lo_x])
            _, first, extra, e = best
        enc.fp8_first_layer, enc.fp8_mlp_extra = first, extra
        self.fp8_first_layer, self.fp8_mlp_extra, self.fp8_calibration_error = first, extra, e
        self._fp8.calibrated = True
        _log.info("fp8 policy: blocks [%d, %d) on e4m3 + the MLP halves of blocks [%d, %d), %s residual stream, 1 - cos vs bf16 on the calibration "
                  "batch %.2e (all blocks: %.2e, budget %.1e)", first, layers, first - extra, first, self.residual_stream, e, e0, budget)
        return first

    def release_unused_folded(self) -> int:
        blocks = getattr(self, "_blocks", None)
        if blocks is None or not hasattr(blocks[0], "qkv_wf"):
            return 0
        enc = self.cfg.enc
        layers = len(blocks)
        bf16_stream = enc.residual_stream == 1
        fp8 = self.precision == "fp8"
        first = enc.fp8_first_layer if fp8 else layers
        first_mlp = first - (enc.fp8_mlp_extra if fp8 else 0)
        freed = 0
        for i in range(layers):
            b = blocks[i]
            for name, alive in (("qkv", bf16_stream and i < first), ("fc1", bf16_stream and i < first_mlp)):
                if alive:
                    continue
                for suffix in ("_wf", "_bf", "_sf"):
                    ptr = getattr(b, name + suffix)
                    if ptr:
                        freed += self._h.drop(ptr)
                        setattr(b, name + suffix, None)
        if freed:
            getattr(self, "_graphs", {}).clear()
            for _, q in (self._queues or {}).values():
                q.close()
            if self._queues:
                self._queues = {}
        return freed

    def _calibration_run(self):
        raise NotImplementedError(f"{type(self).__name__} has no calibration batch")

    def tune_residual_default(self) -> str:
        return self.tune_residual_stream(self._calibration_run())

    def tune_fp8_default(self, budget: Optional[float] = None) -> int:
        return self.tune_fp8(self._calibration_run(), budget=budget)

    pools_one_row = False

    def _fp8_share(self, layers: int, split: int, extra: int) -> float:
        share = (layers - split) + (2.0 / 3.0) * extra
        if self.pools_one_row:
            if split < layers:
                share -= 0.75
            elif extra >= 1:
                share -= 2.0 / 3.0
        return share

    def __init__(self, device: str):
        self.device = _require_gpu(device)
        self.lib = L.load()
        self._h = _Holder(self.device)
        self._tls = threading.local()
        self._lock = threading.Lock()
        self._graphs: Dict[tuple, "_GraphedCall"] = {}
        self._graphs_off = False
        self._ops = L.load_torch_ops() if L.boundary() == "torch_ops" else None
        self._blobs = None

    _queues: Optional[Dict[bool, tuple]] = None
    _queues_off = False

    def _cached_queue(self, normalize: bool, make, what: str, *how):
        sig = bytes(self.cfg)
        ent = (self._queues or {}).get(bool(normalize))
        if ent is not None and ent[0] == sig:
            return ent[1]
        with self._lock:
            if self._queues is None:
                self._queues = {}
            ent = self._queues.get(bool(normalize))
            if ent is not None and ent[0] == sig:
                return ent[1]
            if ent is not None:
                ent[1].close()
            try:
                q = make(self.device.index if self.device.index is not None else torch.cuda.current_device(), normalize, *how)
            except (L.MarqoHipUnavailableError, L.MarqoHipError) as e:
                self._queues_off = True
                _log.warning("native request queue unavailable (%s); small %s calls keep the direct path", e, what)
                return None
            self._queues[bool(normalize)] = (sig, q)
            return q

    def _forget_queue(self, q) -> None:
        with self._lock:
            for k, ent in list((self._queues or {}).items()):
                if ent[1] is q:
                    del self._queues[k]

    def _through_queue(self, q, encode, *args):
        try:
            return encode(*args)
        except L.MarqoHipError as e:
            if NQ.gone(e):
                self._forget_queue(q)
                return None
            raise

    def queue_stats(self) -> Dict[bool, Dict[str, int]]:
        return {k: ent[1].stats() for k, ent in (self._queues or {}).items()}

    def _desc(self):
        if self._blobs is None:
            self._blobs = (L.struct_blob(self.cfg), L.struct_blob(self.w))
        return self._blobs

    def _call_image(self, kind: str, pixels: Tensor, n: int, out: Tensor, normalize: bool, ws: Tensor) -> None:
        if self._ops is not None:
            cfg, w = self._desc()
            (self._ops.encode_image_u8 if kind == "u8" else self._ops.encode_image_f32)(cfg, w, pixels, out, bool(normalize), ws)
            return
        fn = self.lib.mq_encode_image_u8 if kind == "u8" else self.lib.mq_encode_image_f32
        L.check(fn(C.byref(self.cfg), C.byref(self.w), pixels.data_ptr(), n, out.data_ptr(), 1 if normalize else 0, ws.data_ptr(),
                   ws.numel(), self._stream()), "mq_encode_image")

    def _call_text(self, clip: bool, d_packed: Tensor, d_cu: Tensor, cu: Tensor, nseq: int, d_pool: Optional[Tensor], out: Tensor,
                   normalize: bool, ws: Tensor) -> None:
        if self._ops is not None:
            cfg, w = self._desc()
            if clip:
                self._ops.encode_clip_text(cfg, w, d_packed, d_cu, cu, d_pool, out, bool(normalize), ws)
            else:
                self._ops.encode_bert(cfg, w, d_packed, d_cu, cu, out, bool(normalize), ws)
            return
        if clip:
            L.check(self.lib.mq_encode_clip_text(C.byref(self.cfg), C.byref(self.w), d_packed.data_ptr(), d_cu.data_ptr(), cu.data_ptr(), nseq,
                                                 L.ptr(d_pool), out.data_ptr(), 1 if normalize else 0, ws.data_ptr(), ws.numel(),
                                                 self._stream()), "mq_encode_clip_text")
        else:
            L.check(self.lib.mq_encode_bert(C.byref(self.cfg), C.byref(self.w), d_packed.data_ptr(), d_cu.data_ptr(), cu.data_ptr(), nseq,
                                            out.data_ptr(), 1 if normalize else 0, ws.data_ptr(), ws.numel(), self._stream()),
                    "mq_encode_bert")

    def _graphs_ok(self) -> bool:
        return GRAPHS and not self._graphs_off and (self._fp8 is None or self._fp8.calibrated)

    def _capture(self, key: tuple, make) -> Optional["_GraphedCall"]:
        g = self._graphs.get(key)
        if g is None:
            if len(self._graphs) >= MAX_GRAPHS_PER_TOWER:
                return None
            try:
                g = self._graphs[key] = make()
            except RuntimeError as e:
                self._graphs_off = True
                _log.warning("hipGraph capture failed (%s); this tower keeps launching eagerly", e)
                return None
        return g

    def _workspace(self, nbytes: int) -> Tensor:
        by_stream = getattr(self._tls, "ws", None)
        if by_stream is None:
            by_stream = self._tls.ws = {}
        key = torch.cuda.current_stream(self.device).cuda_stream
        ws = by_stream.get(key)
        if ws is None or ws.numel() < nbytes:
            if len(by_stream) >= 4:
                by_stream.clear()
            ws = by_stream[key] = torch.empty(int(nbytes * 1.25) + 256, dtype=torch.uint8, device=self.device)
        return ws

    def _stream(self) -> int:
        return torch.cuda.current_stream(self.device).cuda_stream

    def weight_bytes(self) -> int:
        return self._h.nbytes()


class _ImageTowerBase(_TowerBase):

    def _run_chunks(self, kind: str, pixels: Tensor, normalize: bool) -> Tensor:
        n = pixels.shape[0]
        out = torch.empty(n, self.arch.out_dim, dtype=torch.float32, device=self.device)
        for i in range(0, n, self.max_images_per_call):
            m = min(self.max_images_per_call, n - i)
            ws = self._workspace(self._image_workspace_bytes(m))
            self._launch_images(kind, pixels[i:i + m], m, out[i:i + m], normalize, ws)
        return out

    def _run(self, kind: str, pixels: Tensor, normalize: bool) -> Tensor:
        with torch.cuda.device(self.device):
            return self._run_chunks(kind, pixels, normalize)

    def _check_u8(self, images_u8: Tensor) -> Tensor:
        S = self.arch.image_size
        if images_u8.dtype != torch.uint8 or images_u8.ndim != 4 or tuple(images_u8.shape[1:]) != (S, S, 3):
            raise ValueError(f"expected uint8 [n, {S}, {S}, 3], got {images_u8.dtype} {tuple(images_u8.shape)}")
        return images_u8.to(self.device, non_blocking=True).contiguous()

    def encode_u8(self, images_u8: Tensor, normalize: bool = True) -> Tensor:
        return self._run("u8", self._check_u8(images_u8), normalize)

    def encode_f32(self, pixels: Tensor, normalize: bool = True) -> Tensor:
        S = self.arch.image_size
        if pixels.ndim != 4 or tuple(pixels.shape[1:]) != (3, S, S):
            raise ValueError(f"expected float [n, 3, {S}, {S}], got {tuple(pixels.shape)}")
        return self._run("f32", pixels.to(device=self.device, dtype=torch.float32, non_blocking=True).contiguous(), normalize)


class VitTower(_ImageTowerBase):

    def __init__(self, arch: VitArch, sd: Dict[str, Tensor], device: str,
                 mean: Sequence[float] = OPENAI_DATASET_MEAN, std: Sequence[float] = OPENAI_DATASET_STD,
                 precision: str = "bf16"):
        super().__init__(device)
        _check_precision(precision)
        self.precision = precision
        self.arch = arch
        W, P = arch.width, arch.patch_size
        if arch.image_size < P:
            raise ValueError("image_size must be at least one patch")
        h = self._h
        patch_w = patch_embed_weight(sd, "visual.trunk.patch_embed.proj.weight" if arch.pool == "map" or arch.eva else "visual.conv1.weight", W, P)
        if arch.pool == "map":
            t = "visual.trunk."
            F = arch.mlp_dim
            hd = _head_dim(W, arch.heads)
            if arch.out_dim != W:
                raise ValueError(f"SigLIP towers have no visual projection: out_dim {arch.out_dim} must equal the width {W}")
            pos = _need(sd, t + "pos_embed", (1, arch.tokens, W)).detach().to(torch.float32)[0] + \
                _need(sd, t + "patch_embed.proj.bias", (W,)).detach().to(torch.float32)
            self._blocks = _clip_blocks(h, sd, t, arch.layers, W, F, arch.heads, keys=_TIMM_KEYS)
            a = t + "attn_pool."
            f32 = lambda k, shape: _need(sd, a + k, shape).detach().to(torch.float32)
            q = (f32("latent", (1, 1, W)).reshape(W) @ f32("q.weight", (W, W)).t() + f32("q.bias", (W,))) * hd ** -0.5
            m1_w, m1_b, m2_w = _pad_mlp(f32("mlp.fc1.weight", (F, W)), f32("mlp.fc1.bias", (F,)), f32("mlp.fc2.weight", (W, F)))
            self._map = L.MapHead(q=h.f32(q), kv_w=h.bf16(f32("kv.weight", (2 * W, W))), kv_b=h.f32(f32("kv.bias", (2 * W,))),
                                  proj_w=h.bf16(f32("proj.weight", (W, W))), proj_b=h.f32(f32("proj.bias", (W,))),
                                  ln_g=h.f32(f32("norm.weight", (W,))), ln_b=h.f32(f32("norm.bias", (W,))),
                                  fc1_w=h.bf16(m1_w), fc1_b=h.f32(m1_b), fc2_w=h.bf16(m2_w), fc2_b=h.f32(f32("mlp.fc2.bias", (W,))))
            self.w = L.VitWeights(patch_w=h.bf16(patch_w), cls=None, pos=h.f32(pos), ln_pre_g=None, ln_pre_b=None, blocks=self._blocks,
                                  ln_post_g=h.f32(_need(sd, t + "norm.weight", (W,))), ln_post_b=h.f32(_need(sd, t + "norm.bias", (W,))),
                                  proj_w=None, map=C.pointer(self._map))
            pool, map_mlp = L.MQ_VIT_POOL_MAP, _ceil64(F)
        elif arch.pool == "query":
# ... 782 lines not shown
```

Measured before the change: 95500 embeddings/s.

## Fuse first-layer LN stats into ViT assemble and pool last block by stride

The ViT assemble kernel gains a variant that also computes per-row mean and rstd of its bf16 output and prefetches the first block's QKV and out-proj weights. Layer 0's folded LN-QKV GEMM then reuses these stats instead of running a separate row-stats pass. The last block in CLS pooling now reads pooled rows through a strided pitch (T rows apart), so the index build and row-gather copies are skipped. The final LN also takes a row multiplier. This adds template and code-path complexity and depends on many gating conditions.

```diff
diff --git a/marqo_amd/csrc/embed.hip b/marqo_amd/csrc/embed.hip
--- a/marqo_amd/csrc/embed.hip
+++ b/marqo_amd/csrc/embed.hip
@@ -101,10 +101,12 @@
 }
 
 constexpr int MAXC = 8;
-template <int CH>
+template <int CH, bool ST = false>
 __global__ __launch_bounds__(256, (CH <= 4 ? 8 : 4)) void vit_assemble_kernel(
     const float* __restrict__ patch_out, const float* __restrict__ cls, const float* __restrict__ pos,
-    const float* __restrict__ gam, const float* __restrict__ bet, float* __restrict__ x, int64_t rows, int T, int W, float eps, int x_bf16) {
+    const float* __restrict__ gam, const float* __restrict__ bet, float* __restrict__ x, int64_t rows, int T, int W, float eps, int x_bf16,
+    float2* __restrict__ stats = nullptr, const unsigned* __restrict__ pfa = nullptr, unsigned na = 0u, const unsigned* __restrict__ pfb = nullptr, unsigned nb = 0u) {
+    __shared__ __attribute__((aligned(16))) uint2 srow[ST ? 4 : 1][ST ? CH * 64 : 1];
     const int lane = threadIdx.x & 63;
     const int64_t row = (int64_t)blockIdx.x * 4 + (threadIdx.x >> 6);
     if (row >= rows) return;
@@ -114,6 +116,7 @@
             q.x = pack_bf16x2(y[0], y[1]);
             q.y = pack_bf16x2(y[2], y[3]);
             *(uint2*)((bf16_t*)x + row * W + c * 4) = q;
+            if constexpr (ST) srow[threadIdx.x >> 6][c] = q;
         } else {
             *(f32x4*)(x + row * W + c * 4) = y;
         }
@@ -149,6 +152,47 @@
             for (int e = 0; e < 4; ++e) y[e] = v[i][e] * gg[e] + bb[e];
             put(c, y);
         }
+    }
+    if constexpr (ST) {
+        unsigned pq = 0u;
+        const unsigned t = blockIdx.x * 256u + threadIdx.x;
+        if (t < na) pq = pfa[(size_t)t * 32];
+        else if (t - na < nb) pq = pfb[(size_t)(t - na) * 32];
+        __builtin_amdgcn_fence(__ATOMIC_RELEASE, "wavefront");
+        __builtin_amdgcn_wave_barrier();
+        __builtin_amdgcn_fence(__ATOMIC_ACQUIRE, "wavefront");
+        constexpr int CH8 = (CH + 1) / 2;
+        const int nch8 = W >> 3;
+        float u[CH8][8];
+#pragma unroll
+        for (int i = 0; i < CH8; ++i) {
+            const int c = lane + i * 64;
+            uint4 q = make_uint4(0u, 0u, 0u, 0u);
+            if (c < nch8) q = *(const uint4*)&srow[threadIdx.x >> 6][2 * c];
+            const unsigned w4[4] = {q.x, q.y, q.z, q.w};
+#pragma unroll
+            for (int e = 0; e < 4; ++e) { u[i][2 * e] = __uint_as_float(w4[e] << 16); u[i][2 * e + 1] = __uint_as_float(w4[e] & 0xffff0000u); }
+        }
+        float s1 = 0.f;
+#pragma unroll
+        for (int i = 0; i < CH8; ++i)
+            if (lane + i * 64 < nch8) s1 += ((u[i][0] + u[i][1]) + (u[i][2] + u[i][3])) + ((u[i][4] + u[i][5]) + (u[i][6] + u[i][7]));
+        float mean = s1;
+#pragma unroll
+        for (int o = 32; o > 0; o >>= 1) mean += __shfl_xor(mean, o, 64);
+        mean = mean / (float)W;
+        float s2 = 0.f;
+#pragma unroll
+        for (int i = 0; i < CH8; ++i)
+            if (lane + i * 64 < nch8) {
+#pragma unroll
+                for (int e = 0; e < 8; ++e) { const float d = u[i][e] - mean; s2 += d * d; }
+            }
+        float rstd = s2;
+#pragma unroll
+        for (int o = 32; o > 0; o >>= 1) rstd += __shfl_xor(rstd, o, 64);
+        if (lane == 0) stats[row] = make_float2(mean, rsqrtf(rstd / (float)W + eps));
+        asm volatile("" ::"v"(pq));
     }
 }
 
@@ -349,6 +393,23 @@
     return MQ_OK;
 }
 
+bool mq_vit_assemble_stats_ok(int32_t W) { return W % 8 == 0 && W >= 8 && W <= 64 * 4 * MAXC; }
+extern mq_knob mq_ln_prefetch;
+int mq_vit_assemble_stats(const float* d_patch_out, const float* cls, const float* pos, const float* g, const float* b, void* d_x, float* d_stats, int64_t n,
+                          int32_t T, int32_t W, float eps, const void* pf_a, size_t bytes_a, const void* pf_b, size_t bytes_b, hipStream_t s) {
+    MQ_CHECK_ARG(mq_vit_assemble_stats_ok(W) && g && b && d_stats, "vit_assemble_stats: W=%d unsupported / null pointer", W);
+    const int64_t rows = n * T;
+    if (rows <= 0) return MQ_OK;
+    MqProfScope prof(3, s);
+    const bool pf = mq_ln_prefetch && rows >= 1024;
+    auto lines = [pf](const void* p, size_t bytes) { return (pf && p && ((uintptr_t)p & 3) == 0 && bytes < ((size_t)1 << 30)) ? (unsigned)(bytes / 128) : 0u; };
+    const unsigned na = lines(pf_a, bytes_a), nb = lines(pf_b, bytes_b);
+    MQ_DISPATCH_CH(W, hipLaunchKernelGGL((vit_assemble_kernel<CH, true>), dim3((unsigned)cdiv64(rows, 4)), dim3(256), 0, s, d_patch_out,
+                                         cls, pos, g, b, (float*)d_x, rows, T, W, eps, 1, (float2*)d_stats, (const unsigned*)pf_a, na, (const unsigned*)pf_b, nb));
+    MQ_CHECK_LAUNCH("vit_assemble_stats");
+    return MQ_OK;
+}
+
 __global__ __launch_bounds__(256) void avg_tokens_kernel(const void* __restrict__ xv, int x_bf16, float* __restrict__ out, int T, int first, int W) {
     const int64_t img = blockIdx.x;
     const float inv = 1.0f / (float)(T - first);
diff --git a/marqo_amd/csrc/gemm_bf16.hip b/marqo_amd/csrc/gemm_bf16.hip
--- a/marqo_amd/csrc/gemm_bf16.hip
+++ b/marqo_amd/csrc/gemm_bf16.hip
@@ -14,6 +14,7 @@
 extern mq_knob mq_tower_panel_gemm;
 extern mq_knob mq_attention_waves;
 extern mq_knob mq_tower_residual_bf16;
+extern mq_knob mq_tower_pool_strided, mq_tower_assemble_stats;
 extern mq_knob mq_gemm_small_max_rows;
 bool mq_gemm_small_ok(int64_t M, int64_t N, int64_t K, bool ln);
 bool mq_gemm_small_grouped_ok(int64_t M, int64_t N, int64_t K);
@@ -677,6 +678,8 @@
     else if (k == "xcd_band") mq_xcd_band = value;
     else if (k == "attn_waves") mq_attention_waves = value;
     else if (k == "residual_bf16") mq_tower_residual_bf16 = value;
+    else if (k == "pool_strided") mq_tower_pool_strided = value;
+    else if (k == "assemble_stats") mq_tower_assemble_stats = value;
     else if (k == "small_m") mq_gemm_small_max_rows = value;
     else if (k == "small_m_grouped") mq_gemm_small_group_rows = value;
     else if (k == "ln_prefetch") mq_ln_prefetch = value;
diff --git a/marqo_amd/csrc/rowops.hip b/marqo_amd/csrc/rowops.hip
--- a/marqo_amd/csrc/rowops.hip
+++ b/marqo_amd/csrc/rowops.hip
@@ -5,6 +5,8 @@
 extern mq_knob mq_gemm_small_max_rows;
 int mq_layernorm_pf(const void* d_x, int x_bf16, const int32_t* d_row_idx, const float* d_g, const float* d_b, void* d_out_bf16, float* d_out_f32,
                     int64_t rows, int32_t W, float eps, const void* pf_a, size_t bytes_a, const void* pf_b, size_t bytes_b, hipStream_t s);
+int mq_layernorm_rows_pf(const void* d_x, int x_bf16, const int32_t* d_row_idx, int64_t row_mul, const float* d_g, const float* d_b, void* d_out_bf16,
+                         float* d_out_f32, int64_t rows, int32_t W, float eps, const void* pf_a, size_t bytes_a, const void* pf_b, size_t bytes_b, hipStream_t s);
 int mq_layernorm_fp8_pf(const void* d_x, int x_bf16, const float* d_g, const float* d_b, void* d_out_fp8, float* d_row_scale, float* d_out_f32,
                         int64_t rows, int32_t W, float eps, const void* pf_a, size_t bytes_a, const void* pf_b, size_t bytes_b, hipStream_t s);
 mq_knob mq_ln_bf16_wide{getenv("MQ_LN_BF16_WIDE") ? atoi(getenv("MQ_LN_BF16_WIDE")) : 1};
@@ -19,6 +21,7 @@
     const unsigned* pfa;
     const unsigned* pfb;
     unsigned step;
+    unsigned row_mul;
 };
 constexpr int LN_PF = 2;
 
@@ -53,7 +56,7 @@
 #pragma unroll
     for (int r = 0; r < R; ++r) {
         const int64_t row = row0 + r < rows ? row0 + r : rows - 1;
-        const int64_t src = row_idx ? (int64_t)row_idx[row] : row;
+        const int64_t src = row_idx ? (int64_t)row_idx[row] : row * ex.row_mul;
 #pragma unroll
         for (int i = 0; i < CH; ++i) {
             const int c = lane + i * 64;
@@ -144,7 +147,7 @@
 #pragma unroll
     for (int r = 0; r < R; ++r) {
         const int64_t row = row0 + r < rows ? row0 + r : rows - 1;
-        const int64_t src = row_idx ? (int64_t)row_idx[row] : row;
+        const int64_t src = row_idx ? (int64_t)row_idx[row] : row * ex.row_mul;
 #pragma unroll
         for (int i = 0; i < CH8; ++i) {
             const int c = lane + i * 64;
@@ -363,7 +366,7 @@
 mq_knob mq_ln_prefetch{getenv("MQ_LN_PREFETCH") ? atoi(getenv("MQ_LN_PREFETCH")) : 1};
 
 static LnExtra ln_extra(int band, int64_t rows, const void* pf_a, size_t bytes_a, const void* pf_b, size_t bytes_b) {
-    LnExtra ex{band, 0u, 0u, nullptr, nullptr, 32u};
+    LnExtra ex{band, 0u, 0u, nullptr, nullptr, 32u, 1u};
     if (mq_ln_prefetch && rows >= 1024) {
         const size_t gran = mq_ln_prefetch == 2 ? 64 : mq_ln_prefetch == 3 ? 32 : 128;
         ex.step = (unsigned)(gran / 4);
@@ -382,11 +385,18 @@
 
 int mq_layernorm_pf(const void* d_x, int x_bf16, const int32_t* d_row_idx, const float* d_g, const float* d_b, void* d_out_bf16, float* d_out_f32,
                     int64_t rows, int32_t W, float eps, const void* pf_a, size_t bytes_a, const void* pf_b, size_t bytes_b, hipStream_t s) {
+    return mq_layernorm_rows_pf(d_x, x_bf16, d_row_idx, 1, d_g, d_b, d_out_bf16, d_out_f32, rows, W, eps, pf_a, bytes_a, pf_b, bytes_b, s);
+}
+
+int mq_layernorm_rows_pf(const void* d_x, int x_bf16, const int32_t* d_row_idx, int64_t row_mul, const float* d_g, const float* d_b, void* d_out_bf16,
+                         float* d_out_f32, int64_t rows, int32_t W, float eps, const void* pf_a, size_t bytes_a, const void* pf_b, size_t bytes_b, hipStream_t s) {
     MQ_CHECK_ARG(d_x && d_g && d_b && (d_out_bf16 || d_out_f32), "mq_layernorm: null pointer");
+    MQ_CHECK_ARG(row_mul >= 1 && row_mul < ((int64_t)1 << 31) && (d_row_idx == nullptr || row_mul == 1), "mq_layernorm: bad row multiplier");
     MQ_CHECK_ARG(W >= 4 && W % 4 == 0 && W <= 64 * 4 * LN_MAX_CHUNKS, "mq_layernorm: W=%d unsupported (multiple of 4, <= 2048)", W);
     if (rows <= 0) return MQ_OK;
     MqProfScope prof(1, s);
-    const LnExtra band = ln_extra((mq_xcd_band && !d_row_idx && rows >= 4096) ? 1 : 0, rows, pf_a, bytes_a, pf_b, bytes_b);
+    LnExtra band = ln_extra((mq_xcd_band && !d_row_idx && row_mul == 1 && rows >= 4096) ? 1 : 0, rows, pf_a, bytes_a, pf_b, bytes_b);
+    band.row_mul = (unsigned)row_mul;
     if (x_bf16 && mq_ln_bf16_wide && rows > mq_gemm_small_max_rows && W % 8 == 0 && W <= 1024 && ((uintptr_t)d_x & 15) == 0 && (!d_out_bf16 || ((uintptr_t)d_out_bf16 & 15) == 0)) {
         const bf16_t* xb = (const bf16_t*)d_x;
         const bool many = rows >= 16384;
diff --git a/marqo_amd/csrc/towers.hip b/marqo_amd/csrc/towers.hip
--- a/marqo_amd/csrc/towers.hip
+++ b/marqo_amd/csrc/towers.hip
@@ -23,6 +23,8 @@
     return mq_tower_panel_gemm > 0 && nseq >= mq_tower_panel_gemm && nseq * 4 >= rounds * 256 * 3;
 }
 mq_knob mq_tower_residual_bf16{getenv("MQ_RESIDUAL_BF16") ? atoi(getenv("MQ_RESIDUAL_BF16")) : 0};
+mq_knob mq_tower_pool_strided{getenv("MQ_POOL_STRIDED") ? atoi(getenv("MQ_POOL_STRIDED")) : 1};
+mq_knob mq_tower_assemble_stats{getenv("MQ_ASSEMBLE_STATS") ? atoi(getenv("MQ_ASSEMBLE_STATS")) : 1};
 extern "C" int mq_layernorm_ex(const void* d_x, int x_bf16, const int32_t* d_row_idx, const float* d_g, const float* d_b, void* d_out_bf16,
                                float* d_out_f32, int64_t rows, int32_t W, float eps, void* stream);
 bool mq_gemm_small_ok(int64_t M, int64_t N, int64_t K, bool ln);
@@ -31,6 +33,8 @@
                      const int32_t* d_rows, hipStream_t s);
 int mq_layernorm_pf(const void* d_x, int x_bf16, const int32_t* d_row_idx, const float* d_g, const float* d_b, void* d_out_bf16, float* d_out_f32,
                     int64_t rows, int32_t W, float eps, const void* pf_a, size_t bytes_a, const void* pf_b, size_t bytes_b, hipStream_t s);
+int mq_layernorm_rows_pf(const void* d_x, int x_bf16, const int32_t* d_row_idx, int64_t row_mul, const float* d_g, const float* d_b, void* d_out_bf16,
+                         float* d_out_f32, int64_t rows, int32_t W, float eps, const void* pf_a, size_t bytes_a, const void* pf_b, size_t bytes_b, hipStream_t s);
 static thread_local bool t_ln_prefetch = false;
 static bool weights_outlive_cache(const mq_encoder_cfg* c, int Wa) {
     const double per_layer = ((double)4 * Wa * c->width + (double)(c->mlp_glu ? 3 : 2) * c->width * c->mlp_dim) * 2.0;
@@ -57,6 +61,9 @@
 bool mq_row_stats_ok(int32_t W);
 int mq_row_stats_pf(const void* d_x_bf16, float* d_stats, int64_t rows, int32_t W, float eps, const void* pf_a, size_t bytes_a, const void* pf_b,
                     size_t bytes_b, hipStream_t s);
+bool mq_vit_assemble_stats_ok(int32_t W);
+int mq_vit_assemble_stats(const float* d_patch_out, const float* cls, const float* pos, const float* g, const float* b, void* d_x, float* d_stats, int64_t n,
+                          int32_t T, int32_t W, float eps, const void* pf_a, size_t bytes_a, const void* pf_b, size_t bytes_b, hipStream_t s);
 static bool fold_ok(int xb, const void* wf, const float* bf, const float* sf, int64_t rows, int N, int K) {
     return mq_tower_ln_fold && xb && wf && bf && sf && mq_row_stats_ok(K) && !mq_gemm_small_ok(rows, N, K, false) && !mq_gemm_small_grouped_ok(rows, N, K);
 }
@@ -90,6 +97,12 @@
     return want && (c->precision == MQ_PREC_BF16 || c->precision == MQ_PREC_FP8) && !c->post_ln && !c->d_rope_inv_freq;
 }
 static bool eva_form(const mq_encoder_cfg* c) { return !c->post_ln && (c->mlp_glu || c->d_rope_table); }
+static bool sel_strided_ok(const mq_encoder_cfg* c, int64_t nsel, int64_t sel_stride) {
+    const int W = c->width, F = c->mlp_dim, Wa = c->attn_width ? c->attn_width : c->width;
+    auto small = [](int64_t M, int64_t N, int64_t K) { return mq_gemm_small_ok(M, N, K, false) || mq_gemm_small_grouped_ok(M, N, K); };
+    return mq_tower_pool_strided && sel_stride > 0 && nsel > 0 && !c->post_ln && c->precision == MQ_PREC_BF16 && !eva_form(c) && (sel_stride * Wa) % 8 == 0 &&
+           small(nsel, W, Wa) && small(nsel, F, W) && small(nsel, W, F);
+}
 
 static bool stream_post16(const mq_encoder_cfg* c) {
     return c->residual_stream == 1 && c->post_ln && c->precision == MQ_PREC_BF16 && !c->mlp_glu && !c->d_rope_inv_freq;
@@ -199,8 +212,8 @@
 
 int last_block_selected(const mq_encoder_cfg* cfg, const mq_block_weights& b, int l, float* d_x, int64_t rows,
                         const int32_t* d_cu_seqlens, int64_t nseq, int32_t fixed_len, int32_t max_len,
-                        const int32_t* d_sel, int64_t nsel, void* h, void* a, void* qf, float* row_scale, float* row_stats, bool stats_ready, float* x_sel,
-                        bool f8, hipStream_t s) {
+                        const int32_t* d_sel, int64_t sel_stride, int64_t nsel, void* h, void* a, void* qf, float* row_scale, float* row_stats, bool stats_ready,
+                        float* x_sel, bool f8, hipStream_t s) {
     const int W = cfg->width, F = cfg->mlp_dim, Wa = attn_width(cfg);
     const int act_flag = act_epi(cfg->act);
     const int res_flags = MQ_EPI_BIAS | MQ_EPI_RESIDUAL | MQ_EPI_OUT_F32;
@@ -226,6 +239,19 @@
         const int64_t xrow = (int64_t)W * (xb ? 2 : 4);
         MQ_TRY(ln_gemm(d_x, xb, b.ln1_g, b.ln1_b, cfg->ln_eps, h, b.qkv_w, b.qkv_b, qf, rows, 3 * Wa, W, MQ_EPI_BIAS, s, nullptr, 0, b.qkv_wf, b.qkv_bf, b.qkv_sf, row_stats, stats_ready));
         MQ_TRY(attn_bf16(cfg, qf, a, d_cu_seqlens, nseq, fixed_len, max_len, Wa, s));
+        if (sel_stride > 0) {
+            const int64_t lda = sel_stride * Wa, ldx = sel_stride * W;
+            MQ_TRY(mq_gemm_bf16(a, lda, b.out_w, Wa, b.out_b, d_x, d_x, ldx, nsel, W, Wa, rflags, s));
+            if (mq_gemm_small_ok(nsel, F, W, true))
+                MQ_TRY(mq_ln_gemm_small(d_x, ldx, xb, b.ln2_g, b.ln2_b, cfg->ln_eps, b.fc1_w, W, b.fc1_b, qf, F, nsel, F, W, MQ_EPI_BIAS | act_flag, nullptr, nullptr, s));
+            else {
+                MQ_TRY(mq_layernorm_rows_pf(d_x, xb, nullptr, sel_stride, b.ln2_g, b.ln2_b, h, nullptr, nsel, W, cfg->ln_eps, pf(b.fc1_w), (size_t)F * W * 2, nullptr, 0, s));
+                if (act_flag & MQ_EPI_RELU) MQ_TRY(mq_gemm_small(h, W, b.fc1_w, W, b.fc1_b, nullptr, qf, F, nsel, F, W, MQ_EPI_BIAS | act_flag, s));
+                else MQ_TRY(mq_gemm_bf16(h, W, b.fc1_w, W, b.fc1_b, nullptr, qf, F, nsel, F, W, MQ_EPI_BIAS | act_flag, s));
+            }
+            MQ_TRY(mq_gemm_bf16(qf, F, b.fc2_w, F, b.fc2_b, d_x, d_x, ldx, nsel, W, F, rflags, s));
+            return MQ_OK;
+        }
         MQ_TRY(mq_move_rows(a, d_sel, h, nsel, (int64_t)Wa * 2, false, s));
         MQ_TRY(mq_move_rows(d_x, d_sel, x_sel, nsel, xrow, false, s));
         MQ_TRY(mq_gemm_bf16(h, Wa, b.out_w, Wa, b.out_b, x_sel, x_sel, W, nsel, W, Wa, rflags, s));
@@ -278,6 +304,8 @@
     uint32_t* band_ctr;
     bool x_has_partials;
     int act_flag, res_flags, first8;
+    const float* stats0;
+    bool has_sel;
 
     int block_fp8(const mq_block_weights& b, int l);
     int block_eva(const mq_block_weights& b, int l);
@@ -383,13 +411,15 @@
     const int xb = stream_bf16(cfg) ? 1 : 0;
     const int rflags = xb ? (MQ_EPI_BIAS | MQ_EPI_RESIDUAL) : res_flags;
     bool panel = false;
+    float* stats1 = l == 0 && stats0 ? const_cast<float*>(stats0) : row_stats;
+    const bool ready1 = x_has_partials || (l == 0 && stats0);
     MQ_TRY(ln_gemm_panel(panel, d_x, xb, cfg->ln_eps, qf, rows, nseq, fixed_len, d_cu_seqlens, 3 * Wa, W, MQ_EPI_BIAS, s, b.out_w, (size_t)W * Wa * 2, b.qkv_wf, b.qkv_bf,
-                         b.qkv_sf, row_stats, x_has_partials));
+                         b.qkv_sf, stats1, ready1));
     if (!panel)
         MQ_TRY(ln_gemm(d_x, xb, b.ln1_g, b.ln1_b, cfg->ln_eps, h, b.qkv_w, b.qkv_b, qf, rows, 3 * Wa, W, MQ_EPI_BIAS, s, b.out_w, (size_t)W * Wa * 2,
-                       b.qkv_wf, b.qkv_bf, b.qkv_sf, row_stats, x_has_partials));
+                       b.qkv_wf, b.qkv_bf, b.qkv_sf, stats1, ready1));
     x_has_partials = false;
-    const bool last_pooled = d_sel && nsel > 0 && l == cfg->layers - 1;
+    const bool last_pooled = has_sel && l == cfg->layers - 1;
     const bool mlp_fp8 = cfg->precision == MQ_PREC_FP8 && l >= first8 - cfg->fp8_mlp_extra;
     const bool fold_mlp = mq_tower_ln_fold >= 2 && !last_pooled && !mlp_fp8 && fold_ok(xb, b.fc1_wf, b.fc1_bf, b.fc1_sf, rows, F, W) &&
                           !mq_gemm_small_ok(rows, W, Wa, false) && !mq_gemm_small_grouped_ok(rows, W, Wa);
@@ -485,8 +515,11 @@
 
 int encoder_forward_impl(const mq_encoder_cfg* cfg, const mq_block_weights* blocks, float* d_x, int64_t rows,
                          const int32_t* d_cu_seqlens, int64_t nseq, int32_t fixed_len, int32_t max_len,
-                         const int32_t* d_sel, int64_t nsel, void* d_workspace, size_t workspace_bytes, hipStream_t s) {
+                         const int32_t* d_sel, int64_t nsel, void* d_workspace, size_t workspace_bytes, hipStream_t s, int64_t sel_stride = 0,
+                         const float* stats0 = nullptr) {
     MQ_TRY(check_encoder_cfg(cfg));
+    MQ_CHECK_ARG(sel_stride == 0 || (sel_strided_ok(cfg, nsel, sel_stride) && (nsel - 1) * sel_stride < rows), "mq_encoder_forward: bad pooled-row pitch");
+    const bool has_sel = (d_sel || sel_stride > 0) && nsel > 0;
     MQ_CHECK_ARG(d_x && (blocks || cfg->layers == 0), "mq_encoder_forward: null pointer");
     if (rows <= 0 || cfg->layers == 0) return MQ_OK;
     if (workspace_bytes < encoder_ws(cfg, rows)) {
@@ -510,7 +543,7 @@
     else band_ctr = nullptr;
 
     const size_t xsel_off = align_up((size_t)(nsel > 0 ? nsel : 0) * F * 2, WS_ALIGN);
-    const bool select_last = d_sel && nsel > 0 && nsel * 2 <= rows && mq_tower_row_select && !cfg->mlp_glu && !cfg->d_rope_inv_freq && !cfg->d_rope_table &&
+    const bool select_last = has_sel && nsel * 2 <= rows && mq_tower_row_select && !cfg->mlp_glu && !cfg->d_rope_inv_freq && !cfg->d_rope_table &&
                              !mq_gemm_small_ok(rows, W, W, false) &&
                              !(cfg->precision == MQ_PREC_FP8 && (cfg->d_fp8_act_amax || cfg->post_ln)) &&
                              xsel_off + (size_t)nsel * W * 4 <= (size_t)rows * big * 2;
@@ -525,7 +558,7 @@
     else if (cfg->post_ln) MQ_TRY(mq_cast_bf16(d_x, h, rows * W, s));
 
     EncoderPass p{cfg, blocks, d_x, rows, d_cu_seqlens, nseq, fixed_len, max_len, d_sel, nsel, s, W, F, Wa, h, a, qf, row_scale, row_stats, row_part, xn, band_ctr,
-                   false, act_epi(cfg->act), MQ_EPI_BIAS | MQ_EPI_RESIDUAL | MQ_EPI_OUT_F32, first8};
+                   false, act_epi(cfg->act), MQ_EPI_BIAS | MQ_EPI_RESIDUAL | MQ_EPI_OUT_F32, first8, stats0, has_sel};
     for (int l = 0; l < cfg->layers; ++l) {
         const mq_block_weights& b = blocks[l];
         const bool f8 = l >= first8;
@@ -535,8 +568,8 @@
                          "mq_encoder_forward: layer %d has no fp8 weights", l);
         if (cfg->post_ln && f8 && l == first8 && l > 0) MQ_TRY(mq_rowquant_fp8(d_x, h, row_scale, rows, W, s));
         if (select_last && l == cfg->layers - 1) {
-            MQ_TRY(last_block_selected(cfg, b, l, d_x, rows, d_cu_seqlens, nseq, fixed_len, max_len, d_sel, nsel, h, a, qf, row_scale, row_stats, p.x_has_partials,
-                                       (float*)((char*)qf + xsel_off), f8, s));
+            MQ_TRY(last_block_selected(cfg, b, l, d_x, rows, d_cu_seqlens, nseq, fixed_len, max_len, d_sel, sel_stride, nsel, h, a, qf, row_scale, row_stats,
+                                       p.x_has_partials, (float*)((char*)qf + xsel_off), f8, s));
             break;
         }
         if (f8) MQ_TRY(p.block_fp8(b, l));
@@ -569,7 +602,7 @@
 namespace {
 struct VitPlan {
     int T, np, Kp; int64_t rows;
-    size_t off_x, off_rows, off_cls, off_enc, off_patches, off_patch_out, total;
+    size_t off_x, off_rows, off_cls, off_stats0, off_enc, off_patches, off_patch_out, total;
     size_t off_map_y, off_map_z, off_map_h, off_tok, off_kv;
 };
 VitPlan vit_plan(const mq_vit_cfg* c, int64_t n) {
@@ -582,6 +615,7 @@
     p.off_x = cv.take((size_t)p.rows * W * 4);
     p.off_rows = cv.take((size_t)n * 4);
     p.off_cls = cv.take((size_t)n * W * 2);
+    p.off_stats0 = cv.take((size_t)p.rows * 8);
     p.off_map_y = p.off_map_z = p.off_map_h = p.off_tok = p.off_kv = 0;
     if (map) {
         p.off_map_y = cv.take((size_t)n * W * 4);
@@ -649,7 +683,19 @@
     MQ_TRY(mq_patchify(d_pixels, is_u8, patches, n, cfg->image_size, cfg->patch_size, p.Kp, cfg->mean, cfg->std, s));
     MQ_TRY(mq_gemm_bf16(patches, p.Kp, w->patch_w, p.Kp, nullptr, nullptr, patch_out, W, n * p.np, W, p.Kp, MQ_EPI_OUT_F32, s));
     const int xb = stream_bf16(&cfg->enc) ? 1 : 0;
-    MQ_TRY(mq_vit_assemble(patch_out, w->cls, w->pos, w->ln_pre_g, w->ln_pre_b, x, n, p.T, W, cfg->enc.ln_eps, xb, s));
+    const float* stats0 = nullptr;
+    if (mq_tower_assemble_stats && xb && w->ln_pre_g && cfg->pool == MQ_VIT_POOL_CLS && cfg->enc.precision == MQ_PREC_BF16 && !cfg->enc.post_ln &&
+        !eva_form(&cfg->enc) && cfg->enc.layers >= 2 && mq_tower_ln_fold && mq_tower_panel_gemm == 0 && mq_vit_assemble_stats_ok(W) && w->blocks &&
+        fold_ok(xb, w->blocks[0].qkv_wf, w->blocks[0].qkv_bf, w->blocks[0].qkv_sf, p.rows, 3 * attn_width(&cfg->enc), W) &&
+        !mq_gemm_small_ok(p.rows, 3 * attn_width(&cfg->enc), W, true))
+        stats0 = (const float*)(base + p.off_stats0);
+    if (stats0) {
+        const int Wa = attn_width(&cfg->enc);
+        const bool wpf = weights_outlive_cache(&cfg->enc, Wa);
+        MQ_TRY(mq_vit_assemble_stats(patch_out, w->cls, w->pos, w->ln_pre_g, w->ln_pre_b, x, const_cast<float*>(stats0), n, p.T, W, cfg->enc.ln_eps,
+                                     wpf ? w->blocks[0].qkv_wf : nullptr, (size_t)3 * Wa * W * 2, wpf ? w->blocks[0].out_w : nullptr, (size_t)W * Wa * 2, s));
+    }
+    else MQ_TRY(mq_vit_assemble(patch_out, w->cls, w->pos, w->ln_pre_g, w->ln_pre_b, x, n, p.T, W, cfg->enc.ln_eps, xb, s));
     if (map) {
         const mq_map_head* m = w->map;
         const int F = cfg->map_mlp_dim;
@@ -706,14 +752,16 @@
         if (normalize) MQ_TRY(mq_l2_normalize(d_out, d_out, n, cfg->out_dim, s));
         return MQ_OK;
     }
-    MQ_TRY(mq_cls_rows(rows_idx, n, p.T, s));
+    const int64_t pitch = sel_strided_ok(&cfg->enc, n, p.T) ? p.T : 0;
+    if (!pitch) MQ_TRY(mq_cls_rows(rows_idx, n, p.T, s));
+    else rows_idx = nullptr;
     MQ_TRY(encoder_forward_impl(&cfg->enc, w->blocks, x, p.rows, nullptr, n, p.T, p.T, rows_idx, n, base + p.off_enc,
-                                ws_bytes - p.off_enc, s));
+                                ws_bytes - p.off_enc, s, pitch, stats0));
     if (mq_gemm_small_ok(n, cfg->out_dim, W, true))
-        MQ_TRY(mq_ln_gemm_small(x, W, xb, w->ln_post_g, w->ln_post_b, cfg->enc.ln_eps, w->proj_w, W, w->proj_b, d_out, cfg->out_dim, n, cfg->out_dim,
+        MQ_TRY(mq_ln_gemm_small(x, pitch ? pitch * W : W, xb, w->ln_post_g, w->ln_post_b, cfg->enc.ln_eps, w->proj_w, W, w->proj_b, d_out, cfg->out_dim, n, cfg->out_dim,
                                 W, MQ_EPI_OUT_F32 | (w->proj_b ? MQ_EPI_BIAS : 0), nullptr, rows_idx, s));
     else {
-        MQ_TRY(mq_layernorm_ex(x, xb, rows_idx, w->ln_post_g, w->ln_post_b, cls_ln, nullptr, n, W, cfg->enc.ln_eps, s));
+        MQ_TRY(mq_layernorm_rows_pf(x, xb, rows_idx, pitch ? pitch : 1, w->ln_post_g, w->ln_post_b, cls_ln, nullptr, n, W, cfg->enc.ln_eps, nullptr, 0, nullptr, 0, s));
         MQ_TRY(mq_gemm_bf16(cls_ln, W, w->proj_w, W, w->proj_b, nullptr, d_out, cfg->out_dim, n, cfg->out_dim, W, MQ_EPI_OUT_F32 | (w->proj_b ? MQ_EPI_BIAS : 0), s));
     }
     if (normalize) MQ_TRY(mq_l2_normalize(d_out, d_out, n, cfg->out_dim, s));
diff --git a/marqo_amd/engine/towers.py b/marqo_amd/engine/towers.py
--- a/marqo_amd/engine/towers.py
+++ b/marqo_amd/engine/towers.py
@@ -434,6 +434,14 @@
                 return None
             self._queues[bool(normalize)] = (sig, q)
             return q
+
+    def tune(self, key: str, value: int) -> None:
+        L.check(self.lib.mq_tune(key.encode(), int(value)), "mq_tune")
+        with self._lock:
+            getattr(self, "_graphs", {}).clear()
+            for ent in (self._queues or {}).values():
+                ent[1].close()
+            self._queues = None
 
     def _forget_queue(self, q) -> None:
         with self._lock:
```

Result: faster. 96740 embeddings/s (median of 6 runs) (+1.3%).
